# maneymarkus/BERT4Rec

Measured on AMD Instinct MI355X. Metric: masked positions/sec, higher is better.
Workload: dtype f32 (split products on the 16-bit matrix cores, fp32 accumulate: bf16 hi/lo x3 in the encoder, fp16 hi/lo x3 logits + x2 value products in the masked-LM head; softmax / LayerNorm / AdamW in fp32)

## Files before the change

bert4rec_amd/csrc/b4r_common.h:

```cpp
#pragma once
#include <hip/hip_runtime.h>
#include <stdint.h>
#include "../../include/b4r.h"

typedef float f32x4 __attribute__((ext_vector_type(4)));
typedef float f32x16 __attribute__((ext_vector_type(16)));

#define B4R_WAVE 64

void b4r_set_error(const char* fmt, ...);
#define B4R_CHECK_ARG(cond, code, ...)            \
  do {                                            \
    if (!(cond)) {                                \
      b4r_set_error(__VA_ARGS__);                 \
      return (code);                              \
    }                                             \
  } while (0)
void b4r_timing_mark(const char* what);
void b4r_timing_detail(const char* fmt, ...);
#define B4R_CHECK_LAUNCH(what)                                                   \
  do {                                                                           \
    hipError_t e__ = hipGetLastError();                                          \
    if (e__ != hipSuccess) {                                                     \
      b4r_set_error("%s: launch failed: %s", (what), hipGetErrorString(e__));    \
      return B4R_E_HIP;                                                          \
    }                                                                            \
    b4r_timing_mark(what);                                                       \
  } while (0)

static inline int b4r_cdiv(int64_t a, int64_t b) { return (int)((a + b - 1) / b); }
static inline bool b4r_aligned16(const void* p) { return (((uintptr_t)p) & 15u) == 0; }

struct B4rReduceJob {
  const float* slab; const float* cslab; const float* caslab;
  float* out; float* colsum; float* colsum_a;
  int S, Mo, No, ldo, accumulate;
  const long long* fix = nullptr; const long long* fix_hot = nullptr;
  int fix_hot_elems = 0, fix_slots = 0;
  const int* fix_poison = nullptr;
};
constexpr int B4R_MAX_REDUCE_JOBS = 40;
struct B4rReduceQueue {
  B4rReduceJob jobs[B4R_MAX_REDUCE_JOBS];
  int n;
};
void b4r_reduce_queue_begin(B4rReduceQueue* q);
int b4r_reduce_queue_flush(hipStream_t stream, float* sq_partial = nullptr, int sq_cap = 0, int* sq_np = nullptr,
                           int64_t* covered = nullptr);
bool b4r_reduce_queue_push(const B4rReduceJob& job);
bool b4r_reduce_queue_attach_fixed(const float* out, const long long* fix, const long long* fix_hot, int fix_hot_elems, int fix_slots,
                                   const int* fix_poison = nullptr);
int b4r_launch_reduce_job(const B4rReduceJob& job, hipStream_t stream);

struct B4rHeadMerge {
  const float* part; int slices, M, V;
  const float* T; const float* E; const float* bias; const int64_t* y;
  float* row_out; float* lse_out; int32_t* ylab;
};

#define B4R_STREAM_EMB 0u
#define B4R_STREAM_ATTN_PROBS(layer) (1u + 4u * (uint32_t)(layer))
#define B4R_STREAM_ATTN_OUT(layer) (2u + 4u * (uint32_t)(layer))
#define B4R_STREAM_FFN_OUT(layer) (3u + 4u * (uint32_t)(layer))

constexpr int B4R_ATTN_PITCH = 256;

struct DropArgs {
  const uint32_t* rng;
  uint32_t stream;
  uint32_t thr;
  float scale;
};

static inline DropArgs b4r_make_drop(const uint32_t* rng, uint32_t stream, float rate, int training) {
  DropArgs d;
  d.rng = nullptr; d.stream = stream; d.thr = 0; d.scale = 1.0f;
  if (training && rate > 0.0f && rng != nullptr) {
    d.rng = rng;
    d.thr = (uint32_t)((double)rate * 65536.0);
    d.scale = 1.0f / (1.0f - rate);
  }
  return d;
}

__host__ __device__ __forceinline__ uint32_t b4r_hash32(uint32_t x) {
  x ^= x >> 16; x *= 0x7FEB352Du; x ^= x >> 15; x *= 0x846CA68Bu; x ^= x >> 16;
  return x;
}

__host__ __device__ __forceinline__ float b4r_uniform23(uint32_t h) {
  return ((float)(h >> 9) + 0.5f) * (1.0f / 8388608.0f);
}

__host__ __device__ __forceinline__ uint32_t b4r_sample_word_hd(uint64_t seed, int64_t stream, int64_t id) {
  uint32_t h = b4r_hash32((uint32_t)(uint64_t)id ^ (uint32_t)seed);
  h = b4r_hash32((h ^ (uint32_t)(uint64_t)stream) + (uint32_t)(seed >> 32));
  return b4r_hash32(h ^ (uint32_t)((uint64_t)stream >> 32));
}

__host__ __device__ __forceinline__ double b4r_xln(double x) {
#pragma clang fp contract(off)
  const uint64_t b = __builtin_bit_cast(uint64_t, x);
  int e = (int)(b >> 52) - 1023;
  double m = __builtin_bit_cast(double, (b & 0x000FFFFFFFFFFFFFull) | 0x3FF0000000000000ull);
  if (m > 1.4142135623730951) { m = m * 0.5; e += 1; }
  const double s = (m - 1.0) / (m + 1.0);
  const double z = s * s;
  double p = 1.0 / 15.0;
  p = p * z + 1.0 / 13.0;
  p = p * z + 1.0 / 11.0;
  p = p * z + 1.0 / 9.0;
  p = p * z + 1.0 / 7.0;
  p = p * z + 1.0 / 5.0;
  p = p * z + 1.0 / 3.0;
  p = p * z + 1.0;
  return (double)e * 0.6931471805599453 + (2.0 * s) * p;
}

__host__ __device__ __forceinline__ float b4r_gumbel23(uint32_t h) {
#pragma clang fp contract(off)
  const double u = ((double)(h >> 9) + 0.5) * (1.0 / 8388608.0);
  return (float)(0.0 - b4r_xln(0.0 - b4r_xln(u)));
}

struct DropCtx {
  uint32_t seed, key, thr;
  float scale;
  bool on;
};

__device__ __forceinline__ DropCtx b4r_drop_ctx(const DropArgs& a) {
  DropCtx c;
  c.on = (a.rng != nullptr) && (a.thr != 0);
  c.thr = a.thr; c.scale = a.scale; c.seed = 0; c.key = 0;
  if (c.on) {
    c.seed = a.rng[0];
    c.key = b4r_hash32(a.stream * 0x9E3779B9u + a.rng[1]);
  }
  return c;
}

__device__ __forceinline__ void b4r_group_hash(const DropCtx& c, uint64_t g, uint32_t& h1, uint32_t& h2) {
  const uint32_t lo = (uint32_t)g, hi = (uint32_t)(g >> 32);
  uint32_t h = b4r_hash32(lo ^ c.seed);
  h = b4r_hash32((h ^ hi) + c.key);
  h1 = h;
  h ^= h << 13; h ^= h >> 17; h ^= h << 5;
  h2 = h;
}

struct B4rKeep4 {
  bool k[4];
  __device__ __forceinline__ uint32_t bits() const { return (k[0] ? 1u : 0u) | (k[1] ? 2u : 0u) | (k[2] ? 4u : 0u) | (k[3] ? 8u : 0u); }
};
__device__ __forceinline__ B4rKeep4 b4r_keep4p(const DropCtx& c, uint64_t idx4) {
  uint32_t h1, h2;
  b4r_group_hash(c, idx4 >> 2, h1, h2);
  B4rKeep4 r;
  r.k[0] = (h1 & 0xFFFFu) >= c.thr; r.k[1] = (h1 >> 16) >= c.thr;
  r.k[2] = (h2 & 0xFFFFu) >= c.thr; r.k[3] = (h2 >> 16) >= c.thr;
  return r;
}
__device__ __forceinline__ uint32_t b4r_keep4(const DropCtx& c, uint64_t idx4) { return b4r_keep4p(c, idx4).bits(); }

__device__ __forceinline__ bool b4r_keep(const DropCtx& c, uint64_t idx) {
  uint32_t h1, h2;
  b4r_group_hash(c, idx >> 2, h1, h2);
  const uint32_t w = (idx & 2) ? h2 : h1;
  const uint32_t u = (idx & 1) ? (w >> 16) : (w & 0xFFFFu);
  return u >= c.thr;
}

__device__ __forceinline__ float b4r_drop(const DropCtx& c, float x, uint64_t idx) {
  if (!c.on) return x;
  return b4r_keep(c, idx) ? x * c.scale : 0.0f;
}

__device__ __forceinline__ f32x4 b4r_drop4(const DropCtx& c, f32x4 x, uint64_t idx) {
  if (!c.on) return x;
  if ((idx & 3) == 0) {
    const B4rKeep4 k = b4r_keep4p(c, idx);
    const f32x4 xs = x * c.scale;
#pragma unroll
    for (int e = 0; e < 4; ++e) x[e] = k.k[e] ? xs[e] : 0.0f;
  } else {
#pragma unroll
    for (int e = 0; e < 4; ++e) x[e] = b4r_keep(c, idx + e) ? x[e] * c.scale : 0.0f;
  }
  return x;
}

#include <mutex>
#include <unordered_map>
static inline int b4r_raise_lds(const void* kernel, size_t bytes, const char* who) {
  if (bytes <= 48 * 1024) return B4R_OK;
  static std::mutex mu;
  static std::unordered_map<const void*, size_t> raised;
  std::lock_guard<std::mutex> lock(mu);
  auto it = raised.find(kernel);
  if (it != raised.end() && it->second >= bytes) return B4R_OK;
  hipError_t e = hipFuncSetAttribute(kernel, hipFuncAttributeMaxDynamicSharedMemorySize, (int)bytes);
  if (e != hipSuccess) { b4r_set_error("%s: cannot raise the LDS limit to %zu: %s", who, bytes, hipGetErrorString(e)); return B4R_E_HIP; }
  raised[kernel] = bytes;
  return B4R_OK;
}

typedef __bf16 b4r_bf16x8 __attribute__((ext_vector_type(8)));
typedef __bf16 b4r_bf16x4 __attribute__((ext_vector_type(4)));
typedef __bf16 b4r_bf16x2 __attribute__((ext_vector_type(2)));
typedef float b4r_f32x8 __attribute__((ext_vector_type(8)));
typedef float b4r_f32x2 __attribute__((ext_vector_type(2)));
typedef unsigned int b4r_u32x4 __attribute__((ext_vector_type(4)));
typedef unsigned int b4r_u32x2 __attribute__((ext_vector_type(2)));

__device__ __forceinline__ void b4r_split_pair(float a, float b, uint32_t& hw, uint32_t& lw) {
  const b4r_bf16x2 h = __builtin_convertvector((b4r_f32x2){a, b}, b4r_bf16x2);
  hw = __builtin_bit_cast(uint32_t, h);
  const float h0 = __builtin_bit_cast(float, hw << 16), h1 = __builtin_bit_cast(float, hw & 0xFFFF0000u);
  lw = __builtin_bit_cast(uint32_t, __builtin_convertvector((b4r_f32x2){a - h0, b - h1}, b4r_bf16x2));
}
__device__ __forceinline__ void b4r_split8(const b4r_f32x8 x, b4r_bf16x8& hi, b4r_bf16x8& lo) {
  b4r_u32x4 hw, lw;
#pragma unroll
  for (int j = 0; j < 4; ++j) {
    uint32_t h, l;
    b4r_split_pair(x[2 * j], x[2 * j + 1], h, l);
    hw[j] = h; lw[j] = l;
  }
  hi = __builtin_bit_cast(b4r_bf16x8, hw);
  lo = __builtin_bit_cast(b4r_bf16x8, lw);
}
__device__ __forceinline__ void b4r_split4(const f32x4 x, b4r_bf16x4& hi, b4r_bf16x4& lo) {
  b4r_u32x2 hw, lw;
#pragma unroll
  for (int j = 0; j < 2; ++j) {
    uint32_t h, l;
    b4r_split_pair(x[2 * j], x[2 * j + 1], h, l);
    hw[j] = h; lw[j] = l;
  }
  hi = __builtin_bit_cast(b4r_bf16x4, hw);
  lo = __builtin_bit_cast(b4r_bf16x4, lw);
}

__device__ __forceinline__ float b4r_gelu(float x) { return 0.5f * x * (1.0f + erff(x * 0.70710678118654752440f)); }
__device__ __forceinline__ float b4r_gelu_grad(float x) {
  return 0.5f * (1.0f + erff(x * 0.70710678118654752440f)) + x * 0.39894228040143267794f * __expf(-0.5f * x * x);
}

__device__ __forceinline__ float b4r_erf_as(float u, float& e) {
  const float a = fabsf(u);
  const float t = __builtin_amdgcn_rcpf(fmaf(0.3275911f, a, 1.0f));
  e = __expf(-a * a);
  float q = fmaf(t, 1.061405429f, -1.453152027f);
  q = fmaf(q, t, 1.421413741f);
  q = fmaf(q, t, -0.284496736f);
  q = fmaf(q, t, 0.254829592f);
  return copysignf(fmaf(-q * t, e, 1.0f), u);
}
__device__ __forceinline__ float b4r_gelu_fast(float x) {
  float e;
  return 0.5f * x * (1.0f + b4r_erf_as(x * 0.70710678118654752440f, e));
}
__device__ __forceinline__ float b4r_gelu_grad_fast(float x) {
  float e;
  const float er = b4r_erf_as(x * 0.70710678118654752440f, e);
  return fmaf(x * 0.39894228040143267794f, e, 0.5f * (1.0f + er));
}

constexpr int B4R_ACT_ANY = -1;
constexpr float B4R_SELU_ALPHA = 1.6732632423543772f, B4R_SELU_SCALE = 1.0507009873554805f;

template <bool FAST> __device__ __forceinline__ float b4r_exp_(float x) { return FAST ? __expf(x) : expf(x); }
template <bool FAST> __device__ __forceinline__ float b4r_rcp_(float x) { return FAST ? __builtin_amdgcn_rcpf(x) : 1.0f / x; }
template <bool FAST> __device__ __forceinline__ float b4r_sigmoid_(float x) { return b4r_rcp_<FAST>(1.0f + b4r_exp_<FAST>(-x)); }
template <bool FAST> __device__ __forceinline__ float b4r_tanh_(float x) {
  if (!FAST) return tanhf(x);
  const float t = 1.0f - 2.0f * __builtin_amdgcn_rcpf(__expf(2.0f * fabsf(x)) + 1.0f);
  return copysignf(t, x);
}
template <bool FAST> __device__ __forceinline__ float b4r_expm1_(float x) { return FAST ? __expf(x) - 1.0f : expm1f(x); }

template <bool FAST>
__device__ __forceinline__ void b4r_act_both(int id, float x, float& f, float& d) {
  switch (id) {
    case B4R_ACT_GELU:
      if (FAST) { float e; const float er = b4r_erf_as(x * 0.70710678118654752440f, e); const float cdf = 0.5f * (1.0f + er);
                  f = x * cdf; d = fmaf(x * 0.39894228040143267794f, e, cdf); }
      else { f = b4r_gelu(x); d = b4r_gelu_grad(x); }
      break;
    case B4R_ACT_RELU: f = x > 0.f ? x : 0.f; d = x > 0.f ? 1.f : 0.f; break;
    case B4R_ACT_SWISH: { const float s = b4r_sigmoid_<FAST>(x); f = x * s; d = s * fmaf(x, 1.0f - s, 1.0f); break; }
    case B4R_ACT_TANH: { const float t = b4r_tanh_<FAST>(x); f = t; d = fmaf(-t, t, 1.0f); break; }
    case B4R_ACT_SIGMOID: { const float s = b4r_sigmoid_<FAST>(x); f = s; d = s * (1.0f - s); break; }
    case B4R_ACT_ELU: { const float e = b4r_exp_<FAST>(fminf(x, 0.f)); f = x > 0.f ? x : b4r_expm1_<FAST>(fminf(x, 0.f)); d = x > 0.f ? 1.f : e; break; }
    case B4R_ACT_SELU: {
      const float e = b4r_exp_<FAST>(fminf(x, 0.f));
      f = x > 0.f ? B4R_SELU_SCALE * x : (B4R_SELU_SCALE * B4R_SELU_ALPHA) * b4r_expm1_<FAST>(fminf(x, 0.f));
      d = x > 0.f ? B4R_SELU_SCALE : (B4R_SELU_SCALE * B4R_SELU_ALPHA) * e;
      break;
    }
    case B4R_ACT_SOFTPLUS: {
      const float e = b4r_exp_<FAST>(-fabsf(x));
      f = fmaxf(x, 0.f) + (FAST ? __logf(1.0f + e) : log1pf(e));
      d = x >= 0.f ? b4r_rcp_<FAST>(1.0f + e) : e * b4r_rcp_<FAST>(1.0f + e);
      break;
    }
    default: f = x; d = 1.f; break;
  }
}
template <bool FAST> __device__ __forceinline__ float b4r_act_val(int id, float x) { float f, d; b4r_act_both<FAST>(id, x, f, d); return f; }
template <bool FAST> __device__ __forceinline__ float b4r_act_grad(int id, float x) { float f, d; b4r_act_both<FAST>(id, x, f, d); return d; }
template <int ACT> __device__ __forceinline__ int b4r_act_id(int id) { return ACT == B4R_ACT_ANY ? id : ACT; }

#include <type_traits>
template <class F>
static inline int b4r_act_dispatch(int act, F&& f) {
  switch (act) {
    case B4R_ACT_RELU: return f(std::integral_constant<int, B4R_ACT_RELU>{});
    case B4R_ACT_SWISH: return f(std::integral_constant<int, B4R_ACT_SWISH>{});
    case B4R_ACT_TANH: return f(std::integral_constant<int, B4R_ACT_TANH>{});
    case B4R_ACT_SIGMOID: return f(std::integral_constant<int, B4R_ACT_SIGMOID>{});
    case B4R_ACT_ELU: return f(std::integral_constant<int, B4R_ACT_ELU>{});
    case B4R_ACT_SELU: return f(std::integral_constant<int, B4R_ACT_SELU>{});
    case B4R_ACT_SOFTPLUS: return f(std::integral_constant<int, B4R_ACT_SOFTPLUS>{});
    case B4R_ACT_LINEAR: return f(std::integral_constant<int, B4R_ACT_LINEAR>{});
    default: return f(std::integral_constant<int, B4R_ACT_GELU>{});
  }
}

__device__ __forceinline__ float b4r_seq_amax(const int64_t* mask_row, int L) {
  int any = 0;
  for (int k = threadIdx.x; k < L; k += blockDim.x) any |= (mask_row[k] != 0) ? 1 : 0;
  return __syncthreads_or(any) ? 0.0f : -1e9f;
}

__device__ __forceinline__ float b4r_wave_sum(float v) {
#pragma unroll
  for (int o = 32; o > 0; o >>= 1) v += __shfl_xor(v, o, 64);
  return v;
}
__device__ __forceinline__ float b4r_wave_max(float v) {
#pragma unroll
  for (int o = 32; o > 0; o >>= 1) v = fmaxf(v, __shfl_xor(v, o, 64));
  return v;
}
```

bert4rec_amd/csrc/b4r_gemm.hip:

```cpp
#include "b4r_common.h"

namespace {

constexpr int BM = 128, BN = 64, BK = 32;
constexpr int LDS_A = BK + 4;
constexpr int LDS_BN = BN;
constexpr int LDS_BK = BK + 4;

struct GemmP {
  const float* A; const float* B; float* C; const float* bias; float* C2; const float* R;
  int lda, ldb, ldc, ldc2, ldr;
  int M, N, K;
  int tiles_n;
  int k_chunk;
  int64_t split_stride;
  int a_vec, b_vec;
  float qscale; int qcols;
  DropArgs drop;
  int act;
};
constexpr int EPI_BIAS_ACT = 12, EPI_ACT_BWD = 13;

__device__ __forceinline__ f32x4 load4_guard(const float* base, int64_t off, int n_valid, bool vec) {
  f32x4 v = {0.f, 0.f, 0.f, 0.f};
  if (n_valid >= 4 && vec) {
    v = *reinterpret_cast<const f32x4*>(base + off);
  } else {
#pragma unroll
    for (int e = 0; e < 4; ++e)
      if (e < n_valid) v[e] = base[off + e];
  }
  return v;
}

template <bool B_NK, int EPI, bool A_DROP>
__global__ __launch_bounds__(256) void gemm_kernel(GemmP p) {
  __shared__ __attribute__((aligned(16))) float sA[BM * LDS_A];
  __shared__ __attribute__((aligned(16))) float sB[B_NK ? BN * LDS_BK : BK * LDS_BN];

  const int tid = threadIdx.x, lane = tid & 63, wave = __builtin_amdgcn_readfirstlane(tid >> 6);
  const int tile_m = blockIdx.x / p.tiles_n, tile_n = blockIdx.x % p.tiles_n;
  const int m0 = tile_m * BM, n0 = tile_n * BN;
  const int h = lane >> 5, l31 = lane & 31;

  DropCtx dctx = b4r_drop_ctx(p.drop);

  f32x16 acc0, acc1;
#pragma unroll
  for (int i = 0; i < 16; ++i) { acc0[i] = 0.f; acc1[i] = 0.f; }

  f32x4 ra[4], rb[2];

  auto load_tiles = [&](int k0) {
#pragma unroll
    for (int i = 0; i < 4; ++i) {
      const int f = tid + 256 * i;
      const int row = f >> 3, c4 = (f & 7) * 4;
      const int gr = m0 + row, gk = k0 + c4;
      f32x4 v = {0.f, 0.f, 0.f, 0.f};
      if (gr < p.M) v = load4_guard(p.A, (int64_t)gr * p.lda + gk, p.K - gk, p.a_vec != 0);
      if (A_DROP) {
        if (dctx.on) {
#pragma unroll
          for (int e = 0; e < 4; ++e) v[e] = b4r_drop(dctx, v[e], (uint64_t)gr * (uint64_t)p.K + (uint64_t)(gk + e));
        }
      }
      ra[i] = v;
    }
#pragma unroll
    for (int i = 0; i < 2; ++i) {
      const int f = tid + 256 * i;
      f32x4 v = {0.f, 0.f, 0.f, 0.f};
      if (B_NK) {
        const int nr = f >> 3, c4 = (f & 7) * 4;
        const int gn = n0 + nr, gk = k0 + c4;
        if (gn < p.N) v = load4_guard(p.B, (int64_t)gn * p.ldb + gk, p.K - gk, p.b_vec != 0);
      } else {
        const int kr = f >> 4, c4 = (f & 15) * 4;
        const int gk = k0 + kr, gn = n0 + c4;
        if (gk < p.K) v = load4_guard(p.B, (int64_t)gk * p.ldb + gn, p.N - gn, p.b_vec != 0);
      }
      rb[i] = v;
    }
  };

  auto store_tiles = [&]() {
#pragma unroll
    for (int i = 0; i < 4; ++i) {
      const int f = tid + 256 * i;
      const int row = f >> 3, c4 = (f & 7) * 4;
      *reinterpret_cast<f32x4*>(&sA[row * LDS_A + c4]) = ra[i];
    }
#pragma unroll
    for (int i = 0; i < 2; ++i) {
      const int f = tid + 256 * i;
      if (B_NK) {
        const int nr = f >> 3, c4 = (f & 7) * 4;
        *reinterpret_cast<f32x4*>(&sB[nr * LDS_BK + c4]) = rb[i];
      } else {
        const int kr = f >> 4, c4 = (f & 15) * 4;
        *reinterpret_cast<f32x4*>(&sB[kr * LDS_BN + c4]) = rb[i];
      }
    }
  };

  const int k_begin = blockIdx.y * p.k_chunk;
  const int k_end = min(p.K, k_begin + p.k_chunk);
  const int nk = (k_end - k_begin + BK - 1) / BK;
  if (blockIdx.y > 0) p.C += (int64_t)blockIdx.y * p.split_stride;
  if (nk > 0) load_tiles(k_begin);
  for (int kt = 0; kt < nk; ++kt) {
    __syncthreads();
    store_tiles();
    __syncthreads();
    if (kt + 1 < nk) load_tiles(k_begin + (kt + 1) * BK);
    const int arow = wave * 32 + l31;
#pragma unroll
    for (int t = 0; t < 4; ++t) {
      const f32x4 a = *reinterpret_cast<const f32x4*>(&sA[arow * LDS_A + 8 * t + 4 * h]);
      if (B_NK) {
        const f32x4 b0 = *reinterpret_cast<const f32x4*>(&sB[l31 * LDS_BK + 8 * t + 4 * h]);
        const f32x4 b1 = *reinterpret_cast<const f32x4*>(&sB[(32 + l31) * LDS_BK + 8 * t + 4 * h]);
#pragma unroll
        for (int r = 0; r < 4; ++r) {
          acc0 = __builtin_amdgcn_mfma_f32_32x32x2f32(a[r], b0[r], acc0, 0, 0, 0);
          acc1 = __builtin_amdgcn_mfma_f32_32x32x2f32(a[r], b1[r], acc1, 0, 0, 0);
        }
      } else {
#pragma unroll
        for (int r = 0; r < 4; ++r) {
          const int kk = 8 * t + 4 * h + r;
          const float b0 = sB[kk * LDS_BN + l31];
          const float b1 = sB[kk * LDS_BN + 32 + l31];
          acc0 = __builtin_amdgcn_mfma_f32_32x32x2f32(a[r], b0, acc0, 0, 0, 0);
          acc1 = __builtin_amdgcn_mfma_f32_32x32x2f32(a[r], b1, acc1, 0, 0, 0);
        }
      }
    }
  }

#pragma unroll
  for (int jt = 0; jt < 2; ++jt) {
    const int col = n0 + jt * 32 + l31;
    if (col >= p.N) continue;
    float bv = 0.f;
    if (EPI == B4R_EPI_BIAS || EPI == B4R_EPI_BIAS_QSCALE || EPI == B4R_EPI_BIAS_GELU || EPI == B4R_EPI_BIAS_DROP_RES ||
        EPI == B4R_EPI_BIAS_TANH || EPI == EPI_BIAS_ACT)
      bv = p.bias[col];
    const float qs = (EPI == B4R_EPI_BIAS_QSCALE && col < p.qcols) ? p.qscale : 1.0f;
#pragma unroll
    for (int reg = 0; reg < 16; ++reg) {
      const int row = m0 + wave * 32 + (reg & 3) + 8 * (reg >> 2) + 4 * h;
      if (row >= p.M) continue;
      float v = (jt == 0 ? acc0[reg] : acc1[reg]);
      const int64_t co = (int64_t)row * p.ldc + col;
      if (EPI == B4R_EPI_NONE) {
        p.C[co] = v;
      } else if (EPI == B4R_EPI_BIAS) {
        p.C[co] = v + bv;
      } else if (EPI == B4R_EPI_BIAS_QSCALE) {
        p.C[co] = (v + bv) * qs;
      } else if (EPI == B4R_EPI_BIAS_GELU) {
        const float pre = v + bv;
        p.C2[(int64_t)row * p.ldc2 + col] = pre;
        p.C[co] = b4r_gelu(pre);
      } else if (EPI == EPI_BIAS_ACT) {
        const float pre = v + bv;
        p.C2[(int64_t)row * p.ldc2 + col] = pre;
        p.C[co] = b4r_act_val<false>(p.act, pre);
      } else if (EPI == B4R_EPI_BIAS_DROP_RES) {
        float y = v + bv;
        y = b4r_drop(dctx, y, (uint64_t)row * (uint64_t)p.N + (uint64_t)col);
        p.C[co] = p.R[(int64_t)row * p.ldr + col] + y;
      } else if (EPI == B4R_EPI_GELU_BWD) {
        p.C[co] = v * b4r_gelu_grad(p.R[(int64_t)row * p.ldr + col]);
      } else if (EPI == EPI_ACT_BWD) {
        p.C[co] = v * b4r_act_grad<false>(p.act, p.R[(int64_t)row * p.ldr + col]);
      } else if (EPI == B4R_EPI_ADD_RES) {
        p.C[co] = v + p.R[(int64_t)row * p.ldr + col];
      } else if (EPI == B4R_EPI_BIAS_TANH) {
        p.C[co] = tanhf(v + bv);
      }
    }
  }
}

constexpr int TB = 64;
constexpr int TK = 32;

struct TnP {
  const float* A; const float* B; float* slab; float* colsum_slab; float* colsum_a_slab;
  int lda, ldb;
  int R, Mo, No;
  int chunk;
  int a_vec, b_vec;
  DropArgs drop;
};

template <bool B_DROP>
__global__ __launch_bounds__(256) void gemm_tn_kernel(TnP p) {
  __shared__ __attribute__((aligned(16))) float sA[TK * TB];
  __shared__ __attribute__((aligned(16))) float sB[TK * TB];
  __shared__ float sRed[4 * TB];

  const int tid = threadIdx.x, lane = tid & 63, wave = __builtin_amdgcn_readfirstlane(tid >> 6);
  const int i0 = blockIdx.x * TB, j0 = blockIdx.y * TB, z = blockIdx.z;
  const int r_begin = z * p.chunk;
  const int r_end = min(p.R, r_begin + p.chunk);
  const int h = lane >> 5, l31 = lane & 31;
  const int wm = wave >> 1, wn = wave & 1;
  const bool do_colsum = (p.colsum_slab != nullptr) && (blockIdx.x == 0);
  const bool do_colsum_a = (p.colsum_a_slab != nullptr) && (blockIdx.y == 0);

  DropCtx dctx = b4r_drop_ctx(p.drop);

  f32x16 acc;
#pragma unroll
  for (int i = 0; i < 16; ++i) acc[i] = 0.f;
  float cs = 0.f, csa = 0.f;

  f32x4 ra[2], rb[2];
  auto load_tiles = [&](int r0) {
#pragma unroll
    for (int i = 0; i < 2; ++i) {
      const int f = tid + 256 * i;
      const int rr = f >> 4, c4 = (f & 15) * 4;
      const int gr = r0 + rr;
      f32x4 va = {0.f, 0.f, 0.f, 0.f}, vb = {0.f, 0.f, 0.f, 0.f};
      if (gr < r_end) {
        va = load4_guard(p.A, (int64_t)gr * p.lda + i0 + c4, p.Mo - (i0 + c4), p.a_vec != 0);
        vb = load4_guard(p.B, (int64_t)gr * p.ldb + j0 + c4, p.No - (j0 + c4), p.b_vec != 0);
        if (B_DROP) {
          if (dctx.on) {
#pragma unroll
            for (int e = 0; e < 4; ++e)
              vb[e] = b4r_drop(dctx, vb[e], (uint64_t)gr * (uint64_t)p.No + (uint64_t)(j0 + c4 + e));
          }
        }
      }
      ra[i] = va; rb[i] = vb;
    }
  };
  auto store_tiles = [&]() {
#pragma unroll
    for (int i = 0; i < 2; ++i) {
      const int f = tid + 256 * i;
      const int rr = f >> 4, c4 = (f & 15) * 4;
      *reinterpret_cast<f32x4*>(&sA[rr * TB + c4]) = ra[i];
      *reinterpret_cast<f32x4*>(&sB[rr * TB + c4]) = rb[i];
    }
  };

  if (r_begin < r_end) load_tiles(r_begin);
  for (int r0 = r_begin; r0 < r_end; r0 += TK) {
    __syncthreads();
    store_tiles();
    __syncthreads();
    if (r0 + TK < r_end) load_tiles(r0 + TK);
#pragma unroll
    for (int s = 0; s < 16; ++s) {
      const float a = sA[(2 * s + h) * TB + 32 * wm + l31];
      const float b = sB[(2 * s + h) * TB + 32 * wn + l31];
      acc = __builtin_amdgcn_mfma_f32_32x32x2f32(a, b, acc, 0, 0, 0);
    }
    if (do_colsum) {
#pragma unroll
      for (int r = 0; r < 8; ++r) cs += sB[(wave * 8 + r) * TB + lane];
    }
    if (do_colsum_a) {
#pragma unroll
      for (int r = 0; r < 8; ++r) csa += sA[(wave * 8 + r) * TB + lane];
    }
  }

  const int col = j0 + 32 * wn + l31;
  if (col < p.No) {
    float* slab = p.slab + (int64_t)z * p.Mo * p.No;
#pragma unroll
    for (int reg = 0; reg < 16; ++reg) {
      const int row = i0 + 32 * wm + (reg & 3) + 8 * (reg >> 2) + 4 * h;
      if (row < p.Mo) slab[(int64_t)row * p.No + col] = acc[reg];
    }
  }
  if (do_colsum) {
    sRed[wave * TB + lane] = cs;
    __syncthreads();
    if (tid < TB && j0 + tid < p.No)
      p.colsum_slab[(int64_t)z * p.No + j0 + tid] = (sRed[tid] + sRed[TB + tid]) + (sRed[2 * TB + tid] + sRed[3 * TB + tid]);
  }
  if (do_colsum_a) {
    __syncthreads();
    sRed[wave * TB + lane] = csa;
    __syncthreads();
    if (tid < TB && i0 + tid < p.Mo)
      p.colsum_a_slab[(int64_t)z * p.Mo + i0 + tid] = (sRed[tid] + sRed[TB + tid]) + (sRed[2 * TB + tid] + sRed[3 * TB + tid]);
  }
}

constexpr int RZ = 16;
constexpr int RE = 256;
constexpr int RQ = 4096;
typedef B4rReduceJob ReduceJobView;
__device__ __forceinline__ int reduce_mat_blocks(int S, int64_t total) { return (int)((total + (S <= RZ ? RQ : RE) - 1) / (S <= RZ ? RQ : RE)); }
__device__ __forceinline__ float reduce_store(const ReduceJobView& job, int64_t eo, float r) {
  const int row = (int)(eo / job.No), col = (int)(eo % job.No);
  float* o = job.out + (int64_t)row * job.ldo + col;
  if (job.fix != nullptr) {
    long long q = job.fix[eo];
    if (eo < job.fix_hot_elems) {
      for (int s0 = 0; s0 < job.fix_slots; s0 += 16) {
        long long v[16];
#pragma unroll
        for (int u = 0; u < 16; ++u) v[u] = s0 + u < job.fix_slots ? job.fix_hot[(int64_t)(s0 + u) * job.fix_hot_elems + eo] : 0ll;
#pragma unroll
        for (int u = 0; u < 16; ++u) q += v[u];
      }
    }
    r += (float)q * (1.f / 68719476736.f);
    if (job.fix_poison != nullptr && *job.fix_poison != 0) r = __builtin_nanf("");
  }
  if (job.accumulate) r += *o;
  *o = r;
  return r;
}
__device__ __forceinline__ float slab_reduce_block(const ReduceJobView& job, int block, float (*sp)[RE]) {
  float sq = 0.f;
  const int64_t total = (int64_t)job.Mo * job.No;
  const int mat_blocks = reduce_mat_blocks(job.S, total);
  const int lane = threadIdx.x & 63, zl = __builtin_amdgcn_readfirstlane(threadIdx.x >> 6);
  const bool vec = (total % 4 == 0) && ((reinterpret_cast<uintptr_t>(job.slab) & 15) == 0);
  if (block < mat_blocks && job.S <= RZ) {
    const int64_t e = (int64_t)block * RQ + 4 * (int64_t)threadIdx.x;
    if (e >= total) return sq;
    f32x4 v[RZ];
#pragma unroll
    for (int z = 0; z < RZ; ++z) {
      v[z] = (f32x4){0.f, 0.f, 0.f, 0.f};
      if (z < job.S) {
        if (vec) v[z] = *reinterpret_cast<const f32x4*>(job.slab + (int64_t)z * total + e);
        else
#pragma unroll
          for (int k = 0; k < 4; ++k)
            if (e + k < total) v[z][k] = job.slab[(int64_t)z * total + e + k];
      }
    }
    f32x4 r = {0.f, 0.f, 0.f, 0.f};
#pragma unroll
    for (int z = 0; z < RZ; ++z) r += v[z];
#pragma unroll
    for (int k = 0; k < 4; ++k)
      if (e + k < total) { const float w = reduce_store(job, e + k, r[k]); sq = fmaf(w, w, sq); }
    return sq;
  }
  if (block < mat_blocks) {
    const int64_t e = (int64_t)block * RE + 4 * lane;
    f32x4 s = {0.f, 0.f, 0.f, 0.f};
    if (vec) {
      if (e < total) {
        const float* src = job.slab + e;
        for (int z = zl; z < job.S; z += 8 * RZ) {
          f32x4 v[8];
#pragma unroll
          for (int u = 0; u < 8; ++u)
            v[u] = z + u * RZ < job.S ? *reinterpret_cast<const f32x4*>(src + (int64_t)(z + u * RZ) * total) : (f32x4){0.f, 0.f, 0.f, 0.f};
#pragma unroll
          for (int u = 0; u < 8; ++u) s += v[u];
        }
      }
    } else {
      for (int z = zl; z < job.S; z += RZ) {
#pragma unroll
        for (int c = 0; c < 4; ++c)
          if (e + c < total) s[c] += job.slab[(int64_t)z * total + e + c];
      }
    }
    *reinterpret_cast<f32x4*>(&sp[zl][4 * lane]) = s;
    __syncthreads();
    if (zl < 4) {
      const int l = threadIdx.x;
      const int64_t eo = (int64_t)block * RE + l;
      if (eo < total) {
        float r = 0.f;
#pragma unroll
        for (int z = 0; z < RZ; ++z) r += sp[z][l];
        const float v = reduce_store(job, eo, r);
        sq = v * v;
      }
    }
    return sq;
  }
  const int64_t n_cs = job.colsum ? job.No : 0, n_csa = job.colsum_a ? job.Mo : 0;
  const int64_t e = (int64_t)(block - mat_blocks) * 64 + lane;
  const float* src = nullptr;
  int64_t stride = 0, idx = 0;
  if (e < n_cs) { src = job.cslab; stride = job.No; idx = e; }
  else if (e < n_cs + n_csa) { src = job.caslab; stride = job.Mo; idx = e - n_cs; }
  float s = 0.f;
  if (src) {
    for (int z = zl; z < job.S; z += 8 * RZ) {
      float v[8];
#pragma unroll
      for (int u = 0; u < 8; ++u) v[u] = z + u * RZ < job.S ? src[(int64_t)(z + u * RZ) * stride + idx] : 0.f;
#pragma unroll
      for (int u = 0; u < 8; ++u) s += v[u];
    }
  }
  sp[zl][lane] = s;
  __syncthreads();
  if (zl == 0 && src) {
    float r = 0.f;
#pragma unroll
    for (int z = 0; z < RZ; ++z) r += sp[z][lane];
    if (e < n_cs) job.colsum[idx] = r;
    else job.colsum_a[idx] = r;
    sq = r * r;
  }
  return sq;
}

__global__ __launch_bounds__(64 * RZ) void slab_reduce_kernel(ReduceJobView job) {
  __shared__ __attribute__((aligned(16))) float sp[RZ][RE];
  (void)slab_reduce_block(job, (int)blockIdx.x, sp);
}

int slab_reduce_grid(int S, int Mo, int No, bool cs, bool csa) {
  return b4r_cdiv((int64_t)Mo * No, S <= RZ ? RQ : RE) + b4r_cdiv((int64_t)(cs ? No : 0) + (csa ? Mo : 0), 64);
}

int tn_split(int R, int Mo, int No) {
  const int tiles = b4r_cdiv(Mo, TB) * b4r_cdiv(No, TB);
  int S = b4r_cdiv(1024, tiles);
  const int max_s = b4r_cdiv(R, 4 * TK);
  if (S > max_s) S = max_s;
  if (S > 256) S = 256;
  if (S < 1) S = 1;
  return S;
}

template <bool B_NK, int EPI>
void launch_gemm(const GemmP& p, int a_drop, dim3 grid, hipStream_t s) {
  if (a_drop)
    hipLaunchKernelGGL((gemm_kernel<B_NK, EPI, true>), grid, dim3(256), 0, s, p);
  else
    hipLaunchKernelGGL((gemm_kernel<B_NK, EPI, false>), grid, dim3(256), 0, s, p);
}

template <bool B_NK>
int dispatch_epi(const GemmP& p, int epi, int a_drop, dim3 grid, hipStream_t s) {
  switch (epi) {
    case B4R_EPI_NONE: launch_gemm<B_NK, B4R_EPI_NONE>(p, a_drop, grid, s); break;
    case B4R_EPI_BIAS: launch_gemm<B_NK, B4R_EPI_BIAS>(p, a_drop, grid, s); break;
    case B4R_EPI_BIAS_QSCALE: launch_gemm<B_NK, B4R_EPI_BIAS_QSCALE>(p, a_drop, grid, s); break;
    case B4R_EPI_BIAS_GELU:
      if (p.act != B4R_ACT_GELU) launch_gemm<B_NK, EPI_BIAS_ACT>(p, a_drop, grid, s);
      else launch_gemm<B_NK, B4R_EPI_BIAS_GELU>(p, a_drop, grid, s);
      break;
    case B4R_EPI_BIAS_DROP_RES: launch_gemm<B_NK, B4R_EPI_BIAS_DROP_RES>(p, a_drop, grid, s); break;
    case B4R_EPI_GELU_BWD:
      if (p.act != B4R_ACT_GELU) launch_gemm<B_NK, EPI_ACT_BWD>(p, a_drop, grid, s);
      else launch_gemm<B_NK, B4R_EPI_GELU_BWD>(p, a_drop, grid, s);
      break;
    case B4R_EPI_ADD_RES: launch_gemm<B_NK, B4R_EPI_ADD_RES>(p, a_drop, grid, s); break;
    case B4R_EPI_BIAS_TANH: launch_gemm<B_NK, B4R_EPI_BIAS_TANH>(p, a_drop, grid, s); break;
    default: b4r_set_error("b4r_gemm_f32: unknown epilogue %d", epi); return B4R_E_BADARG;
  }
  return B4R_OK;
}

}

int b4r_launch_slab_reduce(const float* slab, int S, int Mo, int No, float* out, int ldo, int accumulate,
                           hipStream_t stream) {
  ReduceJobView job{slab, nullptr, nullptr, out, nullptr, nullptr, S, Mo, No, ldo, accumulate};
  hipLaunchKernelGGL(slab_reduce_kernel, dim3(slab_reduce_grid(S, Mo, No, false, false)), dim3(64 * RZ), 0, stream, job);
  B4R_CHECK_LAUNCH("slab_reduce");
  return B4R_OK;
}

namespace {
struct MultiReduceP {
  B4rReduceJob jobs[B4R_MAX_REDUCE_JOBS];
  int block_begin[B4R_MAX_REDUCE_JOBS + 1];
  int n;
  float* sq_partial;
};
__global__ __launch_bounds__(64 * RZ) void multi_slab_reduce_kernel(MultiReduceP p) {
  __shared__ __attribute__((aligned(16))) float sp[RZ][RE];
  int j = 0;
  while (j + 1 < p.n && (int)blockIdx.x >= p.block_begin[j + 1]) ++j;
  const B4rReduceJob q = p.jobs[j];
  float sq = slab_reduce_block(q, (int)blockIdx.x - p.block_begin[j], sp);
  if (p.sq_partial != nullptr) {
    __shared__ float s_sq[RZ];
    sq = b4r_wave_sum(sq);
    __syncthreads();
    if ((threadIdx.x & 63) == 0) s_sq[threadIdx.x >> 6] = sq;
    __syncthreads();
    if (threadIdx.x == 0) {
      float t = 0.f;
#pragma unroll
      for (int z = 0; z < RZ; ++z) t += s_sq[z];
      p.sq_partial[blockIdx.x] = t;
    }
  }
}
thread_local B4rReduceQueue* g_queue = nullptr;
}

void b4r_reduce_queue_begin(B4rReduceQueue* q) { q->n = 0; g_queue = q; }
bool b4r_reduce_queue_push(const B4rReduceJob& job) {
  if (g_queue == nullptr || g_queue->n >= B4R_MAX_REDUCE_JOBS) return false;
  g_queue->jobs[g_queue->n++] = job;
  return true;
}
bool b4r_reduce_queue_attach_fixed(const float* out, const long long* fix, const long long* fix_hot, int fix_hot_elems, int fix_slots,
                                   const int* fix_poison) {
  if (g_queue == nullptr) return false;
  for (int j = 0; j < g_queue->n; ++j) {
    B4rReduceJob& job = g_queue->jobs[j];
    if (job.out == out && job.ldo == job.No && job.fix == nullptr) {
      job.fix = fix; job.fix_hot = fix_hot; job.fix_hot_elems = fix_hot_elems; job.fix_slots = fix_slots; job.fix_poison = fix_poison;
      return true;
    }
  }
  return false;
}
int b4r_launch_reduce_job(const B4rReduceJob& job, hipStream_t stream) {
  if (b4r_reduce_queue_push(job)) return B4R_OK;
  hipLaunchKernelGGL(slab_reduce_kernel, dim3(slab_reduce_grid(job.S, job.Mo, job.No, job.colsum != nullptr, job.colsum_a != nullptr)),
                     dim3(64 * RZ), 0, stream, job);
  B4R_CHECK_LAUNCH("slab_reduce");
  return B4R_OK;
}
int b4r_reduce_queue_flush(hipStream_t stream, float* sq_partial, int sq_cap, int* sq_np, int64_t* covered) {
  B4rReduceQueue* q = g_queue;
  g_queue = nullptr;
  if (sq_np) *sq_np = 0;
  if (covered) *covered = 0;
  if (q == nullptr || q->n == 0) return B4R_OK;
  MultiReduceP p;
  p.n = q->n;
  int blocks = 0;
  int64_t elems = 0;
  for (int j = 0; j < q->n; ++j) {
    p.jobs[j] = q->jobs[j];
    p.block_begin[j] = blocks;
    blocks += slab_reduce_grid(q->jobs[j].S, q->jobs[j].Mo, q->jobs[j].No, q->jobs[j].colsum != nullptr, q->jobs[j].colsum_a != nullptr);
    elems += (int64_t)q->jobs[j].Mo * q->jobs[j].No + (q->jobs[j].colsum ? q->jobs[j].No : 0) + (q->jobs[j].colsum_a ? q->jobs[j].Mo : 0);
  }
  p.block_begin[q->n] = blocks;
  p.sq_partial = (sq_partial != nullptr && blocks <= sq_cap) ? sq_partial : nullptr;
  if (p.sq_partial && sq_np) *sq_np = blocks;
  if (covered) *covered = elems;
  hipLaunchKernelGGL(multi_slab_reduce_kernel, dim3(blocks), dim3(64 * RZ), 0, stream, p);
  B4R_CHECK_LAUNCH("multi_slab_reduce");
  return B4R_OK;
}

int b4r_launch_slab_reduce_full(const float* slab, int S, int Mo, int No, float* out, int ldo, int accumulate,
                                const float* cslab, float* colsum, const float* caslab, float* colsum_a, hipStream_t stream) {
  B4rReduceJob job{slab, cslab, caslab, out, colsum, colsum_a, S, Mo, No, ldo, accumulate};
  if (b4r_reduce_queue_push(job)) return B4R_OK;
  ReduceJobView view{slab, cslab, caslab, out, colsum, colsum_a, S, Mo, No, ldo, accumulate};
  hipLaunchKernelGGL(slab_reduce_kernel, dim3(slab_reduce_grid(S, Mo, No, colsum != nullptr, colsum_a != nullptr)), dim3(64 * RZ),
                     0, stream, view);
  B4R_CHECK_LAUNCH("slab_reduce");
  return B4R_OK;
}

int b4r_gemm_rx_launch(const b4r_gemm_desc* d, hipStream_t stream);
bool b4r_gemm_rx_supported(const b4r_gemm_desc* d);
bool b4r_gemm_rx_tn_supported(const b4r_gemm_tn_desc* d);
int64_t b4r_gemm_rx_tn_scratch_floats(int R, int Mo, int No);
int b4r_gemm_rx_tn_launch(const b4r_gemm_tn_desc* d, float* scratch, hipStream_t stream);
bool b4r_gemm_rx_tn_pair_supported(const b4r_gemm_tn_desc* d0, const b4r_gemm_tn_desc* d1);
int b4r_gemm_rx_tn_pair_launch(const b4r_gemm_tn_desc* d0, float* scratch0, const b4r_gemm_tn_desc* d1, float* scratch1,
                               hipStream_t stream);
static int g_gemm_mode = B4R_GEMM_BF16X3;
extern "C" int b4r_set_gemm_mode(int mode) {
  B4R_CHECK_ARG(mode == B4R_GEMM_F32 || mode == B4R_GEMM_BF16X3 || mode == B4R_GEMM_BF16, B4R_E_BADARG,
                "b4r_set_gemm_mode: unknown mode %d", mode);
  g_gemm_mode = mode;
  return B4R_OK;
}
extern "C" int b4r_get_gemm_mode(void) { return g_gemm_mode; }
extern "C" int b4r_split_mode(void) { return g_gemm_mode == B4R_GEMM_BF16X3 || g_gemm_mode == B4R_GEMM_BF16; }
extern "C" int b4r_gemm_terms(void) { return g_gemm_mode == B4R_GEMM_BF16 ? 1 : g_gemm_mode == B4R_GEMM_BF16X3 ? 3 : 0; }

extern "C" int64_t b4r_gemm_ln_bwd_partial_floats(int32_t M) { return (int64_t)b4r_cdiv(M > 0 ? M : 1, 64) * 128; }
extern "C" int b4r_gemm_ln_supported(const b4r_gemm_desc* d) {
  if (d == nullptr || !b4r_split_mode() || !d->A || !d->B || !d->C || d->M <= 0) return 0;
  if (d->epilogue == B4R_EPI_BIAS_GELU_LN) return b4r_gemm_rx_supported(d) ? 1 : 0;
  return ((d->epilogue == B4R_EPI_BIAS_DROP_RES_LN || d->epilogue == B4R_EPI_ADD_RES_LN_BWD) && d->R && d->ldr >= d->N &&
          b4r_gemm_rx_supported(d)) ? 1 : 0;
}

extern "C" int b4r_gemm_f32(const b4r_gemm_desc* d, b4r_stream_t stream) {
  B4R_CHECK_ARG(d != nullptr, B4R_E_BADARG, "b4r_gemm_f32: null descriptor");
  B4R_CHECK_ARG(d->A && d->B && d->C, B4R_E_BADARG, "b4r_gemm_f32: null operand");
  B4R_CHECK_ARG(d->M > 0 && d->N > 0 && d->K > 0, B4R_E_SHAPE, "b4r_gemm_f32: bad shape M=%d N=%d K=%d", d->M, d->N, d->K);
  B4R_CHECK_ARG(d->lda >= d->K && d->ldc >= d->N && d->ldb >= (d->b_is_nk ? d->K : d->N), B4R_E_SHAPE,
                "b4r_gemm_f32: leading dimension smaller than the row length");
  const int epi = d->epilogue;
  b4r_timing_detail("M=%d N=%d K=%d epi=%d%s", d->M, d->N, d->K, d->epilogue, d->b_is_nk ? " B^T" : "");
  const bool needs_bias = epi == B4R_EPI_BIAS || epi == B4R_EPI_BIAS_QSCALE || epi == B4R_EPI_BIAS_GELU ||
                          epi == B4R_EPI_BIAS_DROP_RES || epi == B4R_EPI_BIAS_TANH || epi == B4R_EPI_BIAS_DROP_RES_LN ||
                          epi == B4R_EPI_BIAS_GELU_LN;
  B4R_CHECK_ARG(!needs_bias || d->bias, B4R_E_BADARG, "b4r_gemm_f32: epilogue %d needs a bias", epi);
  const bool needs_r = epi == B4R_EPI_BIAS_DROP_RES || epi == B4R_EPI_GELU_BWD || epi == B4R_EPI_ADD_RES ||
                       epi == B4R_EPI_BIAS_DROP_RES_LN || epi == B4R_EPI_ADD_RES_LN_BWD;
  B4R_CHECK_ARG(!needs_r || (d->R && d->ldr >= d->N), B4R_E_BADARG, "b4r_gemm_f32: epilogue %d needs R", epi);
  B4R_CHECK_ARG(epi != B4R_EPI_BIAS_GELU || (d->C2 && d->ldc2 >= d->N), B4R_E_BADARG, "b4r_gemm_f32: BIAS_GELU needs C2");
  B4R_CHECK_ARG(epi >= B4R_EPI_NONE && epi <= B4R_EPI_BIAS_GELU_LN, B4R_E_BADARG, "b4r_gemm_f32: unknown epilogue %d", epi);
  B4R_CHECK_ARG(d->activation >= 0 && d->activation < B4R_ACT_COUNT, B4R_E_BADARG, "b4r_gemm_f32: unknown activation %d",
                d->activation);
  B4R_CHECK_ARG(d->a_gather_idx == nullptr || (epi == B4R_EPI_BIAS_GELU_LN && d->a_gather_add_per > 0 && d->a_gather_per > 0),
                B4R_E_BADARG, "b4r_gemm_f32: a_gather_idx only with B4R_EPI_BIAS_GELU_LN (and a_gather_add_per, a_gather_per > 0)");
  B4R_CHECK_ARG(d->a_copy == nullptr || (d->a_gather_idx != nullptr && d->a_copy_ld >= d->K && d->a_copy_ld % 4 == 0 &&
                                         b4r_aligned16(d->a_copy)),
                B4R_E_BADARG, "b4r_gemm_f32: a_copy needs a_gather_idx, a_copy_ld >= K (multiple of 4) and 16-byte alignment");
  if (epi == B4R_EPI_BIAS_GELU_LN) {
    B4R_CHECK_ARG(d->C2 && d->C3 && d->ln_gamma && d->ln_beta, B4R_E_BADARG, "b4r_gemm_f32: BIAS_GELU_LN needs C2, C3, ln_gamma, ln_beta");
    B4R_CHECK_ARG(b4r_gemm_ln_supported(d), B4R_E_SHAPE,
                  "b4r_gemm_f32: BIAS_GELU_LN not available for M=%d N=%d K=%d in this mode (b4r_gemm_ln_supported)", d->M, d->N,
                  d->K);
  }
  if (epi == B4R_EPI_ADD_RES_LN_BWD) {
    B4R_CHECK_ARG(d->C2 && d->ln_gamma && (d->ln_z || d->ln_ids) && d->ln_mean && d->ln_rstd && d->ln_dgamma, B4R_E_BADARG,
                  "b4r_gemm_f32: ADD_RES_LN_BWD needs C2 (partials), ln_gamma, ln_z (or ln_ids), ln_mean, ln_rstd, ln_dgamma");
    B4R_CHECK_ARG(!d->ln_ids || (d->ln_table && d->ln_pos && d->ln_L > 0 && d->ln_V > 0), B4R_E_BADARG,
                  "b4r_gemm_f32: ADD_RES_LN_BWD with ln_ids needs ln_table, ln_pos, ln_L, ln_V");
    B4R_CHECK_ARG(d->ln_dbeta == d->ln_dgamma + 64, B4R_E_BADARG, "b4r_gemm_f32: ADD_RES_LN_BWD: ln_dbeta must be ln_dgamma + 64");
    B4R_CHECK_ARG(b4r_gemm_ln_supported(d), B4R_E_SHAPE,
                  "b4r_gemm_f32: ADD_RES_LN_BWD not available for M=%d N=%d K=%d in this mode (b4r_gemm_ln_supported)", d->M,
                  d->N, d->K);
    int rc = b4r_gemm_rx_launch(d, (hipStream_t)stream);
    if (rc) return rc;
    return b4r_launch_slab_reduce_full(d->C2, b4r_cdiv(d->M, 64), 1, 128, d->ln_dgamma, 128, 0, nullptr, nullptr, nullptr, nullptr,
                                       (hipStream_t)stream);
  }
  if (epi == B4R_EPI_BIAS_DROP_RES_LN) {
    B4R_CHECK_ARG(d->C2 && d->ln_gamma && d->ln_beta, B4R_E_BADARG, "b4r_gemm_f32: BIAS_DROP_RES_LN needs C2, ln_gamma, ln_beta");
    B4R_CHECK_ARG(b4r_gemm_ln_supported(d), B4R_E_SHAPE,
                  "b4r_gemm_f32: BIAS_DROP_RES_LN not available for M=%d N=%d K=%d in this mode (b4r_gemm_ln_supported)", d->M,
                  d->N, d->K);
  }
  if (b4r_split_mode() && b4r_gemm_rx_supported(d)) return b4r_gemm_rx_launch(d, (hipStream_t)stream);

  GemmP p;
  p.A = d->A; p.B = d->B; p.C = d->C; p.bias = d->bias; p.C2 = d->C2; p.R = d->R;
  p.lda = d->lda; p.ldb = d->ldb; p.ldc = d->ldc; p.ldc2 = d->ldc2; p.ldr = d->ldr;
  p.M = d->M; p.N = d->N; p.K = d->K;
  p.tiles_n = b4r_cdiv(d->N, BN);
  p.k_chunk = b4r_cdiv(d->K, BK) * BK;
  p.split_stride = 0;
  p.a_vec = (b4r_aligned16(d->A) && (d->lda % 4 == 0)) ? 1 : 0;
  p.b_vec = (b4r_aligned16(d->B) && (d->ldb % 4 == 0)) ? 1 : 0;
  p.qscale = d->qscale; p.qcols = d->qcols;
  p.drop = b4r_make_drop(d->rng, d->drop_stream, d->drop_rate, 1);
  p.act = d->activation;
  const int a_drop = (d->a_dropout && p.drop.rng != nullptr) ? 1 : 0;
  const int64_t tiles = (int64_t)b4r_cdiv(d->M, BM) * p.tiles_n;
  B4R_CHECK_ARG(tiles < 2147483647LL, B4R_E_SHAPE, "b4r_gemm_f32: too many tiles");
  dim3 grid((unsigned)tiles);
  int rc = d->b_is_nk ? dispatch_epi<true>(p, epi, a_drop, grid, (hipStream_t)stream)
                      : dispatch_epi<false>(p, epi, a_drop, grid, (hipStream_t)stream);
  if (rc != B4R_OK) return rc;
  B4R_CHECK_LAUNCH("b4r_gemm_f32");
  return B4R_OK;
}

bool b4r_gemm_rx_splitk_supported(const b4r_gemm_desc* d, int k_pad_ok);
int b4r_gemm_rx_splitk_launch(const b4r_gemm_desc* d, int splits, float* slabs, int* slabs_used, hipStream_t stream);

int b4r_gemm_f32_splitk(const b4r_gemm_desc* d, int splits, float* scratch, int k_pad_ok, hipStream_t stream) {
  B4R_CHECK_ARG(d && scratch && d->epilogue == B4R_EPI_NONE && !d->a_dropout, B4R_E_BADARG, "gemm_splitk: plain product only");
  if (splits > 1 && b4r_split_mode() && b4r_gemm_rx_splitk_supported(d, k_pad_ok)) {
    int used = 0;
    int rc = b4r_gemm_rx_splitk_launch(d, splits, scratch, &used, stream);
    if (rc) return rc;
    return b4r_launch_slab_reduce(scratch, used, d->M, d->N, d->C, d->ldc, 0, stream);
  }
  if (splits <= 1) return b4r_gemm_f32(d, (b4r_stream_t)stream);
  GemmP p;
  p.A = d->A; p.B = d->B; p.C = scratch; p.bias = nullptr; p.C2 = nullptr; p.R = nullptr;
  p.lda = d->lda; p.ldb = d->ldb; p.ldc = d->N; p.ldc2 = 0; p.ldr = 0;
  p.M = d->M; p.N = d->N; p.K = d->K;
  p.tiles_n = b4r_cdiv(d->N, BN);
  p.k_chunk = b4r_cdiv(b4r_cdiv(d->K, splits), BK) * BK;
  p.split_stride = (int64_t)d->M * d->N;
  p.a_vec = (b4r_aligned16(d->A) && (d->lda % 4 == 0)) ? 1 : 0;
  p.b_vec = (b4r_aligned16(d->B) && (d->ldb % 4 == 0)) ? 1 : 0;
  p.qscale = 1.f; p.qcols = 0;
  p.drop = b4r_make_drop(nullptr, 0, 0.f, 0);
  p.act = B4R_ACT_GELU;
  const int64_t tiles = (int64_t)b4r_cdiv(d->M, BM) * p.tiles_n;
  dim3 grid((unsigned)tiles, (unsigned)splits);
  if (d->b_is_nk)
    hipLaunchKernelGGL((gemm_kernel<true, B4R_EPI_NONE, false>), grid, dim3(256), 0, stream, p);
  else
    hipLaunchKernelGGL((gemm_kernel<false, B4R_EPI_NONE, false>), grid, dim3(256), 0, stream, p);
  B4R_CHECK_LAUNCH("gemm_splitk");
  return b4r_launch_slab_reduce(scratch, splits, d->M, d->N, d->C, d->ldc, 0, stream);
}

extern "C" int64_t b4r_gemm_tn_scratch_floats(int32_t R, int32_t Mo, int32_t No) {
  if (R <= 0 || Mo <= 0 || No <= 0) return 0;
  const int S = tn_split(R, Mo, No);
  const int64_t a = (int64_t)S * Mo * No + (int64_t)S * No + (int64_t)S * Mo;
  const int64_t b = b4r_gemm_rx_tn_scratch_floats(R, Mo, No);
  return a > b ? a : b;
}

extern "C" int b4r_gemm_tn_dgrad_supported(const b4r_gemm_tn_desc* d) {
  return (d != nullptr && b4r_split_mode() && d->Mo >= 64 && d->Mo % 64 == 0 && d->No == 64 && d->R > 0 && d->A &&
          d->B && d->dgrad_w && d->dgrad_out && d->dgrad_ldw >= 64 && d->dgrad_ldw % 4 == 0 && b4r_aligned16(d->dgrad_w) &&
          d->dgrad_ldo >= d->Mo && (d->dgrad_gelu_pre == nullptr || d->dgrad_ldg >= d->Mo) && b4r_gemm_rx_tn_supported(d)) ? 1 : 0;
}

extern "C" int b4r_gemm_tn_f32(const b4r_gemm_tn_desc* d, float* scratch, b4r_stream_t stream) {
  B4R_CHECK_ARG(d != nullptr && scratch != nullptr, B4R_E_BADARG, "b4r_gemm_tn_f32: null argument");
  B4R_CHECK_ARG(d->A && d->B && d->out, B4R_E_BADARG, "b4r_gemm_tn_f32: null operand");
  B4R_CHECK_ARG(d->R > 0 && d->Mo > 0 && d->No > 0, B4R_E_SHAPE, "b4r_gemm_tn_f32: bad shape");
  B4R_CHECK_ARG(d->lda >= d->Mo && d->ldb >= d->No && d->ldo >= d->No, B4R_E_SHAPE, "b4r_gemm_tn_f32: bad leading dimension");
  b4r_timing_detail("R=%d Mo=%d No=%d%s", d->R, d->Mo, d->No, d->dgrad_out ? " +dgrad" : "");
  B4R_CHECK_ARG(d->activation >= 0 && d->activation < B4R_ACT_COUNT, B4R_E_BADARG, "b4r_gemm_tn_f32: unknown activation %d",
                d->activation);
  if (d->dgrad_out != nullptr) {
    B4R_CHECK_ARG(d->dgrad_w != nullptr, B4R_E_BADARG, "b4r_gemm_tn_f32: dgrad_out needs dgrad_w");
    B4R_CHECK_ARG(b4r_gemm_tn_dgrad_supported(d), B4R_E_SHAPE,
                  "b4r_gemm_tn_f32: the fused input gradient needs No = 64, Mo %% 64 == 0, aligned operands and the bf16x3 mode "
                  "(b4r_gemm_tn_dgrad_supported)");
  }
  if (b4r_split_mode() && b4r_gemm_rx_tn_supported(d)) return b4r_gemm_rx_tn_launch(d, scratch, (hipStream_t)stream);
  const int S = tn_split(d->R, d->Mo, d->No);
  TnP p;
  p.A = d->A; p.B = d->B; p.lda = d->lda; p.ldb = d->ldb;
  p.R = d->R; p.Mo = d->Mo; p.No = d->No;
  p.chunk = b4r_cdiv(b4r_cdiv(d->R, S), TK) * TK;
  p.slab = scratch;
  p.colsum_slab = d->colsum ? scratch + (int64_t)S * d->Mo * d->No : nullptr;
  p.colsum_a_slab = d->colsum_a ? scratch + (int64_t)S * d->Mo * d->No + (int64_t)S * d->No : nullptr;
  p.a_vec = (b4r_aligned16(d->A) && (d->lda % 4 == 0)) ? 1 : 0;
  p.b_vec = (b4r_aligned16(d->B) && (d->ldb % 4 == 0)) ? 1 : 0;
  p.drop = b4r_make_drop(d->rng, d->drop_stream, d->drop_rate, 1);
  const bool b_drop = d->b_dropout && p.drop.rng != nullptr;
  dim3 grid(b4r_cdiv(d->Mo, TB), b4r_cdiv(d->No, TB), S);
  if (b_drop)
    hipLaunchKernelGGL((gemm_tn_kernel<true>), grid, dim3(256), 0, (hipStream_t)stream, p);
  else
    hipLaunchKernelGGL((gemm_tn_kernel<false>), grid, dim3(256), 0, (hipStream_t)stream, p);
  B4R_CHECK_LAUNCH("b4r_gemm_tn_f32");
  return b4r_launch_slab_reduce_full(p.slab, S, d->Mo, d->No, d->out, d->ldo, d->accumulate, p.colsum_slab, d->colsum,
                                     p.colsum_a_slab, d->colsum_a, (hipStream_t)stream);
}

int b4r_gemm_tn_pair(const b4r_gemm_tn_desc* d0, float* scratch0, const b4r_gemm_tn_desc* d1, float* scratch1, hipStream_t stream) {
  const bool plain = d0 && d1 && scratch0 && scratch1 && d0->A && d0->B && d0->out && d1->A && d1->B && d1->out && d0->R > 0 &&
                     d1->R > 0 && d0->Mo > 0 && d0->No > 0 && d1->Mo > 0 && d1->No > 0 && d0->lda >= d0->Mo && d0->ldb >= d0->No &&
                     d0->ldo >= d0->No && d1->lda >= d1->Mo && d1->ldb >= d1->No && d1->ldo >= d1->No;
  if (plain && b4r_split_mode() && b4r_gemm_rx_tn_pair_supported(d0, d1))
    return b4r_gemm_rx_tn_pair_launch(d0, scratch0, d1, scratch1, stream);
  int rc = b4r_gemm_tn_f32(d0, scratch0, (b4r_stream_t)stream);
  if (rc) return rc;
  return b4r_gemm_tn_f32(d1, scratch1, (b4r_stream_t)stream);
}
```

bert4rec_amd/csrc/b4r_model.hip:

```cpp
#include <stdarg.h>
#include <stdio.h>
#include <string.h>

#include <string>
#include <vector>

#include <algorithm>
#include "b4r_common.h"

int b4r_ln_bwd_launch(const float* dy, const float* z, const float* mean, const float* rstd, const float* gamma,
                      int rows, int H, float* dz, float* dgamma, float* dbeta, float* scratch, const int64_t* ids,
                      const float* table, const float* pos_table, int L, int V, DropArgs drop, hipStream_t stream,
                      const float* gelu_pre = nullptr, const B4rHeadMerge* merge = nullptr, int act = B4R_ACT_GELU);
int b4r_scatter_add_rows_impl(const float* src, const int64_t* idx, int64_t idx_add_per, int per, int n, int H,
                              float* dst, int dst_ld, const int64_t* skip_if_zero, int64_t dst_rows, int hot_rows,
                              float* hot_scratch, hipStream_t stream);
int64_t b4r_scatter_hot_scratch_floats(int hot_rows, int H);
int b4r_batch_colsum(const float* x, int B, int L, int H, float* dpos, float* scratch, hipStream_t stream);
int b4r_gemm_f32_splitk(const b4r_gemm_desc* d, int splits, float* scratch, int k_pad_ok, hipStream_t stream);
bool b4r_head32_hidden_ok(int H);
int b4r_head32_fwd_slices(int M, int V, int H);
int64_t b4r_head32_fwd_scratch_floats(int M, int V, int H);
int64_t b4r_head32_dE_scratch_floats(int M, int V, int H);
bool b4r_head32_combine_foldable(int M, int V, int H);
// ... 847 lines not shown
  ModelCfg mc;
  RC(resolve_cfg(cfg_ex, &mc));
  const ModelCfg* cfg = &mc;
  B4R_CHECK_ARG(params && seq && rows && out && scratch && R > 0 && n_seq_rows > 0, B4R_E_BADARG, "b4r_mlm_transform_rows: bad argument");
  B4R_CHECK_ARG(b4r_aligned16(params) && b4r_aligned16(seq) && b4r_aligned16(out) && b4r_aligned16(scratch), B4R_E_ALIGN,
                "b4r_mlm_transform_rows: buffers must be 16-byte aligned");
  const ParamLayout pl = make_param_layout(*cfg);
  const int H = cfg->hidden_size, E = cfg->E;
  float* gath = scratch; float* upre = gath + up4((int64_t)R * H); float* u = upre + up4((int64_t)R * H);
  float* mean = u + up4((int64_t)R * H); float* rstd = mean + up4(R);
  return transform_fwd({.A = seq, .lda = H, .B = params + pl.wd, .ldb = E, .C = u, .ldc = E, .M = R, .N = E, .K = H,
                        .epilogue = B4R_EPI_BIAS_GELU_LN, .bias = params + pl.bd, .C2 = out, .ldc2 = E, .qscale = 1.f,
                        .c_pad_scratch = 0, .ln_gamma = params + pl.lnm_g, .ln_beta = params + pl.lnm_b, .ln_mean = mean,
                        .ln_rstd = rstd, .ln_eps = cfg->ln_eps, .C3 = upre, .ldc3 = E,
                        .a_gather_idx = rows, .a_gather_add_per = n_seq_rows, .a_gather_per = R ,
                        .activation = cfg->act_mlm},
                       gath, stream);
}
extern "C" int b4r_mlm_transform_rows(const b4r_model_config* cfg, const float* params, const float* seq, int64_t n_seq_rows,
                                      const int64_t* rows, int32_t R, float* out, float* scratch, b4r_stream_t stream) {
  const auto x = classic_ex(cfg);
  return b4r_mlm_transform_rows_ex(cfg ? &x : nullptr, params, seq, n_seq_rows, rows, R, out, scratch, stream);
}

extern "C" int b4r_loss_ex(const b4r_model_config_ex* cfg_ex, const b4r_batch* batch, void* workspace, int64_t workspace_bytes,
                           b4r_train_state* state, int32_t want_grad, b4r_stream_t stream) {
  ModelCfg mc;
  RC(resolve_cfg(cfg_ex, &mc));
  const ModelCfg* cfg = &mc;
  RC(check_batch(batch, cfg, true));
  B4R_CHECK_ARG(batch->masked_lm_ids && workspace && state, B4R_E_BADARG, "b4r_loss: needs masked_lm_ids, workspace, state");
  const WsLayout w = make_ws_layout(*cfg, batch->B, batch->L, batch->P);
  B4R_CHECK_ARG(workspace_bytes >= w.total * (int64_t)sizeof(float), B4R_E_NOMEM, "b4r_loss: workspace too small");
  float* ws = static_cast<float*>(workspace);
  if (want_grad & B4R_LOSS_FUSED_HEAD)
    return b4r_ce_finalize_launch(ws + w.rowsc, (int)w.M, state, (want_grad & B4R_LOSS_OVERWRITE) ? 1 : 0, (hipStream_t)stream);
  return b4r_softmax_ce(ws + w.logits, (int)w.M, cfg->vocab_size, (int)w.Vp, batch->masked_lm_ids, ws + w.rowsc, state,
                        want_grad & (1 | B4R_LOSS_OVERWRITE), stream);
}

extern "C" int b4r_loss(const b4r_model_config* cfg, const b4r_batch* batch, void* workspace, int64_t workspace_bytes,
                        b4r_train_state* state, int32_t want_grad, b4r_stream_t stream) {
  const auto x = classic_ex(cfg);
  return b4r_loss_ex(cfg ? &x : nullptr, batch, workspace, workspace_bytes, state, want_grad, stream);
}

namespace {

int head_bwd(Step& c) {
  const StepPlan& p = c.plan;
  const ParamLayout& pl = c.pl; const WsLayout& w = c.w;
  const int H = c.H, E = c.E, M = c.M, V = c.V, Vp = (int)w.Vp;
  const bool loss_sums = (c.flags & B4R_FLAG_LOSS_SUMS) != 0;
  float *fwd_part = nullptr, *dE_scratch = nullptr;
  if (p.fused_head && p.defer_combine) RC(c.take(b4r_head32_fwd_scratch_floats(M, V, E), &fwd_part));
  if (p.fused_head) RC(c.take(b4r_head32_dE_scratch_floats(M, V, E), &dE_scratch));
  alignas(8) char rider[128];
  int rider_blocks = 0;
  if (p.fused_head)
    RC(b4r_head32_dE_pack_job(c.at(w.t), c.at(w.head_lse), reinterpret_cast<const int32_t*>(c.at(w.head_ylab)), M, V, E, dE_scratch,
                              fwd_part, c.batch.masked_lm_ids, rider, sizeof(rider), &rider_blocks));
  RC(b4r_zero2(c.grads, pl.total, c.at(p.rows() ? w.hot : w.dx),
               p.rows() ? (p.slot_only_last ? w.db - w.hot : w.da - w.hot) : w.db - w.dx, c.s,
               ((c.flags & B4R_FLAG_GRAD_TAIL) && !p.defer_combine) ? c.grd(pl.total) : nullptr, c.state,
               (loss_sums && !p.defer_combine) ? c.at(w.rowsc) : nullptr, M, rider_blocks > 0 ? rider : nullptr, rider_blocks));

  float* dlog = c.at(w.logits);
  float* sc;
  if (p.fused_head) {
    RC(b4r_head32_dE_launch(c.at(w.t), c.prm(pl.word_emb), c.prm(pl.out_bias), c.at(w.head_lse),
                            reinterpret_cast<const int32_t*>(c.at(w.head_ylab)), M, V, E, dE_scratch, c.grd(pl.word_emb),
                            c.grd(pl.out_bias), c.s, fwd_part, c.batch.masked_lm_ids, rider_blocks > 0 ? 1 : 0));
  } else {
    const b4r_gemm_desc d{.A = dlog, .lda = Vp, .B = c.prm(pl.word_emb), .ldb = E, .C = c.at(w.dt), .ldc = E, .M = M, .N = E, .K = V,
                          .b_is_nk = 0, .epilogue = B4R_EPI_NONE};
    const int splits = mlm_dt_splits(M, E, V);
    RC(c.take((int64_t)splits * M * E, &sc));
    RC(b4r_gemm_f32_splitk(&d, splits, sc, (pl.word_emb + (int64_t)Vp * E <= pl.total) ? 1 : 0, c.s));
    RC(c.take(b4r_gemm_tn_scratch_floats(M, V, E), &sc));
    RC(gemm_tn_f32({.A = dlog, .lda = Vp, .B = c.at(w.t), .ldb = E, .out = c.grd(pl.word_emb), .ldo = E, .R = M, .Mo = V, .No = E,
                    .colsum_a = c.grd(pl.out_bias)}, sc, c.s));
  }
  const B4rHeadMerge merge{fwd_part, fwd_part ? b4r_head32_fwd_slices(M, V, E) : 0, M, V, c.at(w.t), c.prm(pl.word_emb),
                           c.prm(pl.out_bias), c.batch.masked_lm_ids, c.at(w.rowsc), c.at(w.head_lse),
                           reinterpret_cast<int32_t*>(c.at(w.head_ylab))};
  RC(c.take(b4r_ln_bwd_scratch_floats(M, E), &sc));
  RC(b4r_ln_bwd_launch(c.at(w.dt), c.at(w.u), c.at(w.meanm), c.at(w.rstdm), c.prm(pl.lnm_g), M, E, c.at(w.dt), c.grd(pl.lnm_g),
                       c.grd(pl.lnm_b), sc, nullptr, nullptr, nullptr, 1, 1, b4r_make_drop(nullptr, 0, 0.f, 0), c.s, c.at(w.upre),
                       fwd_part ? &merge : nullptr, c.cfg.act_mlm));
  b4r_gemm_tn_desc d{.A = c.at(w.gath), .lda = H, .B = c.at(w.dt), .ldb = E, .out = c.grd(pl.wd), .ldo = E, .R = M, .Mo = H, .No = E,
                     .colsum = c.grd(pl.bd), .dgrad_w = c.prm(pl.wd), .dgrad_ldw = E, .dgrad_out = c.at(w.dg), .dgrad_ldo = H};
  RC(c.take(b4r_gemm_tn_scratch_floats(M, H, E), &sc));
  if (b4r_gemm_tn_dgrad_supported(&d)) {
    RC(gemm_tn_f32(d, sc, c.s));
  } else {
    d.dgrad_w = nullptr; d.dgrad_ldw = 0; d.dgrad_out = nullptr; d.dgrad_ldo = 0;
    RC(gemm_tn_f32(d, sc, c.s));
    RC(gemm_f32({.A = c.at(w.dt), .lda = E, .B = c.prm(pl.wd), .ldb = E, .C = c.at(w.dg), .ldc = H, .M = M, .N = H, .K = E,
                 .b_is_nk = 1, .epilogue = B4R_EPI_NONE, .qscale = 1.f, .c_pad_scratch = 1}, c.s));
  }
  if (p.rows()) return B4R_OK;
  return b4r_scatter_add_rows_impl(c.at(w.dg), c.batch.masked_lm_positions, c.L, c.P, M, H, c.at(w.dx), H, c.batch.masked_lm_ids, c.N,
                                   0, nullptr, c.s);
}

int wgrad_with_dgrad(Step& c, b4r_gemm_tn_desc d, const b4r_gemm_desc& dx) {
  float* sc; RC(c.take(b4r_gemm_tn_scratch_floats(d.R, d.Mo, d.No), &sc));
  if (b4r_gemm_tn_dgrad_supported(&d)) return gemm_tn_f32(d, sc, c.s);
  RC(gemm_f32(dx, c.s));
  d.dgrad_w = nullptr; d.dgrad_ldw = 0; d.dgrad_out = nullptr; d.dgrad_ldo = 0; d.dgrad_gelu_pre = nullptr; d.dgrad_ldg = 0;
  return gemm_tn_f32(d, sc, c.s);
}

int ffn_bwd_block(Step& c, int i) {
  const ParamLayout& pl = c.pl; const WsLayout& w = c.w;
  b4r_ffn_desc fd = ffn_desc(c, i);
  fd.x1 = c.plan.x1_stored ? c.at(w.x1[i]) : nullptr;
  fd.dz2 = c.at(w.da); fd.z1 = c.at(w.z1[i]); fd.mean1 = c.at(w.mean1[i]); fd.rstd1 = c.at(w.rstd1[i]);
  fd.ln1_gamma = c.prm(pl.ln1_g[i]); fd.ln1_beta = c.prm(pl.ln1_b[i]); fd.dz1 = c.at(w.db);
  fd.dW1 = c.grd(pl.w1[i]); fd.db1 = c.grd(pl.b1[i]); fd.dW2 = c.grd(pl.w2[i]); fd.db2 = c.grd(pl.b2[i]);
  fd.dln1_gamma = c.grd(pl.ln1_g[i]);
  RC(c.take(b4r_ffn_block_bwd_scratch_floats(c.N), &fd.scratch));
  if (c.plan.head_rows && i == c.last) {
    fd.dz2 = nullptr;
    fd.slot_positions = c.batch.masked_lm_positions; fd.slot_ids = c.batch.masked_lm_ids; fd.slots_per_seq = c.batch.P; fd.seq_len = c.L;
    fd.max_rows = (int32_t)w.maxrows;
    fd.slot_grad = c.at(w.dg); fd.z2 = c.at(w.z2[i]); fd.mean2 = c.at(w.mean2[i]); fd.rstd2 = c.at(w.rstd2[i]);
    fd.ln_gamma = c.prm(pl.ln2_g[i]); fd.dln_gamma = c.grd(pl.ln2_g[i]); fd.dz2_rows = c.at(w.dz2c);
  }
  return b4r_ffn_block_bwd(&fd, c.s);
}

int ffn_bwd_compact(Step& c, int i) {
  const ParamLayout& pl = c.pl; const WsLayout& w = c.w;
  const int H = c.H, I = c.I, M = c.M;
  const int64_t* pos = c.batch.masked_lm_positions;
  const CompactRows cr = compact_rows(w, i, M, H, I);
  float* dz2c = c.at(w.dzc_a);
  float* dz2d = c.od > 0.f ? c.at(w.dzc_b) : dz2c;
  float* sc; RC(c.take(ln_scratch_floats(c.N, H), &sc));
  RC(b4r_ln_bwd_launch(c.at(w.dg), c.at(w.z2[i]), c.at(w.mean2[i]), c.at(w.rstd2[i]), c.prm(pl.ln2_g[i]), M, H, dz2c, c.grd(pl.ln2_g[i]),
                       c.grd(pl.ln2_b[i]), sc, nullptr, nullptr, nullptr, 1, 1, b4r_make_drop(nullptr, 0, 0.f, 0), c.s));
  if (c.od > 0.f)
    RC(b4r_slot_rows_drop(dz2c, pos, c.L, c.P, M, H, b4r_make_drop(c.rng, B4R_STREAM_FFN_OUT(i), c.od, 1), dz2d, c.s));
  RC(gemm_f32({.A = dz2d, .lda = H, .B = c.prm(pl.w2[i]), .ldb = H, .C = c.at(w.df), .ldc = I, .M = M, .N = I, .K = H, .b_is_nk = 1,
               .epilogue = B4R_EPI_GELU_BWD, .R = c.at(w.fpre[i]), .ldr = I, .qscale = 1.f, .c_pad_scratch = 1,
               .activation = c.cfg.act_inner}, c.s));
  RC(c.take(b4r_gemm_tn_scratch_floats(M, I, H), &sc));
  RC(gemm_tn_f32({.A = c.at(w.f[i]), .lda = I, .B = dz2d, .ldb = H, .out = c.grd(pl.w2[i]), .ldo = H, .R = M, .Mo = I, .No = H,
                  .colsum = c.grd(pl.b2[i])}, sc, c.s));
  RC(c.take(ln_scratch_floats(c.N, H), &sc));
  RC(dgrad_ln_bwd(c.at(w.df), I, c.prm(pl.w1[i]), I, dz2c, c.at(w.dz2c), M, H, c.at(cr.z1c), c.at(cr.mean1c), c.at(cr.rstd1c),
                  c.prm(pl.ln1_g[i]), c.grd(pl.ln1_g[i]), c.grd(pl.ln1_b[i]), sc, c.s));
  RC(c.take(b4r_gemm_tn_scratch_floats(M, H, I), &sc));
  RC(gemm_tn_f32({.A = c.at(cr.x1c), .lda = H, .B = c.at(w.df), .ldb = I, .out = c.grd(pl.w1[i]), .ldo = I, .R = M, .Mo = H, .No = I,
                  .colsum = c.grd(pl.b1[i])}, sc, c.s));
  return b4r_scatter_add_rows_impl(c.at(w.dz2c), pos, c.L, c.P, M, H, c.at(w.db), H, c.batch.masked_lm_ids, c.N, 0, nullptr, c.s);
}

int ffn_bwd_wide(Step& c, int i) {
  const ParamLayout& pl = c.pl; const WsLayout& w = c.w;
  const int H = c.H, I = c.I, N = c.N;
  b4r_ffn_desc fd = ffn_desc(c, i);
  fd.dz2 = c.at(w.da);
  RC(b4r_ffn32w_bwd(&fd, c.at(w.ffnrec[i]), c.at(w.fpre[i]), c.at(w.df), c.at(w.db), true, c.s));
  float* sc; RC(c.take(b4r_gemm_tn_scratch_floats(N, I, H), &sc));
  RC(gemm_tn_f32({.A = c.at(w.f[i]), .lda = I, .B = c.at(w.da), .ldb = H, .out = c.grd(pl.w2[i]), .ldo = H, .R = N, .Mo = I, .No = H,
                  .colsum = c.grd(pl.b2[i]), .rng = c.rng, .drop_stream = B4R_STREAM_FFN_OUT(i), .drop_rate = c.od, .b_dropout = 1},
                 sc, c.s));
  RC(c.take(ln_scratch_floats(N, H), &sc));
  RC(b4r_ln_bwd_launch(c.at(w.db), c.at(w.z1[i]), c.at(w.mean1[i]), c.at(w.rstd1[i]), c.prm(pl.ln1_g[i]), N, H, c.at(w.db),
                       c.grd(pl.ln1_g[i]), c.grd(pl.ln1_b[i]), sc, nullptr, nullptr, nullptr, 1, 1, b4r_make_drop(nullptr, 0, 0.f, 0), c.s));
  RC(c.take(b4r_gemm_tn_scratch_floats(N, H, I), &sc));
  return gemm_tn_f32({.A = c.at(w.x1[i]), .lda = H, .B = c.at(w.df), .ldb = I, .out = c.grd(pl.w1[i]), .ldo = I, .R = N, .Mo = H,
                      .No = I, .colsum = c.grd(pl.b1[i])}, sc, c.s);
}

int ffn_bwd_tiles(Step& c, int i) {
  const ParamLayout& pl = c.pl; const WsLayout& w = c.w;
  const int H = c.H, I = c.I, N = c.N;
  RC(wgrad_with_dgrad(c, {.A = c.at(w.f[i]), .lda = I, .B = c.at(w.da), .ldb = H, .out = c.grd(pl.w2[i]), .ldo = H, .R = N, .Mo = I,
                          .No = H, .colsum = c.grd(pl.b2[i]), .rng = c.rng, .drop_stream = B4R_STREAM_FFN_OUT(i), .drop_rate = c.od,
                          .b_dropout = 1, .dgrad_w = c.prm(pl.w2[i]), .dgrad_ldw = H, .dgrad_out = c.at(w.df), .dgrad_ldo = I,
                          .dgrad_gelu_pre = c.at(w.fpre[i]), .dgrad_ldg = I, .activation = c.cfg.act_inner},
                      {.A = c.at(w.da), .lda = H, .B = c.prm(pl.w2[i]), .ldb = H, .C = c.at(w.df), .ldc = I, .M = N, .N = I, .K = H,
                       .b_is_nk = 1, .epilogue = B4R_EPI_GELU_BWD, .R = c.at(w.fpre[i]), .ldr = I, .qscale = 1.f, .rng = c.rng,
                       .drop_stream = B4R_STREAM_FFN_OUT(i), .drop_rate = c.od, .a_dropout = 1, .c_pad_scratch = 1,
                       .activation = c.cfg.act_inner}));
  float* sc; RC(c.take(ln_scratch_floats(N, H), &sc));
  RC(dgrad_ln_bwd(c.at(w.df), I, c.prm(pl.w1[i]), I, c.at(w.da), c.at(w.db), N, H, c.at(w.z1[i]), c.at(w.mean1[i]), c.at(w.rstd1[i]),
                  c.prm(pl.ln1_g[i]), c.grd(pl.ln1_g[i]), c.grd(pl.ln1_b[i]), sc, c.s));
  RC(c.take(b4r_gemm_tn_scratch_floats(N, H, I), &sc));
  return gemm_tn_f32({.A = c.at(w.x1[i]), .lda = H, .B = c.at(w.df), .ldb = I, .out = c.grd(pl.w1[i]), .ldo = I, .R = N, .Mo = H,
                      .No = I, .colsum = c.grd(pl.b1[i])}, sc, c.s);
}

int attn_bwd_block(Step& c, int i, const float* x_in) {
  const ParamLayout& pl = c.pl; const WsLayout& w = c.w;
  const bool folded = c.plan.attn_bwd[i] == AttnBwd::BlockFolded;
  float* wo_scratch = nullptr;
  RC(c.take(b4r_gemm_tn_scratch_floats(c.N, c.H, c.H), &wo_scratch));
  b4r_attn_block_bwd_desc bd{};
  bd.B = c.B; bd.L = c.L; bd.H = c.H; bd.heads = c.cfg.num_heads;
  bd.x = x_in; bd.dz1 = c.at(w.db); bd.ctx = c.at(w.ctx[i]); bd.lse = c.at(w.lse[i]);
  bd.keep_bits = c.keep(i); bd.input_mask = c.batch.input_mask;
  bd.Wqkv = c.prm(pl.wqkv[i]); bd.bqkv = c.prm(pl.bqkv[i]); bd.Wo = c.prm(pl.wo[i]);
  bd.rng = (c.od > 0.f || c.adp > 0.f) ? c.rng : nullptr;
  bd.probs_stream = B4R_STREAM_ATTN_PROBS(i); bd.probs_rate = c.adp; bd.out_stream = B4R_STREAM_ATTN_OUT(i); bd.out_rate = c.od;
  if (i > 0) {
    bd.prev_z = c.at(w.z2[i - 1]); bd.prev_mean = c.at(w.mean2[i - 1]); bd.prev_rstd = c.at(w.rstd2[i - 1]);
    bd.prev_gamma = c.prm(pl.ln2_g[i - 1]); bd.dprev_gamma = c.grd(pl.ln2_g[i - 1]);
  } else {
    bd.prev_mean = c.at(w.mean0); bd.prev_rstd = c.at(w.rstd0); bd.prev_gamma = c.prm(pl.emb_ln_g); bd.dprev_gamma = c.grd(pl.emb_ln_g);
    bd.emb_ids = c.batch.input_word_ids; bd.emb_table = c.prm(pl.word_emb); bd.emb_pos = c.prm(pl.pos_emb); bd.emb_vocab = c.V;
    bd.emb_stream = B4R_STREAM_EMB; bd.emb_rate = c.od;
  }
  bd.dqkv = c.at(w.dqkv); bd.dx_prev = c.at(w.da);
  RC(c.take(b4r_attn_block_bwd_scratch_floats(c.B), &bd.scratch));
  if (folded) {
    bd.dqkv = nullptr; bd.dWqkv = c.grd(pl.wqkv[i]); bd.dbqkv = c.grd(pl.bqkv[i]);
    RC(c.take(b4r_attn_block_bwd_dw_scratch_floats(c.B), &bd.dw_scratch));
    bd.dWo = c.grd(pl.wo[i]); bd.dbo = c.grd(pl.bo[i]);
  }
  if (c.plan.slot_only_last && i == c.last) {
    bd.dz1_slot_positions = c.batch.masked_lm_positions; bd.dz1_slot_ids = c.batch.masked_lm_ids; bd.dz1_slots = c.batch.P;
  }
  RC(b4r_attn_block_bwd(&bd, c.s));
  if (folded) return B4R_OK;
  float* sc; RC(c.take(b4r_gemm_tn_scratch_floats(c.N, c.H, 3 * c.H), &sc));
  return attn_wgrad_pair(wo_grad_desc(c.at(w.ctx[i]), c.at(w.db), c.grd(pl.wo[i]), c.grd(pl.bo[i]), c.N, c.H, c.rng, B4R_STREAM_ATTN_OUT(i),
                                      c.od), wo_scratch, x_in, c.at(w.dqkv), c.grd(pl.wqkv[i]), c.grd(pl.bqkv[i]), sc, c.s);
}

int attn_bwd_slotq(Step& c, int i) {
  const ParamLayout& pl = c.pl; const WsLayout& w = c.w;
  const int H = c.H, M = c.M;
  const int64_t* pos = c.batch.masked_lm_positions;
  float* dz1d = c.od > 0.f ? c.at(w.dctx + up4((int64_t)M * H)) : c.at(w.dz2c);
  float* dctx_c = c.at(w.dctx);
  if (c.od > 0.f)
    RC(b4r_slot_rows_drop(c.at(w.dz2c), pos, c.L, c.P, M, H, b4r_make_drop(c.rng, B4R_STREAM_ATTN_OUT(i), c.od, 1), dz1d, c.s));
  float* sc; RC(c.take(b4r_gemm_tn_scratch_floats(c.N, H, H), &sc));
  RC(gemm_tn_f32({.A = c.at(w.ctx[i]), .lda = H, .B = dz1d, .ldb = H, .out = c.grd(pl.wo[i]), .ldo = H, .R = M, .Mo = H, .No = H,
                  .colsum = c.grd(pl.bo[i])}, sc, c.s));
  RC(gemm_f32({.A = dz1d, .lda = H, .B = c.prm(pl.wo[i]), .ldb = H, .C = dctx_c, .ldc = H, .M = M, .N = H, .K = H, .b_is_nk = 1,
               .epilogue = B4R_EPI_NONE, .qscale = 1.f, .c_pad_scratch = 1}, c.s));
  return b4r_attn32_slotq_bwd_launch(c.at(w.qkv[i]), c.batch.input_mask, pos, c.batch.masked_lm_ids, c.at(w.ctx[i]), c.at(w.lse[i]),
                                     dctx_c, c.B, c.L, c.cfg.num_heads, c.P, c.qscale, c.at(w.dqkv),
                                     b4r_make_drop(c.rng, B4R_STREAM_ATTN_PROBS(i), c.adp, 1), c.keep(i), c.s);
}

int attn_bwd_core(Step& c, int i) {
  const ParamLayout& pl = c.pl; const WsLayout& w = c.w;
  const int H = c.H;
  b4r_gemm_tn_desc d = wo_grad_desc(c.at(w.ctx[i]), c.at(w.db), c.grd(pl.wo[i]), c.grd(pl.bo[i]), c.N, H, c.rng, B4R_STREAM_ATTN_OUT(i),
                                    c.od);
  d.dgrad_w = c.prm(pl.wo[i]); d.dgrad_ldw = H; d.dgrad_out = c.at(w.dctx); d.dgrad_ldo = H;
  RC(wgrad_with_dgrad(c, d, {.A = c.at(w.db), .lda = H, .B = c.prm(pl.wo[i]), .ldb = H, .C = c.at(w.dctx), .ldc = H, .M = c.N, .N = H,
                             .K = H, .b_is_nk = 1, .epilogue = B4R_EPI_NONE, .qscale = 1.f, .rng = c.rng,
                             .drop_stream = B4R_STREAM_ATTN_OUT(i), .drop_rate = c.od, .a_dropout = 1, .c_pad_scratch = 1}));
  return b4r_attn_bwd_hd(c.at(w.qkv[i]), c.batch.input_mask, c.at(w.ctx[i]), c.at(w.lse[i]), c.at(w.dctx), c.B, c.L, c.cfg.num_heads,
                         head_dim(&c.cfg), c.qscale, c.at(w.dqkv), c.rng, B4R_STREAM_ATTN_PROBS(i), c.adp, c.keep(i), c.s);
}

int qkv_bwd(Step& c, int i, const float* x_in) {
  const ParamLayout& pl = c.pl; const WsLayout& w = c.w;
  const int H = c.H, N = c.N;
  float* sc; RC(c.take(ln_scratch_floats(N, H), &sc));
  if (i > 0)
    RC(dgrad_ln_bwd(c.at(w.dqkv), 3 * H, c.prm(pl.wqkv[i]), 3 * H, c.at(w.db), c.at(w.da), N, H, c.at(w.z2[i - 1]), c.at(w.mean2[i - 1]),
                    c.at(w.rstd2[i - 1]), c.prm(pl.ln2_g[i - 1]), c.grd(pl.ln2_g[i - 1]), c.grd(pl.ln2_b[i - 1]), sc, c.s));
  else if (c.plan.emb_proj)
    RC(gemm_f32({.A = c.at(w.dqkv), .lda = 3 * H, .B = c.prm(pl.wqkv[i]), .ldb = 3 * H, .C = c.at(w.da), .ldc = H, .M = N, .N = H,
                 .K = 3 * H, .b_is_nk = 1, .epilogue = B4R_EPI_ADD_RES, .R = c.at(w.db), .ldr = H, .qscale = 1.f, .c_pad_scratch = 1}, c.s));
  else
    RC(dgrad_ln_bwd(c.at(w.dqkv), 3 * H, c.prm(pl.wqkv[i]), 3 * H, c.at(w.db), c.at(w.da), N, H, nullptr, c.at(w.mean0), c.at(w.rstd0),
                    c.prm(pl.emb_ln_g), c.grd(pl.emb_ln_g), c.grd(pl.emb_ln_b), sc, c.s, c.batch.input_word_ids, c.prm(pl.word_emb),
                    c.prm(pl.pos_emb), c.L, c.V, c.rng, B4R_STREAM_EMB, c.od));
  RC(c.take(b4r_gemm_tn_scratch_floats(N, H, 3 * H), &sc));
  return gemm_tn_f32({.A = x_in, .lda = H, .B = c.at(w.dqkv), .ldb = 3 * H, .out = c.grd(pl.wqkv[i]), .ldo = 3 * H, .R = N, .Mo = H,
                      .No = 3 * H, .colsum = c.grd(pl.bqkv[i])}, sc, c.s);
}

}

static int backward_impl(const ModelCfg* cfg, const b4r_batch* batch, const StepPlan& plan, const float* params, float* grads,
                         void* workspace, int64_t workspace_bytes, b4r_train_state* state, int32_t flags, b4r_stream_t stream,
                         int* norm_np) {
  B4R_CHECK_ARG(params && grads && workspace && batch->masked_lm_ids, B4R_E_BADARG, "b4r_backward: null argument");
  B4R_CHECK_ARG(b4r_aligned16(params) && b4r_aligned16(grads) && b4r_aligned16(workspace), B4R_E_ALIGN,
                "b4r_backward: buffers must be 16-byte aligned");
  Step c(cfg, batch, plan, params, grads, workspace, state, flags, stream);
  B4R_CHECK_ARG(workspace_bytes >= c.w.total * (int64_t)sizeof(float), B4R_E_NOMEM, "b4r_backward: workspace too small");
  B4R_CHECK_ARG(!(flags & B4R_FLAG_GRAD_TAIL) || state, B4R_E_BADARG, "b4r_backward: B4R_FLAG_GRAD_TAIL needs the state");
  B4R_CHECK_ARG(!(flags & B4R_FLAG_LOSS_SUMS) || ((flags & B4R_FLAG_FUSED_HEAD) && state && batch->masked_lm_ids), B4R_E_BADARG,
                "b4r_backward: B4R_FLAG_LOSS_SUMS needs B4R_FLAG_FUSED_HEAD, the state and masked_lm_ids");
  B4R_CHECK_ARG(!plan.fused_head || fused_head_ok(*cfg), B4R_E_BADARG,
                "b4r_backward: B4R_FLAG_FUSED_HEAD needs an item-table width (hidden size or embedding_width) of 64 / 128 / 256 and the "
                "bf16x3 mode");
  B4R_CHECK_ARG(!plan.emb_proj || (plan.attn_bwd[0] != AttnBwd::Block && plan.attn_bwd[0] != AttnBwd::BlockFolded), B4R_E_SHAPE,
                "b4r_backward: the factorised embedding needs layer 0's attention backward as products");
  const ParamLayout& pl = c.pl; const WsLayout& w = c.w;
  B4rReduceQueue queue;
  b4r_reduce_queue_begin(&queue);
  RC(head_bwd(c));
  for (int i = c.last; i >= 0; --i) {
    const float* x_in = (i == 0) ? c.at(w.x0) : c.at(w.x2[i - 1]);
    if (i == c.last && !plan.rows()) {
      float* sc; RC(c.take(ln_scratch_floats(c.N, c.H), &sc));
      RC(b4r_ln_bwd_launch(c.at(w.dx), c.at(w.z2[i]), c.at(w.mean2[i]), c.at(w.rstd2[i]), c.prm(pl.ln2_g[i]), c.N, c.H, c.at(w.da),
                           c.grd(pl.ln2_g[i]), c.grd(pl.ln2_b[i]), sc, nullptr, nullptr, nullptr, 1, 1, b4r_make_drop(nullptr, 0, 0.f, 0),
                           c.s));
    }
    switch (plan.ffn[i]) {
      case FfnForm::Block: RC(ffn_bwd_block(c, i)); break;
      case FfnForm::CompactRows: RC(ffn_bwd_compact(c, i)); break;
      case FfnForm::Wide: RC(ffn_bwd_wide(c, i)); break;
      case FfnForm::TileProducts: RC(ffn_bwd_tiles(c, i)); break;
    }
    switch (plan.attn_bwd[i]) {
      case AttnBwd::Block: case AttnBwd::BlockFolded: RC(attn_bwd_block(c, i, x_in)); break;
      case AttnBwd::SlotQuery: RC(attn_bwd_slotq(c, i)); RC(qkv_bwd(c, i, x_in)); break;
      case AttnBwd::Core: RC(attn_bwd_core(c, i)); RC(qkv_bwd(c, i, x_in)); break;
    }
  }
  const float* emb_rows = c.at(w.da);
  if (plan.emb_proj) {
    float* psc; RC(c.take(b4r_embed_proj_bwd_scratch_floats_impl(c.N, c.E, c.H), &psc));
    RC(b4r_embed_proj_bwd_launch(c.at(w.da), batch->input_word_ids, c.B, c.L, c.prm(pl.word_emb), c.V, c.prm(pl.pos_emb), c.prm(pl.emb_ln_g),
                                 c.prm(pl.emb_ln_b), c.E, c.at(w.mean0), c.at(w.rstd0), c.prm(pl.proj_w), c.H,
                                 b4r_make_drop(c.rng, B4R_STREAM_EMB, c.od, 1), c.at(w.dctx), c.grd(pl.proj_w), c.grd(pl.proj_b),
                                 c.grd(pl.emb_ln_g), psc, c.s));
    emb_rows = c.at(w.dctx);
  }
  float* sc; RC(c.take((int64_t)b4r_cdiv(c.B, 16) * c.L * c.E, &sc));
  RC(b4r_embed_grads(emb_rows, batch->input_word_ids, c.B, c.L, c.E, c.grd(pl.word_emb), c.V, 3, c.at(w.hot) ,
                     c.grd(pl.pos_emb), sc, c.s, plan.defer_combine ? c.at(w.rowsc) : nullptr, (int)w.M, state,
                     (plan.defer_combine && (flags & B4R_FLAG_GRAD_TAIL)) ? c.grd(pl.total) : nullptr));
  if (norm_np) *norm_np = 0;
  if (!(flags & B4R_FLAG_NORM_PARTIALS_INTERNAL)) return b4r_reduce_queue_flush(c.s);
  int64_t expected = 0;
  for (const ParamEntry& e : pl.entries)
    expected += (int64_t)(e.offset == pl.pos_emb ? c.L : e.rows) * e.cols;
  int np = 0;
  int64_t covered = 0;
  RC(b4r_reduce_queue_flush(c.s, c.ws, 4096, &np, &covered));
  if (norm_np && np > 0 && covered == expected) *norm_np = np;
  return B4R_OK;
}

extern "C" int b4r_optimizer_step_ex(const b4r_model_config_ex* cfg_ex, const b4r_adamw_config* hp, float* params, const float* grads,
                                     float* adam_m, float* adam_v, void* workspace, int64_t workspace_bytes,
                                     b4r_train_state* state, b4r_stream_t stream) {
  ModelCfg mc;
  RC(resolve_cfg(cfg_ex, &mc));
  const ModelCfg* cfg = &mc;
  B4R_CHECK_ARG(hp && params && grads && adam_m && adam_v && workspace && state, B4R_E_BADARG, "b4r_optimizer_step: null argument");
  B4R_CHECK_ARG(workspace_bytes >= 4096 * (int64_t)sizeof(float), B4R_E_NOMEM, "b4r_optimizer_step: workspace too small");
  const ParamLayout pl = make_param_layout(*cfg);
  float* scratch = static_cast<float*>(workspace);
  return b4r_optimizer_fused(hp, params, grads, adam_m, adam_v, pl.total, pl.n_decay, scratch, state, (hipStream_t)stream);
}

extern "C" int b4r_optimizer_step(const b4r_model_config* cfg, const b4r_adamw_config* hp, float* params, const float* grads,
                                  float* adam_m, float* adam_v, void* workspace, int64_t workspace_bytes,
                                  b4r_train_state* state, b4r_stream_t stream) {
  const auto x = classic_ex(cfg);
  return b4r_optimizer_step_ex(cfg ? &x : nullptr, hp, params, grads, adam_m, adam_v, workspace, workspace_bytes, state, stream);
}

extern "C" int b4r_optimizer_step_reduced_ex(const b4r_model_config_ex* cfg_ex, const b4r_adamw_config* hp, float* params,
                                             const float* grads, float* adam_m, float* adam_v, void* workspace, int64_t workspace_bytes,
                                             b4r_train_state* state, b4r_stream_t stream) {
  ModelCfg mc;
  RC(resolve_cfg(cfg_ex, &mc));
  const ModelCfg* cfg = &mc;
  B4R_CHECK_ARG(hp && params && grads && adam_m && adam_v && workspace && state, B4R_E_BADARG, "b4r_optimizer_step_reduced: null argument");
  B4R_CHECK_ARG(workspace_bytes >= 4096 * (int64_t)sizeof(float), B4R_E_NOMEM, "b4r_optimizer_step_reduced: workspace too small");
  const ParamLayout pl = make_param_layout(*cfg);
  return b4r_optimizer_fused(hp, params, grads, adam_m, adam_v, pl.total, pl.n_decay, static_cast<float*>(workspace), state,
                             (hipStream_t)stream, 1);
}

extern "C" int b4r_optimizer_step_reduced(const b4r_model_config* cfg, const b4r_adamw_config* hp, float* params, const float* grads,
                                          float* adam_m, float* adam_v, void* workspace, int64_t workspace_bytes,
                                          b4r_train_state* state, b4r_stream_t stream) {
  const auto x = classic_ex(cfg);
  return b4r_optimizer_step_reduced_ex(cfg ? &x : nullptr, hp, params, grads, adam_m, adam_v, workspace, workspace_bytes, state, stream);
}

extern "C" int b4r_train_step_ex(const b4r_model_config_ex* cfg_ex, const b4r_adamw_config* hp, const b4r_batch* batch, float* params,
                                 float* grads, float* adam_m, float* adam_v, void* workspace, int64_t workspace_bytes,
                                 b4r_train_state* state, b4r_stream_t stream) {
  ModelCfg mc;
  RC(resolve_cfg(cfg_ex, &mc));
  const ModelCfg* cfg = &mc;
  RC(check_batch(batch, cfg, true));
  const int fused = fused_head_ok(*cfg) ? 1 : 0;
  const int defer = (fused && b4r_head32_combine_foldable(batch->B * batch->P, cfg->vocab_size, cfg->E))
                        ? B4R_FLAG_DEFER_COMBINE_INTERNAL : 0;
  const int32_t fwd_flags = B4R_FLAG_TRAINING | B4R_FLAG_HEAD_ROWS_ONLY | (fused ? B4R_FLAG_FUSED_HEAD : 0) | defer;
  const int32_t bwd_flags = fwd_flags | (fused ? B4R_FLAG_LOSS_SUMS : 0) | B4R_FLAG_NORM_PARTIALS_INTERNAL;
  const StepPlan plan = plan_step(cfg, batch, bwd_flags);
  RC(forward_impl(cfg, batch, plan, params, nullptr, workspace, workspace_bytes, state, fwd_flags, stream));
  if (!fused) RC(b4r_loss_ex(cfg_ex, batch, workspace, workspace_bytes, state, 1 | B4R_LOSS_OVERWRITE, stream));
  int np = 0;
  RC(backward_impl(cfg, batch, plan, params, grads, workspace, workspace_bytes, state, bwd_flags, stream, &np));
  if (np > 0) {
    B4R_CHECK_ARG(hp && adam_m && adam_v, B4R_E_BADARG, "b4r_train_step: null argument");
    const ParamLayout pl = make_param_layout(*cfg);
    return b4r_optimizer_fused(hp, params, grads, adam_m, adam_v, pl.total, pl.n_decay, static_cast<float*>(workspace), state,
                               (hipStream_t)stream, 0, np);
  }
  return b4r_optimizer_step_ex(cfg_ex, hp, params, grads, adam_m, adam_v, workspace, workspace_bytes, state, stream);
}
extern "C" int b4r_train_step(const b4r_model_config* cfg, const b4r_adamw_config* hp, const b4r_batch* batch, float* params,
                              float* grads, float* adam_m, float* adam_v, void* workspace, int64_t workspace_bytes,
                              b4r_train_state* state, b4r_stream_t stream) {
  const auto x = classic_ex(cfg);
  return b4r_train_step_ex(cfg ? &x : nullptr, hp, batch, params, grads, adam_m, adam_v, workspace, workspace_bytes, state, stream);
}
```

bert4rec_amd/csrc/b4r_rowops.hip:

```cpp
#include "b4r_common.h"
#include "b4r_head_merge.h"
#include "b4r_head32_pack.h"

int b4r_launch_slab_reduce_full(const float* slab, int S, int Mo, int No, float* out, int ldo, int accumulate,
                                const float* cslab, float* colsum, const float* caslab, float* colsum_a, hipStream_t stream);
int b4r_launch_slab_reduce(const float* slab, int S, int Mo, int No, float* out, int ldo, int accumulate,
                           hipStream_t stream);

namespace {

template <int LPR>
__device__ __forceinline__ float group_sum(float v) {
#pragma unroll
  for (int o = LPR / 2; o > 0; o >>= 1) v += __shfl_xor(v, o, 64);
  return v;
}

struct LnFwdP {
  const float* z;
  const int64_t* ids;
  const float* table;
  const float* pos_table;
  int L, V;
  const float* gamma; const float* beta;
  float* y; float* mean; float* rstd;
  int rows, H;
  float eps;
  DropArgs drop;
};

template <int LPR, int NV, bool EMBED>
__global__ __launch_bounds__(256) void ln_fwd_kernel(LnFwdP p) {
  constexpr int RPW = 64 / LPR;
  const int lane = threadIdx.x & 63, wave = __builtin_amdgcn_readfirstlane(threadIdx.x >> 6);
  const int sub = lane % LPR, slot = lane / LPR;
  const int64_t row = ((int64_t)blockIdx.x * 4 + wave) * RPW + slot;
  if (row >= p.rows) return;
  DropCtx dctx = b4r_drop_ctx(p.drop);

  f32x4 x[NV];
  float s = 0.f;
  if (EMBED) {
    int64_t id = p.ids[row];
    if (id < 0 || id >= p.V) id = 0;
    const int l = (int)(row % p.L);
#pragma unroll
    for (int v = 0; v < NV; ++v) {
      const int c = (v * LPR + sub) * 4;
      const f32x4 e = *reinterpret_cast<const f32x4*>(p.table + id * p.H + c);
      const f32x4 q = *reinterpret_cast<const f32x4*>(p.pos_table + (int64_t)l * p.H + c);
      x[v] = e + q;
    }
  } else {
#pragma unroll
    for (int v = 0; v < NV; ++v) {
      const int c = (v * LPR + sub) * 4;
      x[v] = *reinterpret_cast<const f32x4*>(p.z + row * p.H + c);
    }
  }
#pragma unroll
  for (int v = 0; v < NV; ++v) s += (x[v][0] + x[v][1]) + (x[v][2] + x[v][3]);
  const float mean = group_sum<LPR>(s) / (float)p.H;
  float q = 0.f;
#pragma unroll
  for (int v = 0; v < NV; ++v) {
#pragma unroll
    for (int e = 0; e < 4; ++e) { const float d = x[v][e] - mean; q += d * d; }
  }
  const float var = group_sum<LPR>(q) / (float)p.H;
  const float rstd = rsqrtf(var + p.eps);
#pragma unroll
  for (int v = 0; v < NV; ++v) {
    const int c = (v * LPR + sub) * 4;
    const f32x4 g = *reinterpret_cast<const f32x4*>(p.gamma + c);
    const f32x4 b = *reinterpret_cast<const f32x4*>(p.beta + c);
    f32x4 o;
#pragma unroll
    for (int e = 0; e < 4; ++e) {
      const float inv = rstd * g[e];
      o[e] = x[v][e] * inv + (b[e] - mean * inv);
    }
    o = b4r_drop4(dctx, o, (uint64_t)row * (uint64_t)p.H + (uint64_t)c);
    *reinterpret_cast<f32x4*>(p.y + row * p.H + c) = o;
  }
  if (sub == 0) {
    if (p.mean) p.mean[row] = mean;
    if (p.rstd) p.rstd[row] = rstd;
  }
}

struct LnBwdP {
  const float* dy; const float* z; const float* mean; const float* rstd; const float* gamma;
  const int64_t* ids; const float* table; const float* pos_table; int L, V;
  float* dz; float* partial;
  int rows, H;
  DropArgs drop;
  const float* gelu_pre;
  int act;
  HeadMergeP merge;
};

template <int LPR, int NV, bool EMBED, bool MERGE = false, int ACT = B4R_ACT_GELU>
__global__ __launch_bounds__(256) void ln_bwd_kernel(LnBwdP p) {
  constexpr int RPW = 64 / LPR;
  extern __shared__ float sred[];
  const int lane = threadIdx.x & 63, wave = __builtin_amdgcn_readfirstlane(threadIdx.x >> 6);
  const int sub = lane % LPR, slot = lane / LPR;
  DropCtx dctx = b4r_drop_ctx(p.drop);

  f32x4 g4[NV], dg[NV], db[NV];
#pragma unroll
  for (int v = 0; v < NV; ++v) {
    g4[v] = *reinterpret_cast<const f32x4*>(p.gamma + (v * LPR + sub) * 4);
    dg[v] = (f32x4){0.f, 0.f, 0.f, 0.f};
    db[v] = (f32x4){0.f, 0.f, 0.f, 0.f};
  }
  const int64_t rows_per_block = 4 * RPW;
  for (int64_t base = (int64_t)blockIdx.x * rows_per_block; base < p.rows; base += (int64_t)gridDim.x * rows_per_block) {
    const int64_t row = base + wave * RPW + slot;
    const bool live = row < p.rows;
    const int64_t rr = live ? row : 0;
    const float mean = p.mean[rr], rstd = p.rstd[rr];
    f32x4 xh[NV], gg[NV];
    float s1 = 0.f, s2 = 0.f;
    int64_t id = 0; int l = 0;
    if (EMBED) {
      id = p.ids[rr];
      if (id < 0 || id >= p.V) id = 0;
      l = (int)(rr % p.L);
    }
#pragma unroll
    for (int v = 0; v < NV; ++v) {
      const int c = (v * LPR + sub) * 4;
      f32x4 d;
      if (MERGE) d = head_merge_row<2>(p.merge, (int)rr, sub);
      else d = *reinterpret_cast<const f32x4*>(p.dy + rr * p.H + c);
      f32x4 zz;
      if (EMBED) {
        zz = *reinterpret_cast<const f32x4*>(p.table + id * p.H + c) +
             *reinterpret_cast<const f32x4*>(p.pos_table + (int64_t)l * p.H + c);
      } else {
        zz = *reinterpret_cast<const f32x4*>(p.z + rr * p.H + c);
      }
      if (EMBED) d = b4r_drop4(dctx, d, (uint64_t)rr * (uint64_t)p.H + (uint64_t)c);
#pragma unroll
      for (int e = 0; e < 4; ++e) {
        float de = d[e];
        if (!live) de = 0.f;
        const float xhat = (zz[e] - mean) * rstd;
        const float g = de * g4[v][e];
        xh[v][e] = xhat; gg[v][e] = g;
        s1 += g; s2 += g * xhat;
        dg[v][e] += de * xhat;
        db[v][e] += de;
      }
    }
    const float c1 = group_sum<LPR>(s1) / (float)p.H;
    const float c2 = group_sum<LPR>(s2) / (float)p.H;
    if (live) {
#pragma unroll
      for (int v = 0; v < NV; ++v) {
        const int c = (v * LPR + sub) * 4;
        f32x4 o;
#pragma unroll
        for (int e = 0; e < 4; ++e) o[e] = rstd * (gg[v][e] - c1 - xh[v][e] * c2);
        if (p.gelu_pre) {
          const f32x4 pre = *reinterpret_cast<const f32x4*>(p.gelu_pre + row * p.H + c);
#pragma unroll
          for (int e = 0; e < 4; ++e) o[e] *= (ACT == B4R_ACT_GELU) ? b4r_gelu_grad(pre[e]) : b4r_act_grad<false>(p.act, pre[e]);
        }
        *reinterpret_cast<f32x4*>(p.dz + row * p.H + c) = o;
      }
    }
  }
  const int srow = wave * RPW + slot;
#pragma unroll
  for (int v = 0; v < NV; ++v) {
    const int c = (v * LPR + sub) * 4;
#pragma unroll
    for (int e = 0; e < 4; ++e) {
      sred[srow * 2 * p.H + c + e] = dg[v][e];
      sred[srow * 2 * p.H + p.H + c + e] = db[v][e];
    }
  }
  __syncthreads();
  for (int c = threadIdx.x; c < 2 * p.H; c += 256) {
    float s = 0.f;
    for (int r = 0; r < 4 * RPW; ++r) s += sred[r * 2 * p.H + c];
    p.partial[(int64_t)blockIdx.x * 2 * p.H + c] = s;
  }
}

int ln_bwd_grid(int rows, int H) {
  int lpr = H / 4; if (lpr > 64) lpr = 64;
  const int rpb = 4 * (64 / lpr);
  int g = b4r_cdiv(rows, rpb);
  if (g > 1024) g = 1024;
  if (g < 1) g = 1;
  return g;
}

template <bool EMBED>
int launch_ln_fwd(const LnFwdP& p, hipStream_t s) {
  const int H = p.H;
#define LN_FWD_CASE(LPR_, NV_)                                                                              \
  {                                                                                                         \
    const int rpb = 4 * (64 / LPR_);                                                                        \
    hipLaunchKernelGGL((ln_fwd_kernel<LPR_, NV_, EMBED>), dim3(b4r_cdiv(p.rows, rpb)), dim3(256), 0, s, p); \
  }
  switch (H) {
    case 32: LN_FWD_CASE(8, 1) break;
    case 64: LN_FWD_CASE(16, 1) break;
    case 128: LN_FWD_CASE(32, 1) break;
    case 256: LN_FWD_CASE(64, 1) break;
    case 512: LN_FWD_CASE(64, 2) break;
    case 1024: LN_FWD_CASE(64, 4) break;
    default: b4r_set_error("layer norm: hidden size %d not supported (32,64,128,256,512,1024)", H); return B4R_E_SHAPE;
  }
#undef LN_FWD_CASE
  return B4R_OK;
}

template <bool EMBED, int ACT = B4R_ACT_GELU>
int launch_ln_bwd(const LnBwdP& p, int grid, hipStream_t s) {
  const int H = p.H;
  if (p.merge.part != nullptr) {
    if (EMBED || H != 64) { b4r_set_error("layer norm backward: the head merge needs hidden size 64"); return B4R_E_SHAPE; }
    hipLaunchKernelGGL((ln_bwd_kernel<16, 1, false, true, ACT>), dim3(grid), dim3(256), (size_t)4 * 4 * 2 * H * sizeof(float), s, p);
    return B4R_OK;
  }
#define LN_BWD_CASE(LPR_, NV_)                                                                           \
  {                                                                                                      \
    const size_t sh = (size_t)4 * (64 / LPR_) * 2 * H * sizeof(float);                                   \
    hipLaunchKernelGGL((ln_bwd_kernel<LPR_, NV_, EMBED, false, ACT>), dim3(grid), dim3(256), sh, s, p);  \
  }
  switch (H) {
    case 32: LN_BWD_CASE(8, 1) break;
    case 64: LN_BWD_CASE(16, 1) break;
    case 128: LN_BWD_CASE(32, 1) break;
    case 256: LN_BWD_CASE(64, 1) break;
    case 512: LN_BWD_CASE(64, 2) break;
    case 1024: LN_BWD_CASE(64, 4) break;
    default: b4r_set_error("layer norm: hidden size %d not supported", H); return B4R_E_SHAPE;
  }
#undef LN_BWD_CASE
  return B4R_OK;
}

__global__ __launch_bounds__(256) void gather_rows_kernel(const float* src, int src_ld, const int64_t* idx,
                                                          int64_t idx_add_per, int per, int n, int H, float* dst) {
  const int h4 = H / 4;
  const int64_t total = (int64_t)n * h4;
  for (int64_t t = (int64_t)blockIdx.x * 256 + threadIdx.x; t < total; t += (int64_t)gridDim.x * 256) {
    const int i = (int)(t / h4), c = (int)(t % h4) * 4;
    int64_t pos = idx[i];
    if (idx_add_per > 0) pos = pos < 0 ? 0 : (pos >= idx_add_per ? idx_add_per - 1 : pos);
    const int64_t r = pos + (int64_t)(i / per) * idx_add_per;
    *reinterpret_cast<f32x4*>(dst + (int64_t)i * H + c) = *reinterpret_cast<const f32x4*>(src + r * src_ld + c);
  }
}

constexpr int HOT_SLOTS = 64;
__device__ __forceinline__ void scatter_add_rows_body(const float* src, const int64_t* idx, int64_t idx_add_per,
                                                      int per, int n, int H, float* dst, int dst_ld,
                                                      const int64_t* skip_if_zero, int64_t dst_rows,
                                                      int hot_rows, float* hot_slab, const int block, const int nblocks) {
  extern __shared__ float s_hot[];
  for (int k = threadIdx.x; k < hot_rows * H; k += 256) s_hot[k] = 0.f;
  if (hot_rows > 0) __syncthreads();
  const int64_t total = (int64_t)n * H;
  for (int64_t t = (int64_t)block * 256 + threadIdx.x; t < total; t += (int64_t)nblocks * 256) {
    const int i = (int)(t / H), c = (int)(t % H);
    if (skip_if_zero != nullptr && skip_if_zero[i] == 0) continue;
    int64_t pos = idx[i];
    if (idx_add_per > 0) pos = pos < 0 ? 0 : (pos >= idx_add_per ? idx_add_per - 1 : pos);
    const int64_t r = pos + (int64_t)(i / per) * idx_add_per;
    if (r < 0 || r >= dst_rows) continue;
    const float v = src[(int64_t)i * H + c];
    if (r < hot_rows) atomicAdd(&s_hot[(int)r * H + c], v);
    else atomicAdd(dst + r * dst_ld + c, v);
  }
  if (hot_rows > 0) {
    __syncthreads();
    for (int k = threadIdx.x; k < hot_rows * H; k += 256) {
      const float v = s_hot[k];
      if (v == 0.f) continue;
      if (hot_slab) atomicAdd(hot_slab + (int64_t)(block % HOT_SLOTS) * hot_rows * H + k, v);
      else atomicAdd(dst + (int64_t)(k / H) * dst_ld + (k % H), v);
    }
  }
}

__global__ __launch_bounds__(256) void scatter_add_rows_kernel(const float* src, const int64_t* idx, int64_t idx_add_per,
                                                               int per, int n, int H, float* dst, int dst_ld,
                                                               const int64_t* skip_if_zero, int64_t dst_rows,
                                                               int hot_rows, float* hot_slab) {
  scatter_add_rows_body(src, idx, idx_add_per, per, n, H, dst, dst_ld, skip_if_zero, dst_rows, hot_rows, hot_slab, (int)blockIdx.x,
                        (int)gridDim.x);
}

__device__ __forceinline__ void batch_colsum_body(const float* x, int B, int L, int H, int bchunk, float* partial, const int bx, const int by) {
  const int h4 = H / 4;
  const int64_t t = (int64_t)bx * 256 + threadIdx.x;
  if (t >= (int64_t)L * h4) return;
  const int l = (int)(t / h4), c = (int)(t % h4) * 4;
  const int b0 = by * bchunk, b1 = min(B, b0 + bchunk);
  f32x4 s = {0.f, 0.f, 0.f, 0.f};
  for (int b = b0; b < b1; ++b) s += *reinterpret_cast<const f32x4*>(x + ((int64_t)b * L + l) * H + c);
  *reinterpret_cast<f32x4*>(partial + ((int64_t)by * L + l) * H + c) = s;
}
__global__ __launch_bounds__(256) void batch_colsum_kernel(const float* x, int B, int L, int H, int bchunk, float* partial) {
  batch_colsum_body(x, B, L, H, bchunk, partial, (int)blockIdx.x, (int)blockIdx.y);
}

constexpr float FIX_SCALE = 68719476736.f;
constexpr float FIX_UNSCALE = 1.f / 68719476736.f;
constexpr float FIX_LIMIT = 262144.f;
static float fix_contribution_limit(int64_t n) {
  if (n <= 512) return FIX_LIMIT;
  float lim = (float)(134217728.0 / (double)n);
  while ((double)lim * (double)n > 134217728.0) lim = nextafterf(lim, 0.f);
  return lim;
}
__device__ __forceinline__ void scatter_fixed_rows_body(const float* src, const int64_t* idx, int n, int H, long long* fix,
                                                        int64_t dst_rows, int hot_rows, long long* hot, const int block,
                                                        const int nblocks, int* poison, const float limit) {
  extern __shared__ unsigned long long s_hot64[];
  for (int k = threadIdx.x; k < hot_rows * H; k += 256) s_hot64[k] = 0ull;
  if (hot_rows > 0) __syncthreads();
  const int64_t total = (int64_t)n * H;
  for (int64_t t = (int64_t)block * 256 + threadIdx.x; t < total; t += (int64_t)nblocks * 256) {
    const int i = (int)(t / H), c = (int)(t % H);
    const int64_t r = idx[i];
    if (r < 0 || r >= dst_rows) continue;
    const float val = src[(int64_t)i * H + c];
    if (!(fabsf(val) < limit)) { atomicOr(poison, 1); continue; }
    const unsigned long long q = (unsigned long long)__float2ll_rn(val * FIX_SCALE);
    if (r < hot_rows) atomicAdd(&s_hot64[(int)r * H + c], q);
    else atomicAdd(reinterpret_cast<unsigned long long*>(fix) + r * H + c, q);
  }
  if (hot_rows > 0) {
    __syncthreads();
    for (int k = threadIdx.x; k < hot_rows * H; k += 256) {
      const unsigned long long v = s_hot64[k];
      if (v != 0ull) atomicAdd(reinterpret_cast<unsigned long long*>(hot) + (int64_t)(block % HOT_SLOTS) * hot_rows * H + k, v);
    }
  }
}

__global__ __launch_bounds__(256) void softmax_ce_kernel(float* logits, int V, int ld, const int64_t* y_true,
                                                         float* row_out, int want_grad) {
  __shared__ float s_val[4];
  __shared__ int s_idx[4];
  __shared__ float s_sum[4];
  const int m = blockIdx.x, tid = threadIdx.x, lane = tid & 63, wave = __builtin_amdgcn_readfirstlane(tid >> 6);
  float* row = logits + (int64_t)m * ld;
  const int nv = ld / 4;
  int64_t y = y_true[m];
  const bool y_ok = (y >= 0 && y < V);
  const float y_logit = y_ok ? row[y] : 0.f;

  float best = -INFINITY; int bidx = 0x7fffffff;
  for (int v = tid; v < nv; v += 256) {
    const f32x4 x = *reinterpret_cast<const f32x4*>(row + 4 * v);
#pragma unroll
    for (int e = 0; e < 4; ++e) {
      const int c = 4 * v + e;
      if (c < V && (x[e] > best || (x[e] == best && c < bidx))) { best = x[e]; bidx = c; }
    }
  }
#pragma unroll
  for (int o = 32; o > 0; o >>= 1) {
    const float ov = __shfl_xor(best, o, 64);
    const int oi = __shfl_xor(bidx, o, 64);
    if (ov > best || (ov == best && oi < bidx)) { best = ov; bidx = oi; }
  }
  if (lane == 0) { s_val[wave] = best; s_idx[wave] = bidx; }
  __syncthreads();
  best = s_val[0]; bidx = s_idx[0];
#pragma unroll
  for (int w = 1; w < 4; ++w)
    if (s_val[w] > best || (s_val[w] == best && s_idx[w] < bidx)) { best = s_val[w]; bidx = s_idx[w]; }

  float sum = 0.f;
  for (int v = tid; v < nv; v += 256) {
    const f32x4 x = *reinterpret_cast<const f32x4*>(row + 4 * v);
#pragma unroll
    for (int e = 0; e < 4; ++e)
      if (4 * v + e < V) sum += __expf(x[e] - best);
  }
  sum = b4r_wave_sum(sum);
  if (lane == 0) s_sum[wave] = sum;
  __syncthreads();
  sum = (s_sum[0] + s_sum[1]) + (s_sum[2] + s_sum[3]);
  const float lse = best + __logf(sum);
  const bool valid = (y != 0);
  if (tid == 0) {
    row_out[4 * (int64_t)m + 0] = (valid && y_ok) ? (lse - y_logit) : 0.f;
    row_out[4 * (int64_t)m + 1] = valid ? 1.f : 0.f;
    row_out[4 * (int64_t)m + 2] = (valid && (int64_t)bidx == y) ? 1.f : 0.f;
    row_out[4 * (int64_t)m + 3] = ((int64_t)bidx == y) ? 1.f : 0.f;
  }
  if (want_grad) {
    __syncthreads();
    const float inv_sum = 1.0f / sum;
    for (int v = tid; v < nv; v += 256) {
      f32x4 x = *reinterpret_cast<const f32x4*>(row + 4 * v);
#pragma unroll
      for (int e = 0; e < 4; ++e) {
        const int c = 4 * v + e;
        float g = 0.f;
        if (valid && c < V) g = __expf(x[e] - best) * inv_sum - ((int64_t)c == y ? 1.f : 0.f);
        x[e] = g;
      }
      *reinterpret_cast<f32x4*>(row + 4 * v) = x;
    }
  }
}

__device__ __forceinline__ void loss_rows_reduce(const float* rows, int M, float (*s)[256], float (&out)[4]) {
  const int tid = threadIdx.x;
  f32x4 acc = {0.f, 0.f, 0.f, 0.f};
  constexpr int U = 16;
  for (int m0 = tid; m0 < M; m0 += U * 256) {
    f32x4 r[U];
#pragma unroll
    for (int u = 0; u < U; ++u)
      r[u] = m0 + 256 * u < M ? *reinterpret_cast<const f32x4*>(rows + 4 * (int64_t)(m0 + 256 * u)) : (f32x4){0.f, 0.f, 0.f, 0.f};
#pragma unroll
    for (int u = 0; u < U; ++u)
      if (m0 + 256 * u < M) acc += r[u];
  }
#pragma unroll
  for (int q = 0; q < 4; ++q) s[q][tid] = acc[q];
  __syncthreads();
  if (tid < 256) {
    const int q = tid >> 6, l = tid & 63;
    float v = ((s[q][4 * l] + s[q][4 * l + 1]) + s[q][4 * l + 2]) + s[q][4 * l + 3];
    v = b4r_wave_sum(v);
    if (l == 0) s[q][0] = v;
  }
  __syncthreads();
#pragma unroll
  for (int q = 0; q < 4; ++q) out[q] = s[q][0];
}

__global__ __launch_bounds__(256) void embed_grads_kernel(const float* x, const int64_t* ids, int n, int H, long long* fix,
                                                          int64_t table_rows, int hot_rows, long long* hot, int n_scatter, int B, int L,
                                                          int bchunk, int gx, float* partial, int n_colsum, const float* fin_rows,
                                                          int fin_M, float* state_f, float* tail, float fix_limit) {
  if ((int)blockIdx.x < n_scatter) {
    scatter_fixed_rows_body(x, ids, n, H, fix, table_rows, hot_rows, hot, (int)blockIdx.x, n_scatter,
                            reinterpret_cast<int*>(hot + (int64_t)HOT_SLOTS * hot_rows * H), fix_limit);
  } else if ((int)blockIdx.x < n_scatter + n_colsum) {
    const int k = (int)blockIdx.x - n_scatter;
    batch_colsum_body(x, B, L, H, bchunk, partial, k % gx, k / gx);
  } else {
    __shared__ float s[4][256];
    float r[4];
    loss_rows_reduce(fin_rows, fin_M, s, r);
    if (threadIdx.x == 0) {
      state_f[4] = r[0]; state_f[5] = r[1]; state_f[6] = r[2]; state_f[7] = r[3];
      state_f[8] = (float)fin_M; state_f[9] = 0.f; state_f[10] = 0.f;
    }
    if (tail != nullptr && threadIdx.x < 8) tail[threadIdx.x] = threadIdx.x < 4 ? r[threadIdx.x] : (threadIdx.x == 4 ? (float)fin_M : 0.f);
  }
}

__global__ __launch_bounds__(256) void ce_finalize_kernel(const float* row_out, int M, b4r_train_state* st, int overwrite) {
  __shared__ float s[4][256];
  float r[4];
  loss_rows_reduce(row_out, M, s, r);
  if (threadIdx.x == 0) {
    if (overwrite) {
      st->loss_sum = 0.f; st->valid_count = 0.f; st->correct_masked = 0.f; st->correct_all = 0.f; st->slots_all = 0.f;
      st->grad_sqnorm = 0.f; st->grad_norm = 0.f;
    }
    st->loss_sum += r[0];
    st->valid_count += r[1];
    st->correct_masked += r[2];
    st->correct_all += r[3];
    st->slots_all += (float)M;
  }
}

__global__ void state_begin_kernel(b4r_train_state* st) {
  if (threadIdx.x == 0 && blockIdx.x == 0) {
    st->loss_sum = 0.f; st->valid_count = 0.f; st->correct_masked = 0.f; st->correct_all = 0.f; st->slots_all = 0.f;
    st->grad_sqnorm = 0.f; st->grad_norm = 0.f;
  }
}

__global__ __launch_bounds__(256) void sqnorm_partial_kernel(const float* g, int64_t n, float* partial, const float* tail = nullptr,
                                                             float* state_f = nullptr) {
  __shared__ float s[4];
  if (tail != nullptr && blockIdx.x == 0 && threadIdx.x < 5) state_f[4 + threadIdx.x] = tail[threadIdx.x];
  const int64_t n4 = n / 4;
  const int64_t per = (n4 + gridDim.x - 1) / gridDim.x;
  const int64_t b = (int64_t)blockIdx.x * per, e = min(n4, b + per);
  float acc = 0.f;
  for (int64_t i = b + threadIdx.x; i < e; i += 256) {
    const f32x4 v = *reinterpret_cast<const f32x4*>(g + 4 * i);
    acc += (v[0] * v[0] + v[1] * v[1]) + (v[2] * v[2] + v[3] * v[3]);
  }
  if (blockIdx.x == gridDim.x - 1) {
    for (int64_t i = n4 * 4 + threadIdx.x; i < n; i += 256) acc += g[i] * g[i];
  }
  acc = b4r_wave_sum(acc);
  if ((threadIdx.x & 63) == 0) s[threadIdx.x >> 6] = acc;
  __syncthreads();
  if (threadIdx.x == 0) partial[blockIdx.x] = (s[0] + s[1]) + (s[2] + s[3]);
}

__global__ __launch_bounds__(256) void sqnorm_final_kernel(const float* partial, int np, b4r_train_state* st) {
  __shared__ float s[256];
  float a = 0.f;
  for (int i = threadIdx.x; i < np; i += 256) a += partial[i];
  s[threadIdx.x] = a;
  __syncthreads();
  for (int o = 128; o > 0; o >>= 1) {
    if (threadIdx.x < o) s[threadIdx.x] += s[threadIdx.x + o];
    __syncthreads();
  }
  if (threadIdx.x == 0) st->grad_sqnorm = s[0];
}

struct AdamP {
  float* p; const float* g; float* m; float* v;
  int64_t n, n_decay;
  b4r_adamw_config hp;
  b4r_train_state* st;
};

__device__ __forceinline__ float mul_then_add(float a, float b, float c) {
#pragma clang fp contract(off)
  const float prod = a * b;
  return prod + c;
}

__device__ __forceinline__ float lr_schedule(const b4r_adamw_config& hp, int64_t step) {
  const float s = (float)step;
  if (hp.num_warmup_steps > 0 && s < (float)hp.num_warmup_steps) return hp.init_lr * (s / (float)hp.num_warmup_steps);
  const float T = (float)hp.num_train_steps;
  const float gs = fminf(s, T);
  const float pr = gs / T;
  return mul_then_add(hp.init_lr - hp.end_lr, 1.0f - pr, hp.end_lr);
}

__global__ __launch_bounds__(256) void adamw_kernel(AdamP a) {
  const int64_t step = a.st->step;
  const float cnt = a.st->valid_count;
  const float inv_cnt = cnt > 0.f ? 1.0f / cnt : 1.0f;
  const float gnorm = sqrtf(a.st->grad_sqnorm) * inv_cnt;
  const float clip_scale = a.hp.clip_norm > 0.f ? a.hp.clip_norm / fmaxf(gnorm, a.hp.clip_norm) : 1.0f;
  const float lr_t = lr_schedule(a.hp, step);
  const float t = (float)(step + 1);
  const float b1p = powf(a.hp.beta_1, t), b2p = powf(a.hp.beta_2, t);
  const float alpha = lr_t * sqrtf(1.0f - b2p) / (1.0f - b1p);
  const float omb1 = 1.0f - a.hp.beta_1, omb2 = 1.0f - a.hp.beta_2;
  const float wd = a.hp.weight_decay_rate, eps = a.hp.epsilon;
  const int64_t n4 = a.n / 4;
  for (int64_t i = (int64_t)blockIdx.x * 256 + threadIdx.x; i < n4; i += (int64_t)gridDim.x * 256) {
    f32x4 p = *reinterpret_cast<f32x4*>(a.p + 4 * i);
    const f32x4 g = *reinterpret_cast<const f32x4*>(a.g + 4 * i);
    f32x4 m = *reinterpret_cast<f32x4*>(a.m + 4 * i);
    f32x4 v = *reinterpret_cast<f32x4*>(a.v + 4 * i);
#pragma unroll
    for (int e = 0; e < 4; ++e) {
      const float ge = (g[e] * inv_cnt) * clip_scale;
      float pe = p[e];
      if (wd != 0.f && (a.hp.decay_mask ? a.hp.decay_mask[4 * i + e] != 0 : 4 * i + e < a.n_decay)) pe -= lr_t * pe * wd;
      m[e] += (ge - m[e]) * omb1;
      v[e] += (ge * ge - v[e]) * omb2;
      pe -= (m[e] * alpha) / (sqrtf(v[e]) + eps);
      p[e] = pe;
    }
    *reinterpret_cast<f32x4*>(a.p + 4 * i) = p;
    *reinterpret_cast<f32x4*>(a.m + 4 * i) = m;
    *reinterpret_cast<f32x4*>(a.v + 4 * i) = v;
  }
  if (blockIdx.x == 0 && threadIdx.x == 0) { a.st->grad_norm = gnorm; a.st->lr = lr_t; }
}

__global__ __launch_bounds__(256) void adamw_fused_kernel(AdamP a, const float* partial, int np, unsigned int* ticket) {
  __shared__ float s_red[256];
  const int64_t n4 = a.n / 4;
  const int64_t i0 = (int64_t)blockIdx.x * 256 + threadIdx.x;
  const int64_t i0c = i0 < n4 ? i0 : 0;
  f32x4 p0 = *reinterpret_cast<f32x4*>(a.p + 4 * i0c);
  const f32x4 g0 = *reinterpret_cast<const f32x4*>(a.g + 4 * i0c);
  f32x4 m0 = *reinterpret_cast<f32x4*>(a.m + 4 * i0c);
  f32x4 v0 = *reinterpret_cast<f32x4*>(a.v + 4 * i0c);
  const int64_t step = a.st->step;
  const float cnt = a.st->valid_count;
  float acc = 0.f;
  for (int i = threadIdx.x; i < np; i += 256) acc += partial[i];
  s_red[threadIdx.x] = acc;
  __syncthreads();
  for (int o = 128; o > 0; o >>= 1) {
    if (threadIdx.x < o) s_red[threadIdx.x] += s_red[threadIdx.x + o];
    __syncthreads();
  }
  const float sqnorm = s_red[0];
  const float inv_cnt = cnt > 0.f ? 1.0f / cnt : 1.0f;
  const float gnorm = sqrtf(sqnorm) * inv_cnt;
  const float clip_scale = a.hp.clip_norm > 0.f ? a.hp.clip_norm / fmaxf(gnorm, a.hp.clip_norm) : 1.0f;
  const float lr_t = lr_schedule(a.hp, step);
  const float t = (float)(step + 1);
  const float b1p = powf(a.hp.beta_1, t), b2p = powf(a.hp.beta_2, t);
  const float alpha = lr_t * sqrtf(1.0f - b2p) / (1.0f - b1p);
  const float omb1 = 1.0f - a.hp.beta_1, omb2 = 1.0f - a.hp.beta_2;
  const float wd = a.hp.weight_decay_rate, eps = a.hp.epsilon;
  for (int64_t i = i0; i < n4; i += (int64_t)gridDim.x * 256) {
    f32x4 p, g, m, v;
    if (i == i0) { p = p0; g = g0; m = m0; v = v0; }
    else {
      p = *reinterpret_cast<f32x4*>(a.p + 4 * i);
      g = *reinterpret_cast<const f32x4*>(a.g + 4 * i);
      m = *reinterpret_cast<f32x4*>(a.m + 4 * i);
      v = *reinterpret_cast<f32x4*>(a.v + 4 * i);
    }
#pragma unroll
    for (int e = 0; e < 4; ++e) {
      const float ge = (g[e] * inv_cnt) * clip_scale;
      float pe = p[e];
      if (wd != 0.f && (a.hp.decay_mask ? a.hp.decay_mask[4 * i + e] != 0 : 4 * i + e < a.n_decay)) pe -= lr_t * pe * wd;
      m[e] += (ge - m[e]) * omb1;
      v[e] += (ge * ge - v[e]) * omb2;
      pe -= (m[e] * alpha) / (sqrtf(v[e]) + eps);
      p[e] = pe;
    }
    *reinterpret_cast<f32x4*>(a.p + 4 * i) = p;
    *reinterpret_cast<f32x4*>(a.m + 4 * i) = m;
    *reinterpret_cast<f32x4*>(a.v + 4 * i) = v;
  }
  __builtin_amdgcn_s_barrier();
  if (threadIdx.x == 0) {
    if (atomicAdd(ticket, 1u) == gridDim.x - 1) {
      a.st->grad_sqnorm = sqnorm; a.st->grad_norm = gnorm; a.st->lr = lr_t;
      a.st->step = step + 1; a.st->step_lo = (uint32_t)(step + 1);
      *ticket = 0u;
    }
  }
}

__global__ void state_advance_kernel(b4r_train_state* st) {
  if (threadIdx.x == 0 && blockIdx.x == 0) { st->step += 1; st->step_lo = (uint32_t)st->step; }
}

}

extern "C" int b4r_embed_ln_fwd(const int64_t* ids, int32_t B, int32_t L, const float* table, int32_t V,
                                const float* pos_table, const float* gamma, const float* beta, int32_t H, float eps,
                                float* out, float* mean, float* rstd, const uint32_t* rng, float dropout,
                                b4r_stream_t stream) {
  B4R_CHECK_ARG(ids && table && pos_table && gamma && beta && out, B4R_E_BADARG, "b4r_embed_ln_fwd: null argument");
  B4R_CHECK_ARG(B > 0 && L > 0 && V > 0, B4R_E_SHAPE, "b4r_embed_ln_fwd: bad shape");
  LnFwdP p{};
  p.ids = ids; p.table = table; p.pos_table = pos_table; p.L = L; p.V = V;
  p.gamma = gamma; p.beta = beta; p.y = out; p.mean = mean; p.rstd = rstd;
  p.rows = B * L; p.H = H; p.eps = eps;
  p.drop = b4r_make_drop(rng, B4R_STREAM_EMB, dropout, 1);
  int rc = launch_ln_fwd<true>(p, (hipStream_t)stream);
  if (rc) return rc;
  B4R_CHECK_LAUNCH("b4r_embed_ln_fwd");
  return B4R_OK;
}

extern "C" int b4r_ln_fwd(const float* z, int32_t rows, int32_t H, const float* gamma, const float* beta, float eps,
                          float* y, float* mean, float* rstd, b4r_stream_t stream) {
  B4R_CHECK_ARG(z && gamma && beta && y, B4R_E_BADARG, "b4r_ln_fwd: null argument");
  B4R_CHECK_ARG(rows > 0, B4R_E_SHAPE, "b4r_ln_fwd: bad shape");
  LnFwdP p{};
  p.z = z; p.gamma = gamma; p.beta = beta; p.y = y; p.mean = mean; p.rstd = rstd;
  p.rows = rows; p.H = H; p.eps = eps; p.L = 1; p.V = 1;
  p.drop = b4r_make_drop(nullptr, 0, 0.f, 0);
  int rc = launch_ln_fwd<false>(p, (hipStream_t)stream);
  if (rc) return rc;
  B4R_CHECK_LAUNCH("b4r_ln_fwd");
  return B4R_OK;
}

extern "C" int64_t b4r_ln_bwd_scratch_floats(int32_t rows, int32_t H) {
  if (rows <= 0 || H < 32) return 0;
  return (int64_t)ln_bwd_grid(rows, H) * 2 * H;
}

namespace {
__global__ __launch_bounds__(256) void ln_partial_reduce_kernel(const float* partial, int S, int H, float* dgamma, float* dbeta) {
  __shared__ float sp[64][4];
  const int cl = threadIdx.x & 3, zl = threadIdx.x >> 2;
  const int c = blockIdx.x * 4 + cl;
  float s = 0.f;
  if (c < 2 * H) {
    for (int z = zl; z < S; z += 64) s += partial[(int64_t)z * 2 * H + c];
  }
  sp[zl][cl] = s;
  __syncthreads();
  if (zl == 0 && c < 2 * H) {
    float t = 0.f;
#pragma unroll
    for (int z = 0; z < 64; ++z) t += sp[z][cl];
    if (c < H) dgamma[c] = t; else dbeta[c - H] = t;
  }
}
}

int b4r_ln_bwd_launch(const float* dy, const float* z, const float* mean, const float* rstd, const float* gamma,
                      int rows, int H, float* dz, float* dgamma, float* dbeta, float* scratch, const int64_t* ids,
                      const float* table, const float* pos_table, int L, int V, DropArgs drop, hipStream_t stream,
                      const float* gelu_pre, const B4rHeadMerge* merge, int act) {
  B4R_CHECK_ARG(act >= 0 && act < B4R_ACT_COUNT, B4R_E_BADARG, "ln_bwd: unknown activation %d", act);
  LnBwdP p{};
  p.gelu_pre = gelu_pre; p.act = act;
  if (merge != nullptr)
    p.merge = HeadMergeP{merge->part, merge->slices, merge->M, merge->V, merge->T, merge->E, merge->bias, merge->y, merge->row_out,
                         merge->lse_out, merge->ylab};
  p.dy = dy; p.z = z; p.mean = mean; p.rstd = rstd; p.gamma = gamma; p.dz = dz; p.partial = scratch;
  p.ids = ids; p.table = table; p.pos_table = pos_table; p.L = L; p.V = V;
  p.rows = rows; p.H = H; p.drop = drop;
  const int grid = ln_bwd_grid(rows, H);
  int rc = ids ? launch_ln_bwd<true>(p, grid, stream)
           : (gelu_pre && act != B4R_ACT_GELU) ? launch_ln_bwd<false, B4R_ACT_ANY>(p, grid, stream) : launch_ln_bwd<false>(p, grid, stream);
  if (rc) return rc;
  B4R_CHECK_LAUNCH("ln_bwd");
  if (dbeta == dgamma + H) {
    B4rReduceJob job{scratch, nullptr, nullptr, dgamma, nullptr, nullptr, grid, 1, 2 * H, 2 * H, 0};
    if (b4r_reduce_queue_push(job)) return B4R_OK;
  }
  hipLaunchKernelGGL(ln_partial_reduce_kernel, dim3(b4r_cdiv(2 * H, 4)), dim3(256), 0, stream, scratch, grid, H,
                     dgamma, dbeta);
  B4R_CHECK_LAUNCH("ln_bwd reduce");
  return B4R_OK;
}

extern "C" int b4r_ln_bwd(const float* dy, const float* z, const float* mean, const float* rstd, const float* gamma,
                          int32_t rows, int32_t H, float* dz, float* dgamma, float* dbeta, float* scratch,
                          b4r_stream_t stream) {
  B4R_CHECK_ARG(dy && z && mean && rstd && gamma && dz && dgamma && dbeta && scratch, B4R_E_BADARG,
                "b4r_ln_bwd: null argument");
  B4R_CHECK_ARG(rows > 0, B4R_E_SHAPE, "b4r_ln_bwd: bad shape");
  return b4r_ln_bwd_launch(dy, z, mean, rstd, gamma, rows, H, dz, dgamma, dbeta, scratch, nullptr, nullptr, nullptr, 1,
                           1, b4r_make_drop(nullptr, 0, 0.f, 0), (hipStream_t)stream, nullptr, nullptr, B4R_ACT_GELU);
}
extern "C" int b4r_ln_bwd_act(const float* dy, const float* z, const float* mean, const float* rstd, const float* gamma,
                              int32_t rows, int32_t H, float* dz, float* dgamma, float* dbeta, float* scratch,
                              const float* act_pre, int32_t activation, b4r_stream_t stream) {
  B4R_CHECK_ARG(dy && z && mean && rstd && gamma && dz && dgamma && dbeta && scratch, B4R_E_BADARG,
                "b4r_ln_bwd_act: null argument");
  B4R_CHECK_ARG(rows > 0, B4R_E_SHAPE, "b4r_ln_bwd_act: bad shape");
  return b4r_ln_bwd_launch(dy, z, mean, rstd, gamma, rows, H, dz, dgamma, dbeta, scratch, nullptr, nullptr, nullptr, 1,
                           1, b4r_make_drop(nullptr, 0, 0.f, 0), (hipStream_t)stream, act_pre, nullptr, activation);
}

extern "C" int b4r_gather_rows(const float* src, int32_t src_ld, const int64_t* idx, int64_t idx_add_per, int32_t per,
                               int32_t n, int32_t H, float* dst, b4r_stream_t stream) {
  B4R_CHECK_ARG(src && idx && dst, B4R_E_BADARG, "b4r_gather_rows: null argument");
  B4R_CHECK_ARG(n > 0 && H > 0 && H % 4 == 0 && per > 0 && src_ld % 4 == 0, B4R_E_SHAPE, "b4r_gather_rows: bad shape");
  int grid = b4r_cdiv((int64_t)n * (H / 4), 256);
  if (grid > 4096) grid = 4096;
  hipLaunchKernelGGL(gather_rows_kernel, dim3(grid), dim3(256), 0, (hipStream_t)stream, src, src_ld, idx, idx_add_per,
                     per, n, H, dst);
  B4R_CHECK_LAUNCH("b4r_gather_rows");
  return B4R_OK;
}

int64_t b4r_scatter_hot_scratch_floats(int hot_rows, int H) { return (int64_t)HOT_SLOTS * hot_rows * H; }

int b4r_scatter_add_rows_impl(const float* src, const int64_t* idx, int64_t idx_add_per, int per, int n, int H,
                              float* dst, int dst_ld, const int64_t* skip_if_zero, int64_t dst_rows, int hot_rows,
                              float* hot_scratch, hipStream_t stream) {
  int grid = b4r_cdiv((int64_t)n * H, 256);
  const int cap = hot_rows > 0 ? 1024 : 8192;
  if (grid > cap) grid = cap;
  if (hot_rows <= 0) hot_scratch = nullptr;
  hipLaunchKernelGGL(scatter_add_rows_kernel, dim3(grid), dim3(256), (size_t)hot_rows * H * sizeof(float), stream, src, idx,
                     idx_add_per, per, n, H, dst, dst_ld, skip_if_zero, dst_rows, hot_rows, hot_scratch);
  B4R_CHECK_LAUNCH("b4r_scatter_add_rows");
  if (hot_scratch)
    return b4r_launch_slab_reduce_full(hot_scratch, HOT_SLOTS, hot_rows, H, dst, dst_ld, 1, nullptr, nullptr, nullptr, nullptr, stream);
  return B4R_OK;
}

extern "C" int b4r_scatter_add_rows(const float* src, const int64_t* idx, int64_t idx_add_per, int32_t per, int32_t n,
                                    int32_t H, float* dst, int32_t dst_ld, const int64_t* skip_if_zero,
                                    b4r_stream_t stream) {
  B4R_CHECK_ARG(src && idx && dst, B4R_E_BADARG, "b4r_scatter_add_rows: null argument");
  B4R_CHECK_ARG(n > 0 && H > 0 && H % 4 == 0 && per > 0 && dst_ld % 4 == 0, B4R_E_SHAPE, "b4r_scatter_add_rows: bad shape");
  return b4r_scatter_add_rows_impl(src, idx, idx_add_per, per, n, H, dst, dst_ld, skip_if_zero, (int64_t)1 << 62, 0, nullptr,
                                   (hipStream_t)stream);
}

int b4r_batch_colsum(const float* x, int B, int L, int H, float* dpos, float* scratch, hipStream_t stream) {
  const int bchunk = 16;
  const int S = b4r_cdiv(B, bchunk);
  dim3 grid(b4r_cdiv((int64_t)L * (H / 4), 256), S);
  hipLaunchKernelGGL(batch_colsum_kernel, grid, dim3(256), 0, stream, x, B, L, H, bchunk, scratch);
  B4R_CHECK_LAUNCH("batch_colsum");
  return b4r_launch_slab_reduce_full(scratch, S, L, H, dpos, H, 0, nullptr, nullptr, nullptr, nullptr, stream);
}

int64_t b4r_embed_fixed_floats(int64_t V, int H, int hot_rows) { return 2 * (V * H + (int64_t)HOT_SLOTS * hot_rows * H) + 4; }
int b4r_embed_grads(const float* x, const int64_t* ids, int B, int L, int H, float* table_grad, int64_t V, int hot_rows,
                    float* fixed, float* dpos, float* colsum_scratch, hipStream_t stream, const float* fin_rows, int fin_M,
                    b4r_train_state* state, float* tail) {
  const int n = B * L, bchunk = 16, S = b4r_cdiv(B, bchunk);
  int n_scatter = b4r_cdiv((int64_t)n * H, 256);
  if (n_scatter > 1024) n_scatter = 1024;
  if (hot_rows < 0) hot_rows = 0;
  long long* fix = reinterpret_cast<long long*>(fixed);
  long long* hot = fix + V * H;
  const int gx = b4r_cdiv((int64_t)L * (H / 4), 256);
  hipLaunchKernelGGL(embed_grads_kernel, dim3(n_scatter + gx * S + (fin_rows ? 1 : 0)), dim3(256), (size_t)hot_rows * H * sizeof(long long),
                     stream, x, ids, n, H, fix, V, hot_rows, hot, n_scatter, B, L, bchunk, gx, colsum_scratch, gx * S, fin_rows, fin_M,
                     reinterpret_cast<float*>(state), tail, fix_contribution_limit(n));
  B4R_CHECK_LAUNCH("embedding gradients (scatter-add + position sums)");
  const int* poison = reinterpret_cast<const int*>(hot + (int64_t)HOT_SLOTS * hot_rows * H);
  if (!b4r_reduce_queue_attach_fixed(table_grad, fix, hot, hot_rows * H, HOT_SLOTS, poison)) {
    B4rReduceJob job{nullptr, nullptr, nullptr, table_grad, nullptr, nullptr, 0, (int)V, H, H, 1};
    job.fix = fix; job.fix_hot = hot; job.fix_hot_elems = hot_rows * H; job.fix_slots = HOT_SLOTS; job.fix_poison = poison;
    int rc = b4r_launch_reduce_job(job, stream);
    if (rc) return rc;
  }
  return b4r_launch_slab_reduce_full(colsum_scratch, S, L, H, dpos, H, 0, nullptr, nullptr, nullptr, nullptr, stream);
}

extern "C" int b4r_softmax_ce(float* logits, int32_t M, int32_t V, int32_t ld, const int64_t* y_true,
                              float* row_scratch, b4r_train_state* state, int32_t want_grad, b4r_stream_t stream) {
  B4R_CHECK_ARG(logits && y_true && row_scratch && state, B4R_E_BADARG, "b4r_softmax_ce: null argument");
  B4R_CHECK_ARG(M > 0 && V > 0 && ld >= V, B4R_E_SHAPE, "b4r_softmax_ce: bad shape");
  B4R_CHECK_ARG(ld % 4 == 0 && b4r_aligned16(logits), B4R_E_ALIGN, "b4r_softmax_ce: logits need ld %% 4 == 0 and 16-byte alignment");
  hipLaunchKernelGGL(softmax_ce_kernel, dim3(M), dim3(256), 0, (hipStream_t)stream, logits, V, ld, y_true, row_scratch,
                     want_grad & 1);
  B4R_CHECK_LAUNCH("b4r_softmax_ce");
  hipLaunchKernelGGL(ce_finalize_kernel, dim3(1), dim3(256), 0, (hipStream_t)stream, row_scratch, M, state, (want_grad >> 2) & 1);
  B4R_CHECK_LAUNCH("b4r_softmax_ce finalize");
  return B4R_OK;
}

__global__ __launch_bounds__(256) void zero2_kernel(float* a, int64_t na4, float* b, int64_t nb4, float* tail, float* state_f,
                                                    const float* fin_rows, int fin_M, H32PackP rider, int rider_blocks) {
  __shared__ float s[4][256];
  const int main_blocks = gridDim.x - rider_blocks;
  if ((int)blockIdx.x >= main_blocks) {
    h32_pack_tile_any(rider, (int)blockIdx.x - main_blocks);
    return;
  }
  const f32x4 z = {0.f, 0.f, 0.f, 0.f};
  const bool fin = fin_rows != nullptr && (int)blockIdx.x == main_blocks - 1;
  if (fin) {
    float r[4];
    loss_rows_reduce(fin_rows, fin_M, s, r);
    if (threadIdx.x == 0) {
      state_f[4] = r[0]; state_f[5] = r[1]; state_f[6] = r[2]; state_f[7] = r[3];
      state_f[8] = (float)fin_M; state_f[9] = 0.f; state_f[10] = 0.f;
    }
    __syncthreads();
  }
  if (tail != nullptr && (fin_rows != nullptr ? fin : blockIdx.x == 0) && threadIdx.x < 8)
    tail[threadIdx.x] = threadIdx.x < 5 ? state_f[4 + threadIdx.x] : 0.f;
  for (int64_t i = (int64_t)blockIdx.x * 256 + threadIdx.x; i < na4 + nb4; i += (int64_t)main_blocks * 256) {
    if (i < na4) *reinterpret_cast<f32x4*>(a + 4 * i) = z;
    else *reinterpret_cast<f32x4*>(b + 4 * (i - na4)) = z;
  }
}
int b4r_zero2(float* a, int64_t na, float* b, int64_t nb, hipStream_t stream, float* tail, b4r_train_state* state,
              const float* fin_rows, int fin_M, const void* rider, int rider_blocks) {
  B4R_CHECK_ARG(na % 4 == 0 && nb % 4 == 0 && b4r_aligned16(a) && b4r_aligned16(b), B4R_E_ALIGN, "zero2: regions must be 16-byte granular");
  B4R_CHECK_ARG(fin_rows == nullptr || (state != nullptr && fin_M > 0), B4R_E_BADARG, "zero2: the loss sums need the state");
  int64_t n4 = (na + nb) / 4;
  int grid = (int)((n4 + 255) / 256);
  if (grid > 2048) grid = 2048;
  if (grid < 1) grid = 1;
  H32PackP job{};
  if (rider != nullptr && rider_blocks > 0) job = *reinterpret_cast<const H32PackP*>(rider);
  else rider_blocks = 0;
  hipLaunchKernelGGL(zero2_kernel, dim3(grid + rider_blocks), dim3(256), 0, stream, a, na / 4, b, nb / 4, tail, reinterpret_cast<float*>(state),
                     fin_rows, fin_M, job, rider_blocks);
  B4R_CHECK_LAUNCH(fin_rows ? "zero fill + loss sums" : "zero fill");
  return B4R_OK;
}

int b4r_ce_finalize_launch(const float* row_scratch, int M, b4r_train_state* state, int overwrite, hipStream_t stream) {
  B4R_CHECK_ARG(row_scratch && state && M > 0, B4R_E_BADARG, "ce_finalize: bad argument");
  hipLaunchKernelGGL(ce_finalize_kernel, dim3(1), dim3(256), 0, stream, row_scratch, M, state, overwrite);
  B4R_CHECK_LAUNCH("b4r_loss finalize");
  return B4R_OK;
}

extern "C" int b4r_state_begin_step(b4r_train_state* state, b4r_stream_t stream) {
  B4R_CHECK_ARG(state, B4R_E_BADARG, "b4r_state_begin_step: null state");
  hipLaunchKernelGGL(state_begin_kernel, dim3(1), dim3(64), 0, (hipStream_t)stream, state);
  B4R_CHECK_LAUNCH("b4r_state_begin_step");
  return B4R_OK;
}

extern "C" int b4r_global_sqnorm(const float* g, int64_t n, float* scratch, b4r_train_state* state, b4r_stream_t stream) {
  B4R_CHECK_ARG(g && scratch && state, B4R_E_BADARG, "b4r_global_sqnorm: null argument");
  B4R_CHECK_ARG(n > 0, B4R_E_SHAPE, "b4r_global_sqnorm: bad size");
  B4R_CHECK_ARG(b4r_aligned16(g), B4R_E_ALIGN, "b4r_global_sqnorm: buffer must be 16-byte aligned");
  int np = (int)((n / 4 + 1023) / 1024);
  if (np > 1024) np = 1024;
  if (np < 1) np = 1;
  hipLaunchKernelGGL(sqnorm_partial_kernel, dim3(np), dim3(256), 0, (hipStream_t)stream, g, n, scratch, (const float*)nullptr,
                     (float*)nullptr);
  B4R_CHECK_LAUNCH("b4r_global_sqnorm");
  hipLaunchKernelGGL(sqnorm_final_kernel, dim3(1), dim3(256), 0, (hipStream_t)stream, scratch, np, state);
  B4R_CHECK_LAUNCH("b4r_global_sqnorm final");
  return B4R_OK;
}

int b4r_optimizer_fused(const b4r_adamw_config* hp, float* params, const float* grads, float* adam_m, float* adam_v, int64_t n,
                        int64_t n_decay, float* scratch, b4r_train_state* state, hipStream_t stream, int sums_from_tail, int np_given) {
  int np = (int)((n / 4 + 1023) / 1024);
  if (np > 1024) np = 1024;
  if (np < 1) np = 1;
  unsigned int* ticket = reinterpret_cast<unsigned int*>(&state->reserved[0]);
  if (np_given > 0 && !sums_from_tail) {
    np = np_given;
  } else {
    hipLaunchKernelGGL(sqnorm_partial_kernel, dim3(np), dim3(256), 0, stream, grads, n, scratch,
                       sums_from_tail ? grads + n : (const float*)nullptr, reinterpret_cast<float*>(state));
    B4R_CHECK_LAUNCH("global norm");
  }
  AdamP a;
  a.p = params; a.g = grads; a.m = adam_m; a.v = adam_v; a.n = n; a.n_decay = n_decay; a.hp = *hp; a.st = state;
  int grid = (int)((n / 4 + 255) / 256);
  if (grid > 2048) grid = 2048;
  hipLaunchKernelGGL(adamw_fused_kernel, dim3(grid), dim3(256), 0, stream, a, (const float*)scratch, np, ticket);
  B4R_CHECK_LAUNCH("optimizer step");
  return B4R_OK;
}

extern "C" int b4r_adamw_step(const b4r_adamw_config* hp, float* params, const float* grads, float* adam_m,
                              float* adam_v, int64_t n, int64_t n_decay, b4r_train_state* state, b4r_stream_t stream) {
  B4R_CHECK_ARG(hp && params && grads && adam_m && adam_v && state, B4R_E_BADARG, "b4r_adamw_step: null argument");
  B4R_CHECK_ARG(n > 0 && n % 4 == 0 && n_decay >= 0 && n_decay <= n, B4R_E_SHAPE, "b4r_adamw_step: n must be a positive multiple of 4");
  B4R_CHECK_ARG(b4r_aligned16(params) && b4r_aligned16(grads) && b4r_aligned16(adam_m) && b4r_aligned16(adam_v),
                B4R_E_ALIGN, "b4r_adamw_step: buffers must be 16-byte aligned");
  AdamP a;
  a.p = params; a.g = grads; a.m = adam_m; a.v = adam_v; a.n = n; a.n_decay = n_decay; a.hp = *hp; a.st = state;
  int grid = (int)((n / 4 + 255) / 256);
  if (grid > 2048) grid = 2048;
  hipLaunchKernelGGL(adamw_kernel, dim3(grid), dim3(256), 0, (hipStream_t)stream, a);
  B4R_CHECK_LAUNCH("b4r_adamw_step");
  hipLaunchKernelGGL(state_advance_kernel, dim3(1), dim3(64), 0, (hipStream_t)stream, state);
  B4R_CHECK_LAUNCH("b4r_adamw_step advance");
  return B4R_OK;
}

__global__ __launch_bounds__(64) void mask_batch_kernel(const int64_t* tokens, const int64_t* row_index, const int64_t* row_finetune,
                                                        int L, int P, int V, double rate, float mask_rate,
                                                        float random_rate, int finetune_all, uint32_t seed_lo, uint32_t seed_hi,
                                                        int64_t* ids_out, int64_t* mask_out, int64_t* labels_out,
                                                        int64_t* pos_out, int64_t* mids_out, int64_t* w_out) {
  __shared__ uint32_t s_key[256];
  __shared__ int s_sel[256];
  const int row = blockIdx.x, lane = threadIdx.x;
  const int64_t srow = row_index ? row_index[row] : (int64_t)row;
  const int finetune = (finetune_all != 0 || (row_finetune != nullptr && row_finetune[srow] != 0)) ? 1 : 0;
  const int64_t* src = tokens + srow * L;
  int len = 0, n = 0;
  for (int i = lane; i < L; i += 64) {
    const int64_t t = src[i];
    len += (t != 0) ? 1 : 0;
    n += (t != 0 && t != 2) ? 1 : 0;
  }
#pragma unroll
  for (int o = 32; o > 0; o >>= 1) { len += __shfl_xor(len, o, 64); n += __shfl_xor(n, o, 64); }
  const uint32_t rk = b4r_hash32((uint32_t)srow * 0x9E3779B9u + seed_hi);
  int num;
  if (finetune) num = len > 0 ? 1 : 0;
  else num = n > 0 ? min(P, max(1, (int)((double)n * rate))) : 0;
  for (int i = lane; i < L; i += 64) {
    s_key[i] = b4r_hash32(b4r_hash32((uint32_t)i ^ seed_lo) + rk);
    s_sel[i] = 0;
  }
  __syncthreads();
  for (int i = lane; i < L; i += 64) {
    int sel = 0;
    if (finetune) sel = (i == len - 1) ? 1 : 0;
    else if (i < n) {
      int rank = 0;
      const uint32_t ki = s_key[i];
      for (int j = 0; j < n; ++j) { const uint32_t kj = s_key[j]; rank += (kj < ki || (kj == ki && j < i)) ? 1 : 0; }
      sel = rank < num ? 1 : 0;
    }
    s_sel[i] = sel;
  }
  __syncthreads();
  for (int i = lane; i < L; i += 64) {
    const int64_t t = src[i];
    int64_t out = t;
    if (s_sel[i]) {
      int slot = 0;
      for (int j = 0; j < i; ++j) slot += s_sel[j];
      pos_out[(int64_t)row * P + slot] = i;
      mids_out[(int64_t)row * P + slot] = t;
      w_out[(int64_t)row * P + slot] = 1;
      if (finetune) out = 1;
      else {
        const uint32_t h = b4r_hash32(s_key[i] ^ 0x68E31DA4u);
        const float rn = b4r_uniform23(h);
        if (rn < mask_rate) out = 1;
        else if (rn < mask_rate + random_rate) {
          const uint32_t k = b4r_hash32(h + 0x9E3779B9u) % (uint32_t)(V - 2);
          out = (k == 0) ? 1 : (int64_t)k + 2;
        }
      }
    }
    ids_out[(int64_t)row * L + i] = out;
    mask_out[(int64_t)row * L + i] = (i < len) ? 1 : 0;
    labels_out[(int64_t)row * L + i] = t;
  }
  for (int s = num + lane; s < P; s += 64) {
    pos_out[(int64_t)row * P + s] = 0; mids_out[(int64_t)row * P + s] = 0; w_out[(int64_t)row * P + s] = 0;
  }
}

extern "C" int b4r_mask_batch(const int64_t* tokens, const int64_t* row_index, const int64_t* row_finetune, int32_t B, int32_t L,
                              int32_t P, int32_t V, double selection_rate,
                              float mask_token_rate, float random_token_rate, int32_t finetune, uint64_t seed,
                              int64_t* input_word_ids, int64_t* input_mask, int64_t* labels, int64_t* masked_lm_positions,
                              int64_t* masked_lm_ids, int64_t* masked_lm_weights, b4r_stream_t stream) {
  B4R_CHECK_ARG(tokens && input_word_ids && input_mask && labels && masked_lm_positions && masked_lm_ids && masked_lm_weights,
                B4R_E_BADARG, "b4r_mask_batch: null argument");
  B4R_CHECK_ARG(B > 0 && L > 0 && L <= 256 && P > 0 && V > 3, B4R_E_SHAPE, "b4r_mask_batch: bad shape (L <= 256)");
  hipLaunchKernelGGL(mask_batch_kernel, dim3(B), dim3(64), 0, (hipStream_t)stream, tokens, row_index, row_finetune, L, P, V, selection_rate,
                     mask_token_rate, random_token_rate, finetune, (uint32_t)seed, (uint32_t)(seed >> 32), input_word_ids,
                     input_mask, labels, masked_lm_positions, masked_lm_ids, masked_lm_weights);
  B4R_CHECK_LAUNCH("b4r_mask_batch");
  return B4R_OK;
}

extern "C" float b4r_uniform_from_hash(uint32_t hash_word) { return b4r_uniform23(hash_word); }

__global__ __launch_bounds__(256) void mlm_rows_kernel(const int64_t* pos, const int64_t* ids, int L, int P, int M, int* rows, int* n_rows,
                                                       int* row_slot) {
  const int m = blockIdx.x * 256 + threadIdx.x;
  if (m == 0) *n_rows = M;
  if (m >= M) return;
  const int64_t q = pos[m];
  rows[m] = (m / P) * L + (q < 0 ? 0 : (q >= L ? L - 1 : (int)q));
  row_slot[m] = ids[m] != 0 ? m : -1;
}

extern "C" int b4r_mlm_rows(const int64_t* masked_lm_positions, const int64_t* masked_lm_ids, int32_t B, int32_t L, int32_t P, int32_t* rows,
                            int32_t* n_rows, int32_t* row_slot, b4r_stream_t stream) {
  B4R_CHECK_ARG(masked_lm_positions && masked_lm_ids && rows && n_rows && row_slot, B4R_E_BADARG, "b4r_mlm_rows: null argument");
  B4R_CHECK_ARG(B > 0 && L > 0 && P > 0 && (int64_t)B * L < (1ll << 31) && (int64_t)B * P < (1ll << 31), B4R_E_SHAPE,
                "b4r_mlm_rows: bad shape (B=%d L=%d P=%d)", B, L, P);
  const int M = B * P;
  hipLaunchKernelGGL(mlm_rows_kernel, dim3((M + 255) / 256), dim3(256), 0, (hipStream_t)stream, masked_lm_positions, masked_lm_ids, L, P, M,
                     rows, n_rows, row_slot);
  B4R_CHECK_LAUNCH("b4r_mlm_rows");
  return B4R_OK;
}

__device__ __forceinline__ uint32_t key_image(float k) {
  const uint32_t b = __builtin_bit_cast(uint32_t, k);
  return (b & 0x80000000u) ? ~b : (b | 0x80000000u);
}
constexpr int SAMPLE_MAX_C = 1024;

__global__ __launch_bounds__(256) void sample_candidates_kernel(const float* logp, int V, const int64_t* exclude, int E,
                                                                const int64_t* gt, int C, uint32_t seed_lo,
                                                                uint32_t seed_hi, int64_t* cand, uint8_t* short_flag) {
  extern __shared__ float s_key[];
  __shared__ int s_hist[256];
  __shared__ uint32_t s_selu[SAMPLE_MAX_C];
  __shared__ int s_seli[SAMPLE_MAX_C];
  __shared__ int s_tie[256];
  __shared__ int s_cnt[4];
  __shared__ uint32_t s_prefix;
  __shared__ int s_remaining;
  const int row = blockIdx.x, tid = threadIdx.x;
  const uint32_t rk = b4r_hash32((uint32_t)row * 0x9E3779B9u + seed_hi);
  for (int v = tid; v < V; v += 256) {
    uint32_t h = b4r_hash32((uint32_t)v ^ seed_lo);
    h = b4r_hash32(h + rk);
    const float u = b4r_uniform23(h);
    s_key[v] = logp[v] - __logf(-__logf(u));
  }
  if (tid < 4) s_cnt[tid] = 0;
  __syncthreads();
  for (int e = tid; e < E; e += 256) {
    const int64_t id = exclude[(int64_t)row * E + e];
    if (id >= 0 && id < V) s_key[id] = -INFINITY;
  }
  const int64_t g = gt ? gt[row] : -1;
  if (tid == 0 && g >= 0 && g < V) s_key[g] = -INFINITY;
  __syncthreads();
  {
    int n = 0;
    for (int v = tid; v < V; v += 256) n += s_key[v] > -INFINITY ? 1 : 0;
    n = (int)b4r_wave_sum((float)n);
    if ((tid & 63) == 0) atomicAdd(&s_cnt[0], n);
  }
  __syncthreads();
  const int Ce = min(C, s_cnt[0]);
  int64_t* out = cand + (int64_t)row * (C + 1);
  if (Ce > 0) {
    if (tid == 0) { s_prefix = 0u; s_remaining = Ce; }
    for (int pass = 0; pass < 4; ++pass) {
      const int shift = 24 - 8 * pass;
      s_hist[tid] = 0;
      __syncthreads();
      const uint32_t prefix = s_prefix;
      const uint32_t himask = pass == 0 ? 0u : 0xFFFFFFFFu << (shift + 8);
      for (int v = tid; v < V; v += 256) {
        const uint32_t u = key_image(s_key[v]);
        if ((u & himask) == prefix) atomicAdd(&s_hist[(u >> shift) & 255u], 1);
      }
      __syncthreads();
      if (tid < 64) {
        const int remaining = s_remaining;
        int c4[4], above = 0;
#pragma unroll
        for (int q = 0; q < 4; ++q) c4[q] = s_hist[255 - (4 * tid + q)];
        const int mine = c4[0] + c4[1] + c4[2] + c4[3];
        int incl = mine;
#pragma unroll
        for (int o = 1; o < 64; o <<= 1) {
          const int n = __shfl_up(incl, o, 64);
          if (tid >= o) incl += n;
        }
        above = incl - mine;
// ... 183 lines not shown
```

Baseline: 19.14 million.

## Split reduce queue into ready and late jobs, run ready ones inside embed-grads launch

Queued gradient slab reductions are now tagged ready or late. Reductions that do not depend on the embedding scatter are folded into the embedding-gradient kernel launch as extra rider blocks (1024-thread blocks), and only the late ones (table gradient fix-up, position sums) go to the final multi-reduce. This saves a launch and lets independent reduction work overlap with the scatter. It also quarters the hot slot count when a queue is active, unrolls the batch colsum loads, and moves the reduce code into a shared header. The cost is added complexity in norm-partial indexing and larger blocks for the scatter work.

```diff
diff --git a/bert4rec_amd/csrc/b4r_common.h b/bert4rec_amd/csrc/b4r_common.h
--- a/bert4rec_amd/csrc/b4r_common.h
+++ b/bert4rec_amd/csrc/b4r_common.h
@@ -35,6 +35,7 @@
   const float* slab; const float* cslab; const float* caslab;
   float* out; float* colsum; float* colsum_a;
   int S, Mo, No, ldo, accumulate;
+  int late = 0;
   const long long* fix = nullptr; const long long* fix_hot = nullptr;
   int fix_hot_elems = 0, fix_slots = 0;
   const int* fix_poison = nullptr;
@@ -43,10 +44,12 @@
 struct B4rReduceQueue {
   B4rReduceJob jobs[B4R_MAX_REDUCE_JOBS];
   int n;
-};
-void b4r_reduce_queue_begin(B4rReduceQueue* q);
-int b4r_reduce_queue_flush(hipStream_t stream, float* sq_partial = nullptr, int sq_cap = 0, int* sq_np = nullptr,
-                           int64_t* covered = nullptr);
+  bool ready_taken;
+  float* sq_partial; int sq_cap;
+};
+void b4r_reduce_queue_begin(B4rReduceQueue* q, float* sq_partial = nullptr, int sq_cap = 0);
+int b4r_reduce_queue_flush(hipStream_t stream, int* sq_np = nullptr, int64_t* covered = nullptr);
+bool b4r_reduce_queue_active();
 bool b4r_reduce_queue_push(const B4rReduceJob& job);
 bool b4r_reduce_queue_attach_fixed(const float* out, const long long* fix, const long long* fix_hot, int fix_hot_elems, int fix_slots,
                                    const int* fix_poison = nullptr);
diff --git a/bert4rec_amd/csrc/b4r_gemm.hip b/bert4rec_amd/csrc/b4r_gemm.hip
--- a/bert4rec_amd/csrc/b4r_gemm.hip
+++ b/bert4rec_amd/csrc/b4r_gemm.hip
@@ -1,4 +1,5 @@
 #include "b4r_common.h"
+#include "b4r_slab_reduce.h"
 
 namespace {
 
@@ -297,134 +298,10 @@
   }
 }
 
-constexpr int RZ = 16;
-constexpr int RE = 256;
-constexpr int RQ = 4096;
-typedef B4rReduceJob ReduceJobView;
-__device__ __forceinline__ int reduce_mat_blocks(int S, int64_t total) { return (int)((total + (S <= RZ ? RQ : RE) - 1) / (S <= RZ ? RQ : RE)); }
-__device__ __forceinline__ float reduce_store(const ReduceJobView& job, int64_t eo, float r) {
-  const int row = (int)(eo / job.No), col = (int)(eo % job.No);
-  float* o = job.out + (int64_t)row * job.ldo + col;
-  if (job.fix != nullptr) {
-    long long q = job.fix[eo];
-    if (eo < job.fix_hot_elems) {
-      for (int s0 = 0; s0 < job.fix_slots; s0 += 16) {
-        long long v[16];
-#pragma unroll
-        for (int u = 0; u < 16; ++u) v[u] = s0 + u < job.fix_slots ? job.fix_hot[(int64_t)(s0 + u) * job.fix_hot_elems + eo] : 0ll;
-#pragma unroll
-        for (int u = 0; u < 16; ++u) q += v[u];
-      }
-    }
-    r += (float)q * (1.f / 68719476736.f);
-    if (job.fix_poison != nullptr && *job.fix_poison != 0) r = __builtin_nanf("");
-  }
-  if (job.accumulate) r += *o;
-  *o = r;
-  return r;
-}
-__device__ __forceinline__ float slab_reduce_block(const ReduceJobView& job, int block, float (*sp)[RE]) {
-  float sq = 0.f;
-  const int64_t total = (int64_t)job.Mo * job.No;
-  const int mat_blocks = reduce_mat_blocks(job.S, total);
-  const int lane = threadIdx.x & 63, zl = __builtin_amdgcn_readfirstlane(threadIdx.x >> 6);
-  const bool vec = (total % 4 == 0) && ((reinterpret_cast<uintptr_t>(job.slab) & 15) == 0);
-  if (block < mat_blocks && job.S <= RZ) {
-    const int64_t e = (int64_t)block * RQ + 4 * (int64_t)threadIdx.x;
-    if (e >= total) return sq;
-    f32x4 v[RZ];
-#pragma unroll
-    for (int z = 0; z < RZ; ++z) {
-      v[z] = (f32x4){0.f, 0.f, 0.f, 0.f};
-      if (z < job.S) {
-        if (vec) v[z] = *reinterpret_cast<const f32x4*>(job.slab + (int64_t)z * total + e);
-        else
-#pragma unroll
-          for (int k = 0; k < 4; ++k)
-            if (e + k < total) v[z][k] = job.slab[(int64_t)z * total + e + k];
-      }
-    }
-    f32x4 r = {0.f, 0.f, 0.f, 0.f};
-#pragma unroll
-    for (int z = 0; z < RZ; ++z) r += v[z];
-#pragma unroll
-    for (int k = 0; k < 4; ++k)
-      if (e + k < total) { const float w = reduce_store(job, e + k, r[k]); sq = fmaf(w, w, sq); }
-    return sq;
-  }
-  if (block < mat_blocks) {
-    const int64_t e = (int64_t)block * RE + 4 * lane;
-    f32x4 s = {0.f, 0.f, 0.f, 0.f};
-    if (vec) {
-      if (e < total) {
-        const float* src = job.slab + e;
-        for (int z = zl; z < job.S; z += 8 * RZ) {
-          f32x4 v[8];
-#pragma unroll
-          for (int u = 0; u < 8; ++u)
-            v[u] = z + u * RZ < job.S ? *reinterpret_cast<const f32x4*>(src + (int64_t)(z + u * RZ) * total) : (f32x4){0.f, 0.f, 0.f, 0.f};
-#pragma unroll
-          for (int u = 0; u < 8; ++u) s += v[u];
-        }
-      }
-    } else {
-      for (int z = zl; z < job.S; z += RZ) {
-#pragma unroll
-        for (int c = 0; c < 4; ++c)
-          if (e + c < total) s[c] += job.slab[(int64_t)z * total + e + c];
-      }
-    }
-    *reinterpret_cast<f32x4*>(&sp[zl][4 * lane]) = s;
-    __syncthreads();
-    if (zl < 4) {
-      const int l = threadIdx.x;
-      const int64_t eo = (int64_t)block * RE + l;
-      if (eo < total) {
-        float r = 0.f;
-#pragma unroll
-        for (int z = 0; z < RZ; ++z) r += sp[z][l];
-        const float v = reduce_store(job, eo, r);
-        sq = v * v;
-      }
-    }
-    return sq;
-  }
-  const int64_t n_cs = job.colsum ? job.No : 0, n_csa = job.colsum_a ? job.Mo : 0;
-  const int64_t e = (int64_t)(block - mat_blocks) * 64 + lane;
-  const float* src = nullptr;
-  int64_t stride = 0, idx = 0;
-  if (e < n_cs) { src = job.cslab; stride = job.No; idx = e; }
-  else if (e < n_cs + n_csa) { src = job.caslab; stride = job.Mo; idx = e - n_cs; }
-  float s = 0.f;
-  if (src) {
-    for (int z = zl; z < job.S; z += 8 * RZ) {
-      float v[8];
-#pragma unroll
-      for (int u = 0; u < 8; ++u) v[u] = z + u * RZ < job.S ? src[(int64_t)(z + u * RZ) * stride + idx] : 0.f;
-#pragma unroll
-      for (int u = 0; u < 8; ++u) s += v[u];
-    }
-  }
-  sp[zl][lane] = s;
-  __syncthreads();
-  if (zl == 0 && src) {
-    float r = 0.f;
-#pragma unroll
-    for (int z = 0; z < RZ; ++z) r += sp[z][lane];
-    if (e < n_cs) job.colsum[idx] = r;
-    else job.colsum_a[idx] = r;
-    sq = r * r;
-  }
-  return sq;
-}
 
 __global__ __launch_bounds__(64 * RZ) void slab_reduce_kernel(ReduceJobView job) {
   __shared__ __attribute__((aligned(16))) float sp[RZ][RE];
   (void)slab_reduce_block(job, (int)blockIdx.x, sp);
-}
-
-int slab_reduce_grid(int S, int Mo, int No, bool cs, bool csa) {
-  return b4r_cdiv((int64_t)Mo * No, S <= RZ ? RQ : RE) + b4r_cdiv((int64_t)(cs ? No : 0) + (csa ? Mo : 0), 64);
 }
 
 int tn_split(int R, int Mo, int No) {
@@ -478,48 +355,53 @@
 }
 
 namespace {
-struct MultiReduceP {
-  B4rReduceJob jobs[B4R_MAX_REDUCE_JOBS];
-  int block_begin[B4R_MAX_REDUCE_JOBS + 1];
-  int n;
-  float* sq_partial;
-};
-__global__ __launch_bounds__(64 * RZ) void multi_slab_reduce_kernel(MultiReduceP p) {
+__global__ __launch_bounds__(64 * RZ) void multi_slab_reduce_kernel(B4rMultiReduceP p) {
   __shared__ __attribute__((aligned(16))) float sp[RZ][RE];
-  int j = 0;
-  while (j + 1 < p.n && (int)blockIdx.x >= p.block_begin[j + 1]) ++j;
-  const B4rReduceJob q = p.jobs[j];
-  float sq = slab_reduce_block(q, (int)blockIdx.x - p.block_begin[j], sp);
-  if (p.sq_partial != nullptr) {
-    __shared__ float s_sq[RZ];
-    sq = b4r_wave_sum(sq);
-    __syncthreads();
-    if ((threadIdx.x & 63) == 0) s_sq[threadIdx.x >> 6] = sq;
-    __syncthreads();
-    if (threadIdx.x == 0) {
-      float t = 0.f;
-#pragma unroll
-      for (int z = 0; z < RZ; ++z) t += s_sq[z];
-      p.sq_partial[blockIdx.x] = t;
-    }
-  }
+  __shared__ float s_sq[RZ];
+  multi_reduce_block(p, (int)blockIdx.x, sp, s_sq);
 }
 thread_local B4rReduceQueue* g_queue = nullptr;
-}
-
-void b4r_reduce_queue_begin(B4rReduceQueue* q) { q->n = 0; g_queue = q; }
+
+int job_grid(const B4rReduceJob& j) { return slab_reduce_grid(j.S, j.Mo, j.No, j.colsum != nullptr, j.colsum_a != nullptr); }
+int queue_launch_desc(const B4rReduceQueue& q, int want_late, B4rMultiReduceP* p, int* all_blocks) {
+  int blocks = 0, all = 0;
+  p->n = 0;
+  for (int j = 0; j < q.n; ++j) {
+    const int g = job_grid(q.jobs[j]);
+    if (want_late < 0 || q.jobs[j].late == want_late) {
+      p->jobs[p->n] = q.jobs[j];
+      p->block_begin[p->n] = blocks;
+      p->sq_begin[p->n] = all;
+      ++p->n;
+      blocks += g;
+    }
+    all += g;
+  }
+  p->block_begin[p->n] = blocks;
+  p->sq_partial = (q.sq_partial != nullptr && all <= q.sq_cap) ? q.sq_partial : nullptr;
+  if (all_blocks) *all_blocks = all;
+  return blocks;
+}
+}
+
+void b4r_reduce_queue_begin(B4rReduceQueue* q, float* sq_partial, int sq_cap) {
+  q->n = 0; q->ready_taken = false; q->sq_partial = sq_partial; q->sq_cap = sq_cap;
+  g_queue = q;
+}
+bool b4r_reduce_queue_active() { return g_queue != nullptr && !g_queue->ready_taken; }
 bool b4r_reduce_queue_push(const B4rReduceJob& job) {
-  if (g_queue == nullptr || g_queue->n >= B4R_MAX_REDUCE_JOBS) return false;
+  if (g_queue == nullptr || g_queue->ready_taken || g_queue->n >= B4R_MAX_REDUCE_JOBS) return false;
   g_queue->jobs[g_queue->n++] = job;
   return true;
 }
 bool b4r_reduce_queue_attach_fixed(const float* out, const long long* fix, const long long* fix_hot, int fix_hot_elems, int fix_slots,
                                    const int* fix_poison) {
-  if (g_queue == nullptr) return false;
+  if (g_queue == nullptr || g_queue->ready_taken) return false;
   for (int j = 0; j < g_queue->n; ++j) {
     B4rReduceJob& job = g_queue->jobs[j];
     if (job.out == out && job.ldo == job.No && job.fix == nullptr) {
       job.fix = fix; job.fix_hot = fix_hot; job.fix_hot_elems = fix_hot_elems; job.fix_slots = fix_slots; job.fix_poison = fix_poison;
+      job.late = 1;
       return true;
     }
   }
@@ -527,30 +409,32 @@
 }
 int b4r_launch_reduce_job(const B4rReduceJob& job, hipStream_t stream) {
   if (b4r_reduce_queue_push(job)) return B4R_OK;
-  hipLaunchKernelGGL(slab_reduce_kernel, dim3(slab_reduce_grid(job.S, job.Mo, job.No, job.colsum != nullptr, job.colsum_a != nullptr)),
-                     dim3(64 * RZ), 0, stream, job);
+  hipLaunchKernelGGL(slab_reduce_kernel, dim3(job_grid(job)), dim3(64 * RZ), 0, stream, job);
   B4R_CHECK_LAUNCH("slab_reduce");
   return B4R_OK;
 }
-int b4r_reduce_queue_flush(hipStream_t stream, float* sq_partial, int sq_cap, int* sq_np, int64_t* covered) {
+int b4r_reduce_queue_take_ready(B4rMultiReduceP* p) {
+  B4rReduceQueue* q = g_queue;
+  if (q == nullptr || q->ready_taken) return 0;
+  int n_late = 0;
+  for (int j = 0; j < q->n; ++j) n_late += q->jobs[j].late ? 1 : 0;
+  if (n_late == 0 || n_late == q->n) return 0;
+  q->ready_taken = true;
+  return queue_launch_desc(*q, 0, p, nullptr);
+}
+int b4r_reduce_queue_flush(hipStream_t stream, int* sq_np, int64_t* covered) {
   B4rReduceQueue* q = g_queue;
   g_queue = nullptr;
   if (sq_np) *sq_np = 0;
   if (covered) *covered = 0;
   if (q == nullptr || q->n == 0) return B4R_OK;
-  MultiReduceP p;
-  p.n = q->n;
-  int blocks = 0;
+  B4rMultiReduceP p;
+  int all = 0;
+  const int blocks = queue_launch_desc(*q, q->ready_taken ? 1 : -1, &p, &all);
   int64_t elems = 0;
-  for (int j = 0; j < q->n; ++j) {
-    p.jobs[j] = q->jobs[j];
-    p.block_begin[j] = blocks;
-    blocks += slab_reduce_grid(q->jobs[j].S, q->jobs[j].Mo, q->jobs[j].No, q->jobs[j].colsum != nullptr, q->jobs[j].colsum_a != nullptr);
+  for (int j = 0; j < q->n; ++j)
     elems += (int64_t)q->jobs[j].Mo * q->jobs[j].No + (q->jobs[j].colsum ? q->jobs[j].No : 0) + (q->jobs[j].colsum_a ? q->jobs[j].Mo : 0);
-  }
-  p.block_begin[q->n] = blocks;
-  p.sq_partial = (sq_partial != nullptr && blocks <= sq_cap) ? sq_partial : nullptr;
-  if (p.sq_partial && sq_np) *sq_np = blocks;
+  if (p.sq_partial && sq_np) *sq_np = all;
   if (covered) *covered = elems;
   hipLaunchKernelGGL(multi_slab_reduce_kernel, dim3(blocks), dim3(64 * RZ), 0, stream, p);
   B4R_CHECK_LAUNCH("multi_slab_reduce");
diff --git a/bert4rec_amd/csrc/b4r_model.hip b/bert4rec_amd/csrc/b4r_model.hip
--- a/bert4rec_amd/csrc/b4r_model.hip
+++ b/bert4rec_amd/csrc/b4r_model.hip
@@ -1173,7 +1173,8 @@
                 "b4r_backward: the factorised embedding needs layer 0's attention backward as products");
   const ParamLayout& pl = c.pl; const WsLayout& w = c.w;
   B4rReduceQueue queue;
-  b4r_reduce_queue_begin(&queue);
+  const bool norm_partials = (flags & B4R_FLAG_NORM_PARTIALS_INTERNAL) != 0;
+  b4r_reduce_queue_begin(&queue, norm_partials ? c.ws : nullptr, norm_partials ? 4096 : 0);
   RC(head_bwd(c));
   for (int i = c.last; i >= 0; --i) {
     const float* x_in = (i == 0) ? c.at(w.x0) : c.at(w.x2[i - 1]);
@@ -1209,13 +1210,13 @@
                      c.grd(pl.pos_emb), sc, c.s, plan.defer_combine ? c.at(w.rowsc) : nullptr, (int)w.M, state,
                      (plan.defer_combine && (flags & B4R_FLAG_GRAD_TAIL)) ? c.grd(pl.total) : nullptr));
   if (norm_np) *norm_np = 0;
-  if (!(flags & B4R_FLAG_NORM_PARTIALS_INTERNAL)) return b4r_reduce_queue_flush(c.s);
+  if (!norm_partials) return b4r_reduce_queue_flush(c.s);
   int64_t expected = 0;
   for (const ParamEntry& e : pl.entries)
     expected += (int64_t)(e.offset == pl.pos_emb ? c.L : e.rows) * e.cols;
   int np = 0;
   int64_t covered = 0;
-  RC(b4r_reduce_queue_flush(c.s, c.ws, 4096, &np, &covered));
+  RC(b4r_reduce_queue_flush(c.s, &np, &covered));
   if (norm_np && np > 0 && covered == expected) *norm_np = np;
   return B4R_OK;
 }
diff --git a/bert4rec_amd/csrc/b4r_rowops.hip b/bert4rec_amd/csrc/b4r_rowops.hip
--- a/bert4rec_amd/csrc/b4r_rowops.hip
+++ b/bert4rec_amd/csrc/b4r_rowops.hip
@@ -1,6 +1,7 @@
 #include "b4r_common.h"
 #include "b4r_head_merge.h"
 #include "b4r_head32_pack.h"
+#include "b4r_slab_reduce.h"
 
 int b4r_launch_slab_reduce_full(const float* slab, int S, int Mo, int No, float* out, int ldo, int accumulate,
                                 const float* cslab, float* colsum, const float* caslab, float* colsum_a, hipStream_t stream);
@@ -301,12 +302,21 @@
 
 __device__ __forceinline__ void batch_colsum_body(const float* x, int B, int L, int H, int bchunk, float* partial, const int bx, const int by) {
   const int h4 = H / 4;
-  const int64_t t = (int64_t)bx * 256 + threadIdx.x;
+  const int64_t t = (int64_t)bx * blockDim.x + threadIdx.x;
   if (t >= (int64_t)L * h4) return;
   const int l = (int)(t / h4), c = (int)(t % h4) * 4;
   const int b0 = by * bchunk, b1 = min(B, b0 + bchunk);
   f32x4 s = {0.f, 0.f, 0.f, 0.f};
-  for (int b = b0; b < b1; ++b) s += *reinterpret_cast<const f32x4*>(x + ((int64_t)b * L + l) * H + c);
+  constexpr int U = 8;
+  for (int bb = b0; bb < b1; bb += U) {
+    f32x4 v[U];
+#pragma unroll
+    for (int u = 0; u < U; ++u)
+      v[u] = bb + u < b1 ? *reinterpret_cast<const f32x4*>(x + ((int64_t)(bb + u) * L + l) * H + c) : (f32x4){0.f, 0.f, 0.f, 0.f};
+#pragma unroll
+    for (int u = 0; u < U; ++u)
+      if (bb + u < b1) s += v[u];
+  }
   *reinterpret_cast<f32x4*>(partial + ((int64_t)by * L + l) * H + c) = s;
 }
 __global__ __launch_bounds__(256) void batch_colsum_kernel(const float* x, int B, int L, int H, int bchunk, float* partial) {
@@ -323,13 +333,14 @@
   return lim;
 }
 __device__ __forceinline__ void scatter_fixed_rows_body(const float* src, const int64_t* idx, int n, int H, long long* fix,
-                                                        int64_t dst_rows, int hot_rows, long long* hot, const int block,
-                                                        const int nblocks, int* poison, const float limit) {
+                                                        int64_t dst_rows, int hot_rows, long long* hot, const int hot_slots,
+                                                        const int block, const int nblocks, int* poison, const float limit) {
   extern __shared__ unsigned long long s_hot64[];
-  for (int k = threadIdx.x; k < hot_rows * H; k += 256) s_hot64[k] = 0ull;
+  const int nt = (int)blockDim.x;
+  for (int k = threadIdx.x; k < hot_rows * H; k += nt) s_hot64[k] = 0ull;
   if (hot_rows > 0) __syncthreads();
   const int64_t total = (int64_t)n * H;
-  for (int64_t t = (int64_t)block * 256 + threadIdx.x; t < total; t += (int64_t)nblocks * 256) {
+  for (int64_t t = (int64_t)block * nt + threadIdx.x; t < total; t += (int64_t)nblocks * nt) {
     const int i = (int)(t / H), c = (int)(t % H);
     const int64_t r = idx[i];
     if (r < 0 || r >= dst_rows) continue;
@@ -341,9 +352,9 @@
   }
   if (hot_rows > 0) {
     __syncthreads();
-    for (int k = threadIdx.x; k < hot_rows * H; k += 256) {
+    for (int k = threadIdx.x; k < hot_rows * H; k += nt) {
       const unsigned long long v = s_hot64[k];
-      if (v != 0ull) atomicAdd(reinterpret_cast<unsigned long long*>(hot) + (int64_t)(block % HOT_SLOTS) * hot_rows * H + k, v);
+      if (v != 0ull) atomicAdd(reinterpret_cast<unsigned long long*>(hot) + (int64_t)(block % hot_slots) * hot_rows * H + k, v);
     }
   }
 }
@@ -418,10 +429,11 @@
   }
 }
 
+template <int U = 16>
 __device__ __forceinline__ void loss_rows_reduce(const float* rows, int M, float (*s)[256], float (&out)[4]) {
   const int tid = threadIdx.x;
+  if (tid >= 256) M = 0;
   f32x4 acc = {0.f, 0.f, 0.f, 0.f};
-  constexpr int U = 16;
   for (int m0 = tid; m0 < M; m0 += U * 256) {
     f32x4 r[U];
 #pragma unroll
@@ -431,8 +443,10 @@
     for (int u = 0; u < U; ++u)
       if (m0 + 256 * u < M) acc += r[u];
   }
-#pragma unroll
-  for (int q = 0; q < 4; ++q) s[q][tid] = acc[q];
+  if (tid < 256) {
+#pragma unroll
+    for (int q = 0; q < 4; ++q) s[q][tid] = acc[q];
+  }
   __syncthreads();
   if (tid < 256) {
     const int q = tid >> 6, l = tid & 63;
@@ -445,26 +459,40 @@
   for (int q = 0; q < 4; ++q) out[q] = s[q][0];
 }
 
-__global__ __launch_bounds__(256) void embed_grads_kernel(const float* x, const int64_t* ids, int n, int H, long long* fix,
-                                                          int64_t table_rows, int hot_rows, long long* hot, int n_scatter, int B, int L,
-                                                          int bchunk, int gx, float* partial, int n_colsum, const float* fin_rows,
-                                                          int fin_M, float* state_f, float* tail, float fix_limit) {
-  if ((int)blockIdx.x < n_scatter) {
-    scatter_fixed_rows_body(x, ids, n, H, fix, table_rows, hot_rows, hot, (int)blockIdx.x, n_scatter,
-                            reinterpret_cast<int*>(hot + (int64_t)HOT_SLOTS * hot_rows * H), fix_limit);
-  } else if ((int)blockIdx.x < n_scatter + n_colsum) {
-    const int k = (int)blockIdx.x - n_scatter;
-    batch_colsum_body(x, B, L, H, bchunk, partial, k % gx, k / gx);
+struct EmbedGradsP {
+  const float* x; const int64_t* ids; int n, H;
+  long long* fix; int64_t table_rows; int hot_rows; long long* hot; int hot_slots;
+  int n_scatter, B, L, bchunk, gx; float* partial; int n_colsum;
+  const float* fin_rows; int fin_M; float* state_f; float* tail; float fix_limit;
+};
+template <int LOSS_U>
+__device__ __forceinline__ void embed_grads_block(const EmbedGradsP& p, const int block, float (*s)[256]) {
+  if (block < p.n_scatter) {
+    scatter_fixed_rows_body(p.x, p.ids, p.n, p.H, p.fix, p.table_rows, p.hot_rows, p.hot, p.hot_slots, block, p.n_scatter,
+                            reinterpret_cast<int*>(p.hot + (int64_t)HOT_SLOTS * p.hot_rows * p.H), p.fix_limit);
+  } else if (block < p.n_scatter + p.n_colsum) {
+    const int k = block - p.n_scatter;
+    batch_colsum_body(p.x, p.B, p.L, p.H, p.bchunk, p.partial, k % p.gx, k / p.gx);
   } else {
-    __shared__ float s[4][256];
     float r[4];
-    loss_rows_reduce(fin_rows, fin_M, s, r);
+    loss_rows_reduce<LOSS_U>(p.fin_rows, p.fin_M, s, r);
     if (threadIdx.x == 0) {
-      state_f[4] = r[0]; state_f[5] = r[1]; state_f[6] = r[2]; state_f[7] = r[3];
-      state_f[8] = (float)fin_M; state_f[9] = 0.f; state_f[10] = 0.f;
-    }
-    if (tail != nullptr && threadIdx.x < 8) tail[threadIdx.x] = threadIdx.x < 4 ? r[threadIdx.x] : (threadIdx.x == 4 ? (float)fin_M : 0.f);
-  }
+      p.state_f[4] = r[0]; p.state_f[5] = r[1]; p.state_f[6] = r[2]; p.state_f[7] = r[3];
+      p.state_f[8] = (float)p.fin_M; p.state_f[9] = 0.f; p.state_f[10] = 0.f;
+    }
+    if (p.tail != nullptr && threadIdx.x < 8) p.tail[threadIdx.x] = threadIdx.x < 4 ? r[threadIdx.x] : (threadIdx.x == 4 ? (float)p.fin_M : 0.f);
+  }
+}
+__global__ __launch_bounds__(256) void embed_grads_kernel(EmbedGradsP p) {
+  __shared__ float s[4][256];
+  embed_grads_block<16>(p, (int)blockIdx.x, s);
+}
+__global__ __launch_bounds__(64 * RZ, 8) void embed_grads_ride_kernel(EmbedGradsP p, int main_blocks, B4rMultiReduceP riders) {
+  __shared__ __attribute__((aligned(16))) float sp[RZ][RE];
+  __shared__ float s_sq[RZ];
+  static_assert(RE == 256 && RZ >= 4, "the loss sums use [4][256] floats of sp");
+  if ((int)blockIdx.x < main_blocks) embed_grads_block<8>(p, (int)blockIdx.x, sp);
+  else multi_reduce_block<8>(riders, (int)blockIdx.x - main_blocks, sp, s_sq);
 }
 
 __global__ __launch_bounds__(256) void ce_finalize_kernel(const float* row_out, int M, b4r_train_state* st, int overwrite) {
@@ -805,24 +833,42 @@
                     float* fixed, float* dpos, float* colsum_scratch, hipStream_t stream, const float* fin_rows, int fin_M,
                     b4r_train_state* state, float* tail) {
   const int n = B * L, bchunk = 16, S = b4r_cdiv(B, bchunk);
-  int n_scatter = b4r_cdiv((int64_t)n * H, 256);
-  if (n_scatter > 1024) n_scatter = 1024;
   if (hot_rows < 0) hot_rows = 0;
   long long* fix = reinterpret_cast<long long*>(fixed);
   long long* hot = fix + V * H;
-  const int gx = b4r_cdiv((int64_t)L * (H / 4), 256);
-  hipLaunchKernelGGL(embed_grads_kernel, dim3(n_scatter + gx * S + (fin_rows ? 1 : 0)), dim3(256), (size_t)hot_rows * H * sizeof(long long),
-                     stream, x, ids, n, H, fix, V, hot_rows, hot, n_scatter, B, L, bchunk, gx, colsum_scratch, gx * S, fin_rows, fin_M,
-                     reinterpret_cast<float*>(state), tail, fix_contribution_limit(n));
-  B4R_CHECK_LAUNCH("embedding gradients (scatter-add + position sums)");
   const int* poison = reinterpret_cast<const int*>(hot + (int64_t)HOT_SLOTS * hot_rows * H);
-  if (!b4r_reduce_queue_attach_fixed(table_grad, fix, hot, hot_rows * H, HOT_SLOTS, poison)) {
-    B4rReduceJob job{nullptr, nullptr, nullptr, table_grad, nullptr, nullptr, 0, (int)V, H, H, 1};
-    job.fix = fix; job.fix_hot = hot; job.fix_hot_elems = hot_rows * H; job.fix_slots = HOT_SLOTS; job.fix_poison = poison;
-    int rc = b4r_launch_reduce_job(job, stream);
+  const int hot_slots = b4r_reduce_queue_active() ? HOT_SLOTS / 4 : HOT_SLOTS;
+  B4rReduceJob table_job{nullptr, nullptr, nullptr, table_grad, nullptr, nullptr, 0, (int)V, H, H, 1};
+  table_job.fix = fix; table_job.fix_hot = hot; table_job.fix_hot_elems = hot_rows * H; table_job.fix_slots = hot_slots;
+  table_job.fix_poison = poison; table_job.late = 1;
+  B4rReduceJob pos_job{colsum_scratch, nullptr, nullptr, dpos, nullptr, nullptr, S, L, H, H, 0};
+  pos_job.late = 1;
+  const bool table_pending = !b4r_reduce_queue_attach_fixed(table_grad, fix, hot, hot_rows * H, hot_slots, poison) &&
+                             !b4r_reduce_queue_push(table_job);
+  const bool pos_pending = !b4r_reduce_queue_push(pos_job);
+  B4rMultiReduceP riders;
+  const int rider_blocks = b4r_reduce_queue_take_ready(&riders);
+  const int nt = rider_blocks > 0 ? 64 * RZ : 256;
+  int n_scatter = b4r_cdiv((int64_t)n * H, nt);
+  if (n_scatter > 1024 * 256 / nt) n_scatter = 1024 * 256 / nt;
+  const int gx = b4r_cdiv((int64_t)L * (H / 4), nt);
+  EmbedGradsP p{x, ids, n, H, fix, V, hot_rows, hot, hot_slots, n_scatter, B, L, bchunk, gx, colsum_scratch, gx * S, fin_rows, fin_M,
+                reinterpret_cast<float*>(state), tail, fix_contribution_limit(n)};
+  const int main_blocks = n_scatter + gx * S + (fin_rows ? 1 : 0);
+  const size_t lds = (size_t)hot_rows * H * sizeof(long long);
+  if (rider_blocks > 0) {
+    hipLaunchKernelGGL(embed_grads_ride_kernel, dim3(main_blocks + rider_blocks), dim3(nt), lds, stream, p, main_blocks, riders);
+    B4R_CHECK_LAUNCH("embedding gradients (scatter-add + position sums) + ready reductions");
+  } else {
+    hipLaunchKernelGGL(embed_grads_kernel, dim3(main_blocks), dim3(nt), lds, stream, p);
+    B4R_CHECK_LAUNCH("embedding gradients (scatter-add + position sums)");
+  }
+  if (table_pending) {
+    int rc = b4r_launch_reduce_job(table_job, stream);
     if (rc) return rc;
   }
-  return b4r_launch_slab_reduce_full(colsum_scratch, S, L, H, dpos, H, 0, nullptr, nullptr, nullptr, nullptr, stream);
+  if (pos_pending) return b4r_launch_reduce_job(pos_job, stream);
+  return B4R_OK;
 }
 
 extern "C" int b4r_softmax_ce(float* logits, int32_t M, int32_t V, int32_t ld, const int64_t* y_true,
diff --git a/bert4rec_amd/csrc/b4r_slab_reduce.h b/bert4rec_amd/csrc/b4r_slab_reduce.h
--- /dev/null
+++ b/bert4rec_amd/csrc/b4r_slab_reduce.h
@@ -0,0 +1,168 @@
+#pragma once
+#include "b4r_common.h"
+
+struct B4rMultiReduceP {
+  B4rReduceJob jobs[B4R_MAX_REDUCE_JOBS];
+  int block_begin[B4R_MAX_REDUCE_JOBS + 1];
+  int sq_begin[B4R_MAX_REDUCE_JOBS];
+  int n;
+  float* sq_partial;
+};
+int b4r_reduce_queue_take_ready(B4rMultiReduceP* p);
+
+namespace {
+
+constexpr int RZ = 16;
+constexpr int RE = 256;
+constexpr int RQ = 4096;
+typedef B4rReduceJob ReduceJobView;
+__device__ __forceinline__ int reduce_mat_blocks(int S, int64_t total) { return (int)((total + (S <= RZ ? RQ : RE) - 1) / (S <= RZ ? RQ : RE)); }
+template <int NF = RZ>
+__device__ __forceinline__ float reduce_store(const ReduceJobView& job, int64_t eo, float r) {
+  const int row = (int)(eo / job.No), col = (int)(eo % job.No);
+  float* o = job.out + (int64_t)row * job.ldo + col;
+  if (job.fix != nullptr) {
+    long long q = job.fix[eo];
+    if (eo < job.fix_hot_elems) {
+      for (int s0 = 0; s0 < job.fix_slots; s0 += NF) {
+        long long v[NF];
+#pragma unroll
+        for (int u = 0; u < NF; ++u) v[u] = s0 + u < job.fix_slots ? job.fix_hot[(int64_t)(s0 + u) * job.fix_hot_elems + eo] : 0ll;
+#pragma unroll
+        for (int u = 0; u < NF; ++u) q += v[u];
+      }
+    }
+    r += (float)q * (1.f / 68719476736.f);
+    if (job.fix_poison != nullptr && *job.fix_poison != 0) r = __builtin_nanf("");
+  }
+  if (job.accumulate) r += *o;
+  *o = r;
+  return r;
+}
+template <int NF = RZ>
+__device__ __forceinline__ float slab_reduce_block(const ReduceJobView& job, int block, float (*sp)[RE]) {
+  static_assert(RZ % NF == 0, "whole batches of loads");
+  float sq = 0.f;
+  const int64_t total = (int64_t)job.Mo * job.No;
+  const int mat_blocks = reduce_mat_blocks(job.S, total);
+  const int lane = threadIdx.x & 63, zl = __builtin_amdgcn_readfirstlane(threadIdx.x >> 6);
+  const bool vec = (total % 4 == 0) && ((reinterpret_cast<uintptr_t>(job.slab) & 15) == 0);
+  if (block < mat_blocks && job.S <= RZ) {
+    const int64_t e = (int64_t)block * RQ + 4 * (int64_t)threadIdx.x;
+    if (e >= total) return sq;
+    f32x4 r = {0.f, 0.f, 0.f, 0.f};
+#pragma unroll 1
+    for (int z0 = 0; z0 < RZ; z0 += NF) {
+      f32x4 v[NF];
+#pragma unroll
+      for (int u = 0; u < NF; ++u) {
+        const int z = z0 + u;
+        v[u] = (f32x4){0.f, 0.f, 0.f, 0.f};
+        if (z < job.S) {
+          if (vec) v[u] = *reinterpret_cast<const f32x4*>(job.slab + (int64_t)z * total + e);
+          else
+#pragma unroll
+            for (int k = 0; k < 4; ++k)
+              if (e + k < total) v[u][k] = job.slab[(int64_t)z * total + e + k];
+        }
+      }
+#pragma unroll
+      for (int u = 0; u < NF; ++u) r += v[u];
+    }
+#pragma unroll
+    for (int k = 0; k < 4; ++k)
+      if (e + k < total) { const float w = reduce_store<NF>(job, e + k, r[k]); sq = fmaf(w, w, sq); }
+    return sq;
+  }
+  if (block < mat_blocks) {
+    const int64_t e = (int64_t)block * RE + 4 * lane;
+    f32x4 s = {0.f, 0.f, 0.f, 0.f};
+    if (vec) {
+      if (e < total) {
+        const float* src = job.slab + e;
+        for (int z = zl; z < job.S; z += 8 * RZ) {
+          f32x4 v[8];
+#pragma unroll
+          for (int u = 0; u < 8; ++u)
+            v[u] = z + u * RZ < job.S ? *reinterpret_cast<const f32x4*>(src + (int64_t)(z + u * RZ) * total) : (f32x4){0.f, 0.f, 0.f, 0.f};
+#pragma unroll
+          for (int u = 0; u < 8; ++u) s += v[u];
+        }
+      }
+    } else {
+      for (int z = zl; z < job.S; z += RZ) {
+#pragma unroll
+        for (int c = 0; c < 4; ++c)
+          if (e + c < total) s[c] += job.slab[(int64_t)z * total + e + c];
+      }
+    }
+    *reinterpret_cast<f32x4*>(&sp[zl][4 * lane]) = s;
+    __syncthreads();
+    if (zl < 4) {
+      const int l = threadIdx.x;
+      const int64_t eo = (int64_t)block * RE + l;
+      if (eo < total) {
+        float r = 0.f;
+#pragma unroll
+        for (int z = 0; z < RZ; ++z) r += sp[z][l];
+        const float v = reduce_store<NF>(job, eo, r);
+        sq = v * v;
+      }
+    }
+    return sq;
+  }
+  const int64_t n_cs = job.colsum ? job.No : 0, n_csa = job.colsum_a ? job.Mo : 0;
+  const int64_t e = (int64_t)(block - mat_blocks) * 64 + lane;
+  const float* src = nullptr;
+  int64_t stride = 0, idx = 0;
+  if (e < n_cs) { src = job.cslab; stride = job.No; idx = e; }
+  else if (e < n_cs + n_csa) { src = job.caslab; stride = job.Mo; idx = e - n_cs; }
+  float s = 0.f;
+  if (src) {
+    for (int z = zl; z < job.S; z += 8 * RZ) {
+      float v[8];
+#pragma unroll
+      for (int u = 0; u < 8; ++u) v[u] = z + u * RZ < job.S ? src[(int64_t)(z + u * RZ) * stride + idx] : 0.f;
+#pragma unroll
+      for (int u = 0; u < 8; ++u) s += v[u];
+    }
+  }
+  sp[zl][lane] = s;
+  __syncthreads();
+  if (zl == 0 && src) {
+    float r = 0.f;
+#pragma unroll
+    for (int z = 0; z < RZ; ++z) r += sp[z][lane];
+    if (e < n_cs) job.colsum[idx] = r;
+    else job.colsum_a[idx] = r;
+    sq = r * r;
+  }
+  return sq;
+}
+
+inline int slab_reduce_grid(int S, int Mo, int No, bool cs, bool csa) {
+  return b4r_cdiv((int64_t)Mo * No, S <= RZ ? RQ : RE) + b4r_cdiv((int64_t)(cs ? No : 0) + (csa ? Mo : 0), 64);
+}
+
+template <int NF = RZ>
+__device__ __forceinline__ void multi_reduce_block(const B4rMultiReduceP& p, int block, float (*sp)[RE], float* s_sq) {
+  int j = 0;
+  while (j + 1 < p.n && block >= p.block_begin[j + 1]) ++j;
+  const B4rReduceJob q = p.jobs[j];
+  const int b = block - p.block_begin[j];
+  float sq = slab_reduce_block<NF>(q, b, sp);
+  if (p.sq_partial != nullptr) {
+    sq = b4r_wave_sum(sq);
+    __syncthreads();
+    if ((threadIdx.x & 63) == 0) s_sq[threadIdx.x >> 6] = sq;
+    __syncthreads();
+    if (threadIdx.x == 0) {
+      float t = 0.f;
+#pragma unroll
+      for (int z = 0; z < RZ; ++z) t += s_sq[z];
+      p.sq_partial[p.sq_begin[j] + b] = t;
+    }
+  }
+}
+
+}
```

Measured after the change: 19.29 million (median of 6 runs). About the same (+0.8%).
